# fgnt/padertorch

Measured on AMD Instinct MI355X. Metric: training frames/sec (PIT mask-est, 2-spk 8 kHz), higher is better.
Workload: dtype f32; 1 GPU; BASELINE configs[1]: PIT mask estimator (3xBLSTM-600, K=2, 23.5M params), 32 x 4 s 2-spk 8000 Hz mixtures per GPU and micro-step (8096 frames), 1 micro-step(s) per optimizer step, STFT 512/128 on device, full optimizer step (Adam, clip 1); global_batch=32, parallelism=dp1, blstm=HIP recurrence (csrc/lstm_split.hip), step_driver=one hipGraph per optimizer step (train.graphed.GraphedStep), replayed, lstm_weight_gradients=in place, side stream next to the next recurrence

## Files before the change

include/ptmi.h:

```cpp
#ifndef PTMI_H_
#define PTMI_H_

#include <stdint.h>

#ifdef __cplusplus
extern "C" {
#endif

#define PTMI_OK 0
#define PTMI_E_INVALID (-1)
#define PTMI_E_UNSUPPORTED (-2)

typedef void* ptmi_stream_t;

const char* ptmi_version(void);
const char* ptmi_error_string(int code);

typedef struct ptmi_stft_geom {
    int32_t size;
    int32_t shift;
    int32_t window_length;
    int32_t pad_left;
    int32_t pad_right;
    int32_t pad;
} ptmi_stft_geom;

int64_t ptmi_stft_num_frames(const ptmi_stft_geom* g, int64_t num_samples);
int64_t ptmi_istft_num_samples(const ptmi_stft_geom* g, int64_t num_frames);

#define PTMI_LAYOUT_INTERLEAVED 0
#define PTMI_LAYOUT_CONCAT 1

int ptmi_stft_forward(const float* x, int64_t batch, int64_t x_row_stride, int64_t num_samples,
                      const int32_t* row_samples, const float* window, const float* twiddle,
                      const ptmi_stft_geom* g, int64_t out_frames, int32_t layout, float edge_scale,
                      float* out, ptmi_stream_t stream);

int ptmi_istft_forward(const float* spec, int64_t batch, int64_t num_frames, const int32_t* row_frames,
                       const float* syn_window, const float* twiddle, const ptmi_stft_geom* g,
                       int32_t layout, float edge_scale, int64_t cut_left, int64_t out_samples,
                       int64_t out_row_stride, float* out, ptmi_stream_t stream);

int ptmi_pit_features(const float* y, const float* s, int64_t batch, int32_t K, int64_t row_stride,
                      int64_t num_samples, const int32_t* row_samples, const float* window,
                      const float* twiddle, const ptmi_stft_geom* g, int64_t out_frames, float* Y_abs,
                      float* X_abs, float* cos_pd, ptmi_stream_t stream);
int ptmi_pit_features_packed(const float* y, const float* s, int64_t batch, int32_t K, int64_t row_stride,
                             int64_t num_samples, const int32_t* row_samples, const float* window,
                             const float* twiddle, const ptmi_stft_geom* g, int64_t out_frames, float* Y_abs,
                             float* X_abs, float* cos_pd, float* log1p_packed, uint16_t* log1p_planes,
                             const int64_t* packed_offsets, ptmi_stream_t stream);


int64_t ptmi_pit_workspace_elems(int64_t batch, int64_t t_len, int32_t K, int32_t F);
int ptmi_pit_pairwise_sse(const float* est, const float* obs, const float* tgt, const float* tgt_scale,
                          int64_t batch, int64_t t_len, const int64_t* strides, int32_t K, int32_t F,
                          const int32_t* row_frames, double* workspace, double* sse,
                          ptmi_stream_t stream);

int ptmi_pit_assign(const double* sse, int64_t batch, int32_t nvar, int32_t K, int32_t F,
                    int64_t t_len, const int32_t* row_frames, float* loss, int32_t* perm,
                    float* ex_loss, ptmi_stream_t stream);

int ptmi_pit_backward(const float* est, const float* obs, const float* tgt, const float* tgt_scale,
                      const int32_t* perm, const float* gscale, int64_t batch, int64_t t_len,
                      const int64_t* strides, int32_t K, int32_t F, int32_t nvar, const int32_t* row_frames,
                      float* grad, ptmi_stream_t stream);

int64_t ptmi_dc_workspace_elems(int64_t batch, int64_t T, int32_t F);
int ptmi_dc_loss_forward(const float* x, const float* t, int64_t batch, int64_t T, const int64_t* strides,
                         int32_t E, int32_t K, int32_t F, const int32_t* row_frames, float* workspace,
                         double* gram, float* ex_loss, float* loss, ptmi_stream_t stream);
int ptmi_dc_loss_backward(const float* x, const float* t, const double* gram, const float* gscale,
                          int64_t batch, int64_t T, const int64_t* strides, int32_t E, int32_t K, int32_t F,
                          const int32_t* row_frames, float* dx, ptmi_stream_t stream);


int ptmi_lstm_forward(float* gates, float* hy, float* c, const float* c0, const float* w_hh_pad, const int32_t* batch_sizes,
                      const int64_t* offsets, int32_t T, int32_t max_batch, int32_t H, int32_t KP,
                      int32_t ndir, ptmi_stream_t stream);

int ptmi_lstm_backward(const float* gates, const float* c, const float* c0, const float* dhy, const float* w_hh_t, float* dgates,
                       float* dc_state, const int32_t* batch_sizes, const int64_t* offsets, int32_t T,
                       int32_t max_batch, int32_t H, int32_t ndir, ptmi_stream_t stream);

int64_t ptmi_lstm_flags_elems(int32_t T, int32_t ndir, int32_t max_batch);
int64_t ptmi_lstm_scratch_elems(int32_t T, int32_t ndir, int32_t max_batch, int32_t H, int32_t backward);
int ptmi_lstm_weight_prep(const float* const* w_ih, const float* const* w_hh, const float* const* b_ih,
                          const float* const* b_hh, int32_t ndir, int32_t H, int32_t I, float* w_ih_cat, int32_t Ipad,
                          float* bias, float* w_pad, int32_t KP, float* w_t, uint32_t* amax, ptmi_stream_t stream);
int ptmi_lstm_set_error_sink(uint32_t* word);
int ptmi_lstm_split_enabled(void);
int32_t ptmi_lstm_handoff_cols(int32_t H, int32_t backward);
int32_t ptmi_lstm_backward_planes_ok(int32_t T, int32_t ndir, int32_t max_batch, int64_t rows, int32_t H);
int ptmi_lstm_forward_fills(int32_t T, int32_t ndir, int32_t max_batch, int32_t H);

int ptmi_lstm_forward_persistent(float* gates, float* hy, float* c, const float* c0, const float* w_hh_pad,
                                 const uint32_t* w_hh_amax, const int32_t* batch_sizes_dev, const int64_t* offsets_dev,
                                 const uint64_t* step_masks, uint32_t* flags, int32_t T, int32_t max_batch, int64_t rows,
                                 int32_t H, int32_t KP, int32_t ndir, int32_t prefilled, uint32_t* backward_scratch,
                                 ptmi_stream_t stream);

int ptmi_lstm_backward_persistent(const float* gates, const float* c, const float* c0, const float* dhy, const float* dc_n,
                                  const float* w_hh_t, float* dgates, uint16_t* dgates_t, const int32_t* batch_sizes_dev,
                                  const int64_t* offsets_dev, const uint64_t* step_masks, uint32_t* flags, float* dc_carry,
                                  int32_t T, int32_t max_batch, int64_t rows, int32_t H, int32_t ndir, int32_t s_begin,
                                  int32_t s_end, int32_t prefilled, ptmi_stream_t stream);

int ptmi_stft_logmel(const float* x, int64_t batch, int64_t x_row_stride, int64_t num_samples,
                     const int32_t* row_samples, const float* window, const float* twiddle,
                     const ptmi_stft_geom* g, int64_t out_frames, const int32_t* mel_lo, const int32_t* mel_cnt,
                     const int32_t* mel_off, const float* mel_w, int32_t mel_M, int32_t mel_nnz, int32_t power,
                     int32_t log_, float eps, float* out, ptmi_stream_t stream);
int ptmi_mel_apply(const float* spec, int64_t N, int32_t F, const int32_t* mel_lo, const int32_t* mel_cnt,
                   const int32_t* mel_off, const float* mel_w, int32_t mel_M, int32_t mel_nnz, int32_t log_,
                   float eps, float* out, ptmi_stream_t stream);

typedef struct ptmi_norm_geom {
    int32_t rank;
    int64_t size[5];
    int64_t stat_group_stride[5];
    int64_t indep_stride[5];
    int32_t batch_dim, seq_dim;
} ptmi_norm_geom;
int64_t ptmi_norm_workspace_elems(const ptmi_norm_geom* geom, int32_t which);
int ptmi_norm_reduce(int32_t mode, const float* x, const float* gy, const int32_t* lengths, const float* mean,
                     const float* rstd, const float* gamma, const ptmi_norm_geom* geom, int32_t shift,
                     double* workspace, double* out, ptmi_stream_t stream);
int ptmi_norm_elementwise(int32_t backward, const float* x, const float* gy, const int32_t* lengths,
                          const float* mean, const float* rstd, const float* gamma, const float* beta,
                          const float* c0, const float* c1, const ptmi_norm_geom* geom, int32_t shift,
                          int32_t scale, float* out, ptmi_stream_t stream);

int ptmi_unit_norm_forward(const float* x, float* y, float* inv_norm, int64_t N, int32_t E, int32_t F, float eps,
                           ptmi_stream_t stream);
int ptmi_unit_norm_backward(const float* gy, const float* y, const float* inv_norm, float* dx, int64_t N, int32_t E,
                            int32_t F, float eps, ptmi_stream_t stream);

int64_t ptmi_td_stats_elems(int32_t K);
int64_t ptmi_td_workspace_elems(int64_t batch, int32_t K, int64_t T);
int ptmi_td_pair_stats(const float* est, const float* tgt, const int32_t* lengths, int64_t batch, int32_t K,
                       int64_t T, const int64_t* strides, double* workspace, double* stats,
                       ptmi_stream_t stream);
int ptmi_td_lincomb(const float* x, const float* y, const int32_t* lengths, const float* coef_a,
                    const float* coef_b, const float* coef_c, int64_t batch, int32_t K, int64_t T,
                    const int64_t* strides, float* out, ptmi_stream_t stream);

int ptmi_tas_analysis(const float* x, const float* weight, const float* bias, float* out, int64_t B, int64_t T, int32_t N,
                      int32_t L, int32_t stride, int64_t E, int32_t relu, ptmi_stream_t stream);
int ptmi_tas_synthesis(const float* p, const float* mask, const float* gate, const float* weight, const float* bias, float* y,
                       int32_t K, int64_t B, int32_t N, int32_t L, int32_t stride, int64_t E, int64_t T_out,
                       ptmi_stream_t stream);
int ptmi_tas_masked_decode_backward(const float* gy, const float* mask, const float* encoded, const float* weight, float* dmask,
                                    float* dencoded, int32_t K, int64_t B, int64_t T, int32_t N, int32_t L, int32_t stride,
                                    int64_t E, ptmi_stream_t stream);
int64_t ptmi_tas_wgrad_workspace_elems(int64_t B, int32_t N, int32_t L, int32_t stride, int64_t E);
int ptmi_tas_wgrad(const float* g, const float* mask, const float* gate, const float* x, int32_t K, int64_t B, int64_t T,
                   int32_t N, int32_t L, int32_t stride, int64_t E, float* workspace, float* out, ptmi_stream_t stream);

int64_t ptmi_tcn_depthwise_workspace_elems(int64_t B, int64_t T, int32_t H, int32_t K);
int ptmi_tcn_depthwise_forward(const float* u, const float* slope_in, const float* weight, const float* bias, const float* slope_out,
                               float* v, float* stats, double* workspace, int64_t B, int64_t T, int32_t H, int32_t K,
                               int32_t dilation, float eps, ptmi_stream_t stream);
int ptmi_tcn_depthwise_backward(const float* gv, const float* u, const float* slope_in, const float* weight, const float* bias,
                                const float* slope_out, float* gz, float* gu, float* dparams, double* workspace, int64_t B,
                                int64_t T, int32_t H, int32_t K, int32_t dilation, ptmi_stream_t stream);
int64_t ptmi_tcn_norm_workspace_elems(int64_t B, int64_t T, int32_t C);
int ptmi_tcn_norm_stats(const float* x, float* stats, double* workspace, int64_t B, int64_t T, int32_t C, int32_t rows, float eps,
                        ptmi_stream_t stream);
int ptmi_tcn_norm_apply(const float* x, const float* stats, const float* gamma, const float* beta, float* y, int64_t B, int64_t T,
                        int32_t C, int32_t rows, ptmi_stream_t stream);
int ptmi_tcn_norm_backward(const float* gy, const float* x, const float* stats, const float* gamma, float* dx, float* dparams,
                           float* gsum, double* workspace, int64_t B, int64_t T, int32_t C, int32_t rows, ptmi_stream_t stream);

int64_t ptmi_tasnet_entry_norm_workspace_elems(int64_t B, int32_t N, int64_t E);
int ptmi_tasnet_entry_norm_forward(const float* w, const float* gamma, const float* beta, const void* lengths, int32_t lengths_int64,
                                   float* y, float* stats, int64_t B, int32_t N, int64_t E, float eps, ptmi_stream_t stream);
int ptmi_tasnet_entry_norm_backward(const float* gy, const float* w, const float* stats, const float* gamma, const void* lengths,
                                    int32_t lengths_int64, float* dw, float* dparams, double* workspace, int64_t B, int32_t N,
                                    int64_t E, ptmi_stream_t stream);
int64_t ptmi_tasnet_prelu_workspace_elems(int64_t n);
int ptmi_tasnet_prelu_forward(const float* x, const float* slope, float* y, int64_t n, ptmi_stream_t stream);
int ptmi_tasnet_prelu_backward(const float* g, const float* x, const float* slope, float* gx, float* dslope, double* workspace,
                               int64_t n, ptmi_stream_t stream);
// ... 141 lines not shown
```

padertorch_amd/_lib.py:

```python
import ctypes
import os
import threading
from ctypes import c_char_p, c_double, c_float, c_int, c_int32, c_int64, c_void_p, POINTER
from pathlib import Path

import torch

_PKG = Path(__file__).resolve().parent
LIB_PATH = _PKG / 'libptmi.so'
if os.environ.get('PTMI_LIB'):
    LIB_PATH = Path(os.environ['PTMI_LIB'])


class StftGeom(ctypes.Structure):
    _fields_ = [('size', c_int32), ('shift', c_int32), ('window_length', c_int32),
                ('pad_left', c_int32), ('pad_right', c_int32), ('pad', c_int32)]


class NormGeom(ctypes.Structure):
    _fields_ = [('rank', c_int32), ('size', c_int64 * 5), ('stat_group_stride', c_int64 * 5),
                ('indep_stride', c_int64 * 5), ('batch_dim', c_int32), ('seq_dim', c_int32)]


_P = c_void_p
_G = POINTER(StftGeom)
_I64P = POINTER(c_int64)

SIGNATURES = {
    'ptmi_version': (c_char_p, []),
    'ptmi_error_string': (c_char_p, [c_int]),
    'ptmi_stft_num_frames': (c_int64, [_G, c_int64]),
    'ptmi_istft_num_samples': (c_int64, [_G, c_int64]),
    'ptmi_stft_forward': (c_int, [_P, c_int64, c_int64, c_int64, _P, _P, _P, _G, c_int64, c_int32,
                                  c_float, _P, _P]),
    'ptmi_istft_forward': (c_int, [_P, c_int64, c_int64, _P, _P, _P, _G, c_int32, c_float, c_int64,
                                   c_int64, c_int64, _P, _P]),
    'ptmi_pit_features': (c_int, [_P, _P, c_int64, c_int32, c_int64, c_int64, _P, _P, _P, _G, c_int64,
                                  _P, _P, _P, _P]),
    'ptmi_pit_features_packed': (c_int, [_P, _P, c_int64, c_int32, c_int64, c_int64, _P, _P, _P, _G, c_int64,
                                         _P, _P, _P, _P, _P, _P, _P]),
    'ptmi_pit_workspace_elems': (c_int64, [c_int64, c_int64, c_int32, c_int32]),
    'ptmi_pit_pairwise_sse': (c_int, [_P, _P, _P, _P, c_int64, c_int64, _I64P, c_int32, c_int32, _P,
                                      _P, _P, _P]),
    'ptmi_pit_assign': (c_int, [_P, c_int64, c_int32, c_int32, c_int32, c_int64, _P, _P, _P, _P, _P]),
    'ptmi_pit_backward': (c_int, [_P, _P, _P, _P, _P, _P, c_int64, c_int64, _I64P, c_int32, c_int32,
                                  c_int32, _P, _P, _P]),
    'ptmi_dc_workspace_elems': (c_int64, [c_int64, c_int64, c_int32]),
    'ptmi_dc_loss_forward': (c_int, [_P, _P, c_int64, c_int64, _I64P, c_int32, c_int32, c_int32, _P, _P, _P, _P, _P, _P]),
    'ptmi_dc_loss_backward': (c_int, [_P, _P, _P, _P, c_int64, c_int64, _I64P, c_int32, c_int32, c_int32, _P, _P, _P]),
    'ptmi_stft_logmel': (c_int, [_P, c_int64, c_int64, c_int64, _P, _P, _P, _G, c_int64, _P, _P, _P, _P,
                                 c_int32, c_int32, c_int32, c_int32, c_float, _P, _P]),
    'ptmi_mel_apply': (c_int, [_P, c_int64, c_int32, _P, _P, _P, _P, c_int32, c_int32, c_int32, c_float, _P, _P]),
    'ptmi_norm_workspace_elems': (c_int64, [POINTER(NormGeom), c_int32]),
    'ptmi_norm_reduce': (c_int, [c_int32, _P, _P, _P, _P, _P, _P, POINTER(NormGeom), c_int32, _P, _P, _P]),
    'ptmi_norm_elementwise': (c_int, [c_int32, _P, _P, _P, _P, _P, _P, _P, _P, _P, POINTER(NormGeom), c_int32,
                                      c_int32, _P, _P]),
    'ptmi_td_stats_elems': (c_int64, [c_int32]),
    'ptmi_td_workspace_elems': (c_int64, [c_int64, c_int32, c_int64]),
    'ptmi_td_pair_stats': (c_int, [_P, _P, _P, c_int64, c_int32, c_int64, _I64P, _P, _P, _P]),
    'ptmi_td_lincomb': (c_int, [_P, _P, _P, _P, _P, _P, c_int64, c_int32, c_int64, _I64P, _P, _P]),
    'ptmi_tas_analysis': (c_int, [_P, _P, _P, _P, c_int64, c_int64, c_int32, c_int32, c_int32, c_int64, c_int32, _P]),
    'ptmi_tas_synthesis': (c_int, [_P, _P, _P, _P, _P, _P, c_int32, c_int64, c_int32, c_int32, c_int32, c_int64, c_int64, _P]),
    'ptmi_tas_masked_decode_backward': (c_int, [_P, _P, _P, _P, _P, _P, c_int32, c_int64, c_int64, c_int32, c_int32, c_int32,
                                                c_int64, _P]),
    'ptmi_tas_wgrad_workspace_elems': (c_int64, [c_int64, c_int32, c_int32, c_int32, c_int64]),
    'ptmi_tas_wgrad': (c_int, [_P, _P, _P, _P, c_int32, c_int64, c_int64, c_int32, c_int32, c_int32, c_int64, _P, _P, _P]),
    'ptmi_tcn_depthwise_workspace_elems': (c_int64, [c_int64, c_int64, c_int32, c_int32]),
    'ptmi_tcn_depthwise_forward': (c_int, [_P, _P, _P, _P, _P, _P, _P, _P, c_int64, c_int64, c_int32, c_int32, c_int32, c_float, _P]),
    'ptmi_tcn_depthwise_backward': (c_int, [_P, _P, _P, _P, _P, _P, _P, _P, _P, _P, c_int64, c_int64, c_int32, c_int32, c_int32, _P]),
    'ptmi_tcn_norm_workspace_elems': (c_int64, [c_int64, c_int64, c_int32]),
    'ptmi_tcn_norm_stats': (c_int, [_P, _P, _P, c_int64, c_int64, c_int32, c_int32, c_float, _P]),
    'ptmi_tcn_norm_apply': (c_int, [_P, _P, _P, _P, _P, c_int64, c_int64, c_int32, c_int32, _P]),
    'ptmi_tcn_norm_backward': (c_int, [_P, _P, _P, _P, _P, _P, _P, _P, c_int64, c_int64, c_int32, c_int32, _P]),
    'ptmi_tasnet_entry_norm_workspace_elems': (c_int64, [c_int64, c_int32, c_int64]),
    'ptmi_tasnet_entry_norm_forward': (c_int, [_P, _P, _P, _P, c_int32, _P, _P, c_int64, c_int32, c_int64, c_float, _P]),
    'ptmi_tasnet_entry_norm_backward': (c_int, [_P, _P, _P, _P, _P, c_int32, _P, _P, _P, c_int64, c_int32, c_int64, _P]),
    'ptmi_tasnet_prelu_workspace_elems': (c_int64, [c_int64]),
    'ptmi_tasnet_prelu_forward': (c_int, [_P, _P, _P, c_int64, _P]),
    'ptmi_tasnet_prelu_backward': (c_int, [_P, _P, _P, _P, _P, _P, c_int64, _P]),
    'ptmi_tasnet_mask_head_forward': (c_int, [_P, _P, _P, c_int64, c_int64, c_int32, c_int32, c_int32, c_int32, _P]),
    'ptmi_tasnet_mask_head_backward': (c_int, [_P, _P, _P, _P, c_int64, c_int64, c_int32, c_int32, c_int32, c_int32, _P]),
    'ptmi_tasnet_center_workspace_elems': (c_int64, [c_int64, c_int64, c_int64, c_int64]),
    'ptmi_tasnet_center': (c_int, [_P, _P, _P, c_int64, c_int64, c_int64, c_int64, c_int32, _P]),
    'ptmi_td_rect_workspace_elems': (c_int64, [c_int64, c_int32, c_int32, c_int64]),
    'ptmi_td_rect_stats': (c_int, [_P, _P, c_int64, c_int32, c_int32, c_int64, _I64P, _P, _P, _P, _P]),
    'ptmi_orpit_select': (c_int, [_P, _P, _P, _P, _P, _P, _P, _P, c_int64, c_int32, c_int64, _P]),
    'ptmi_td_rect_lincomb': (c_int, [_P, _P, _P, _P, _P, c_int64, c_int32, c_int32, c_int64, _I64P, _P, _P]),
    'ptmi_orpit_flag_workspace_elems': (c_int64, [c_int64, c_int32, c_int64]),
    'ptmi_orpit_flag_forward': (c_int, [_P, _P, _P, _P, _P, _P, _P, _P, _P, _P, c_int64, c_int32, c_int64, c_int32, c_int32, c_int32,
                                        c_int32, _P]),
    'ptmi_orpit_flag_backward': (c_int, [_P, _P, _P, _P, _P, _P, _P, _P, _P, _P, _P, _P, _P, _P, _P, c_int64, c_int32, c_int64, c_int32,
                                         c_int32, c_int32, c_int32, _P]),
    'ptmi_mask_loss_workspace_elems': (c_int64, [c_int64, c_int32, c_int32, c_int32]),
    'ptmi_mask_loss_forward': (c_int, [_P, _P, _P, c_int32, _P, _I64P, c_int64, c_int32, c_int32, c_int32, c_int32, _P, _P, _P, _P, _P,
                                       _P]),
    'ptmi_mask_loss_backward': (c_int, [_P, _P, _P, c_int32, _P, _I64P, _P, _P, _P, _P, c_int64, c_int32, c_int32, c_int32, c_int32, _P,
                                        _P]),
    'ptmi_gl_partials_elems': (c_int64, []),
    'ptmi_gl_project': (c_int, [_P, _P, c_int64, _P, _P]),
    'ptmi_gl_project_backward': (c_int, [_P, _P, c_int64, _P, _P]),
    'ptmi_gl_update': (c_int, [_P, _P, _P, c_int64, c_float, _P, _P, _P, _P]),
    'ptmi_gl_stft_update': (c_int, [_P, c_int64, c_int64, c_int64, _P, _P, _G, c_int64, c_float, _P, _P, _P, _P, _P, _P]),
    'ptmi_gl_finish': (c_int, [_P, c_int64, c_double, c_int32, _P, _P, _P]),
    'ptmi_bf_psd_workspace_elems': (c_int64, [c_int64, c_int32, c_int64, c_int64, c_int32]),
    'ptmi_bf_psd': (c_int, [_P, _P, _P, _P, c_int64, c_int32, c_int64, c_int64, c_int32, c_int32, c_int32, _P, _P, _P]),
    'ptmi_bf_souden': (c_int, [_P, _P, c_int64, c_int64, c_int32, c_int32, _P, _P, _P, _P, _P]),
    'ptmi_bf_apply': (c_int, [_P, _P, _P, c_int64, c_int32, c_int64, c_int64, _P, _P]),
    'ptmi_bf_eig': (c_int, [_P, _P, c_int64, c_int64, c_int32, c_int32, c_int32, _P, _P, _P, _P]),
    'ptmi_bf_ban': (c_int, [_P, _P, c_int64, c_int64, c_int32, _P, _P]),
    'ptmi_bf_phase': (c_int, [_P, c_int64, c_int64, c_int32, _P, _P]),
    'ptmi_dprnn_num_chunks': (c_int64, [c_int64, c_int32, c_int32]),
    'ptmi_dprnn_tables': (c_int, [_P, c_int32, c_int32, c_int32, c_int32, c_int32, _P, _P, _P, _P]),
    'ptmi_chunk_lstm_max_hidden': (c_int32, []),
    'ptmi_chunk_lstm_max_resident_hidden': (c_int32, []),
    'ptmi_chunk_lstm_tile': (c_int32, []),
    'ptmi_chunk_lstm_forward': (c_int, [_P, _P, _P, _P, _P, _P, _P, _P, c_int32, c_int32, c_int32, c_int32, _P]),
    'ptmi_chunk_lstm_backward': (c_int, [_P, _P, _P, _P, _P, _P, _P, _P, c_int32, c_int32, c_int32, c_int32, _P]),
    'ptmi_dprnn_colsum_workspace_elems': (c_int64, [c_int64, c_int32]),
    'ptmi_dprnn_colsum': (c_int, [_P, c_int64, _P, _P, _P, c_int64, c_int32, _P]),
    'ptmi_dprnn_norm_residual_forward': (c_int, [_P, _P, _P, _P, _P, _P, _P, c_int64, c_int32, c_int32, c_int32, c_float, _P]),
    'ptmi_dprnn_norm_residual_backward': (c_int, [_P, _P, _P, _P, _P, _P, _P, _P, _P, c_int64, c_int32, c_int32, c_int32, _P]),
    'ptmi_dprnn_segment': (c_int, [_P, _I64P, _P, c_int64, c_int64, c_int32, c_int32, c_int32, c_int32, _P]),
    'ptmi_dprnn_overlap_add': (c_int, [_P, _I64P, _P, c_int64, c_int64, c_int32, c_int32, c_int32, c_int32, c_int32, _P]),
    'ptmi_lstm_forward': (c_int, [_P, _P, _P, _P, _P, _P, _P, c_int32, c_int32, c_int32, c_int32, c_int32, _P]),
    'ptmi_lstm_backward': (c_int, [_P, _P, _P, _P, _P, _P, _P, _P, _P, c_int32, c_int32, c_int32, c_int32, _P]),
    'ptmi_unit_norm_forward': (c_int, [_P, _P, _P, c_int64, c_int32, c_int32, c_float, c_void_p]),
    'ptmi_unit_norm_backward': (c_int, [_P, _P, _P, _P, c_int64, c_int32, c_int32, c_float, c_void_p]),
    'ptmi_lstm_flags_elems': (c_int64, [c_int32, c_int32, c_int32]),
    'ptmi_lstm_scratch_elems': (c_int64, [c_int32, c_int32, c_int32, c_int32, c_int32]),
    'ptmi_lstm_weight_prep': (c_int, [_P, _P, _P, _P, c_int32, c_int32, c_int32, _P, c_int32, _P, _P, c_int32, _P, _P, _P]),
    'ptmi_lstm_set_error_sink': (c_int, [_P]),
    'ptmi_lstm_split_enabled': (c_int, []),
    'ptmi_lstm_handoff_cols': (c_int32, [c_int32, c_int32]),
    'ptmi_lstm_forward_persistent': (c_int, [_P, _P, _P, _P, _P, _P, _P, _P, _P, _P, c_int32, c_int32, c_int64, c_int32, c_int32,
                                             c_int32, c_int32, _P, _P]),
    'ptmi_lstm_forward_fills': (c_int, [c_int32, c_int32, c_int32, c_int32]),
    'ptmi_lstm_backward_planes_ok': (c_int32, [c_int32, c_int32, c_int32, c_int64, c_int32]),
    'ptmi_lstm_backward_persistent': (c_int, [_P, _P, _P, _P, _P, _P, _P, _P, _P, _P, _P, _P, _P, c_int32, c_int32, c_int64, c_int32,
                                              c_int32, c_int32, c_int32, c_int32, _P]),
    'ptmi_absmax': (c_int, [_P, c_int64, c_int64, c_int64, _P, _P]),
    'ptmi_absmax_accumulate': (c_int, [_P, c_int64, c_int64, c_int64, _P, _P]),
    'ptmi_planes_elems': (c_int64, [c_int64, c_int64]),
    'ptmi_pack_planes_t': (c_int, [_P, c_int64, c_int64, c_int64, _P, _P, _P]),
    'ptmi_gemm_planes_workspace_elems': (c_int64, [c_int32, c_int32, c_int32, c_int32]),
    'ptmi_pack_planes_n': (c_int, [_P, c_int64, c_int64, c_int64, _P, _P, _P]),
    'ptmi_gemm_planes': (c_int, [_P, _P, _P, _P, _P, _P, c_int64, c_int32, c_int32, c_int32, c_int32, c_int32, c_int32, _P, _P]),
    'ptmi_gemm_planes_relu': (c_int, [_P, _P, _P, _P, _P, _P, c_int64, c_int32, c_int32, c_int32, c_int32, c_int32, _P, _P, c_int32, _P]),
    'ptmi_relu_backward_absmax': (c_int, [_P, _P, _P, c_int64, c_int64, c_int64, c_int64, c_int64, _P, c_int32, _P]),
    'ptmi_pack_planes_t_bf16': (c_int, [_P, c_int64, c_int64, c_int64, _P, _P]),
    'ptmi_pack_planes_n_bf16': (c_int, [_P, c_int64, c_int64, c_int64, _P, _P]),
    'ptmi_pack_planes_into': (c_int, [_P, c_int64, c_int64, c_int64, c_int32, c_int32, _P, _P, c_int64, c_int64, c_int64, _P]),
    'ptmi_gemm_planes_bf16': (c_int, [_P, _P, _P, _P, c_int64, c_int32, c_int32, c_int32, c_int32, c_int32, c_int32, _P, _P]),
    'ptmi_gemm_planes_bf16_two': (c_int, [_P, _P, _P, _P, c_int32, c_int64, c_int32, c_int32, c_int32, c_int32, c_int32, c_int32, _P, _P]),
    'ptmi_gemm_planes_plan': (c_int32, [c_int32, c_int32, c_int32, c_int32]),
    'ptmi_gemm_planes_bf16_group': (c_int, [_P, c_int32, c_int32, _P, _P, c_int32, _P, _P, c_int32, c_int32, c_int32, c_int32, _P, _P]),
    'ptmi_gemm_planes_group_workspace_elems': (c_int64, [c_int32, c_int32, _P, c_int32, _P, c_int32, c_int32]),
    'ptmi_gemm_planes_group_plan': (c_int32, [c_int32, c_int32, _P, c_int32, _P, c_int32, c_int32]),
    'ptmi_pack_planes_t_bf16_list': (c_int, [_P, _P, _P, _P, c_int32, c_int64, _P]),
    'ptmi_comm_rccl_version': (c_int32, []),
    'ptmi_comm_unique_id': (c_int, [_P]),
    'ptmi_comm_create': (c_int, [_P, c_int32, c_int32, _P]),
    'ptmi_allreduce_sum': (c_int, [_P, _P, c_int64, _P]),
    'ptmi_comm_destroy': (c_int, [_P]),
    'ptmi_lstm_bias_grad_add': (c_int, [_P, c_int32, c_int32, _P, _P, _P]),
    'ptmi_grad_norm_workspace_elems': (c_int64, []),
    'ptmi_grad_norm': (c_int32, [_P, c_int64, _P, _P, _P]),
    'ptmi_adam_flat': (c_int32, [_P, _P, _P, _P, c_int32, c_int64, _P, c_float, _P, _P, _P, _P, c_double, c_double, c_double,
                                 c_double, c_double, _P, c_int32, _P]),
}

_lib = None


def load():
    global _lib
    if _lib is None:
        if not LIB_PATH.exists():
            raise ImportError(
                f'{LIB_PATH} is missing: build the HIP kernels first '
                f'(python -m padertorch_amd.build, or __graft_entry__.build()). '
                f'padertorch_amd has no CPU fallback.')
        lib = ctypes.CDLL(str(LIB_PATH))
        for name, (res, args) in SIGNATURES.items():
            fn = getattr(lib, name)
            fn.restype = res
            fn.argtypes = args
        _lib = lib
    return _lib


_hooks = None


def test_hooks():
    global _hooks
    if _hooks is None:
        path = _PKG / 'libptmi_testhooks.so'
        if not path.exists():
            raise ImportError(f'{path} is missing: python -m padertorch_amd.build')
        lib = ctypes.CDLL(str(path))
        lib.ptmi_test_occupy.restype = c_int
        lib.ptmi_test_occupy.argtypes = [c_int32, c_int32, c_int32, c_int64, _P]
        _hooks = lib
    return _hooks


def select_gemm_tile(tile):
    if tile is None or tile < 0:
        os.environ.pop('PTMI_GEMM_TILE', None)
    else:
        assert 0 <= tile <= 5, tile
        os.environ['PTMI_GEMM_TILE'] = str(int(tile))
    return 0


def check(rc, what=''):
    if rc != 0:
        msg = load().ptmi_error_string(int(rc)).decode()
        raise RuntimeError(f'{what}: {msg} (code {rc})')


def ptr(t):
    return None if t is None else t.data_ptr()


def require_gpu(*tensors):
    for t in tensors:
        if t is not None and not t.is_cuda:
            raise RuntimeError(
                'padertorch_amd ops run on an MI355X (HIP) device only and have no CPU fallback; '
                f'got a tensor on {t.device}. Move the example to the GPU first.')


def stream(device):
    return torch.cuda.current_stream(device).cuda_stream


def device_key(device):
    device = torch.device(device)
    return device.type, device.index if device.index is not None else torch.cuda.current_device()


KERNEL_TIMERS = None


def timed(name, fn, *args):
    if KERNEL_TIMERS is None:
        return fn(*args)
    e0 = torch.cuda.Event(enable_timing=True)
    e1 = torch.cuda.Event(enable_timing=True)
    e0.record()
    rc = fn(*args)
    e1.record()
    KERNEL_TIMERS.append((name, e0, e1))
    return rc


class _Staging:

    def __init__(self, half_bytes=1 << 24):
        self.half = half_bytes
        self.buf = torch.empty(2 * half_bytes, dtype=torch.uint8, pin_memory=True)
        self.np = self.buf.numpy()
        self.which, self.off = 0, 0
        self.events = [[], []]
        self.streams = [{}, {}]
        self.lock = threading.Lock()

    def put(self, t, device):
        n = t.numel() * t.element_size()
        if n > self.half // 4:
            return t.pin_memory().to(device, non_blocking=True)
        with self.lock:
            if self.off + n > self.half:
                for stream in self.streams[self.which].values():
                    ev = torch.cuda.Event()
                    ev.record(stream)
                    self.events[self.which].append(ev)
                self.streams[self.which] = {}
                self.which, self.off = self.which ^ 1, 0
                for ev in self.events[self.which]:
                    ev.synchronize()
                self.events[self.which] = []
            start = self.which * self.half + self.off
            self.off += (n + 63) // 64 * 64
            stage = self.buf[start:start + n].view(t.dtype).view(t.shape)
            self.np[start:start + n] = t.numpy().reshape(-1).view('uint8')
            cur = torch.cuda.current_stream(device)
            self.streams[self.which][cur.cuda_stream] = cur
            return stage.to(device, non_blocking=True)


_STAGING = {}


def host_to_device(values, dtype, device):
    t = torch.as_tensor(values, dtype=dtype)
    device = torch.device(device)
# ... 34 lines not shown
```

padertorch_amd/csrc/gemm_planes.hip:

```cpp
#include <algorithm>

#include "common.h"

namespace ptmi {

typedef _Float16 h8 __attribute__((ext_vector_type(8)));
typedef __bf16 b8 __attribute__((ext_vector_type(8)));
typedef float f4 __attribute__((ext_vector_type(4)));

constexpr int PBM = 128, PBN = 128;
constexpr int FR = 64;

__device__ __forceinline__ float plane_scale(const unsigned* amax_bits) {
    if (!amax_bits) return 1.f;
    const unsigned e = (*amax_bits >> 23) & 0xffu;
    if (e == 0u || e == 0xffu) return 1.f;
    return __uint_as_float((unsigned)(127 + 13 + 127 - (int)e) << 23);
}

struct PlanesArgs {
    const uint4* A;
    const uint4* B;
    float* C;
    float* workspace;
    const unsigned* amax_a;
    const unsigned* amax_b;
    const float* bias;
    int M, N, KB;
    long long ldc;
    int accumulate;
    int kb_per_split;
    int tiles_m, tiles_n;
    float* C2 = nullptr;
    int m_split = 0;
    int relu = 0;
    unsigned* amax_out = nullptr;
};

__device__ __forceinline__ void block_amax(unsigned* out, unsigned m, unsigned* red) {
#pragma unroll
    for (int o = 32; o > 0; o >>= 1) m = max(m, (unsigned)__shfl_xor((int)m, o));
    if ((threadIdx.x & 63) == 0) red[threadIdx.x >> 6] = m;
    __syncthreads();
    if (threadIdx.x == 0) {
        for (unsigned w = 1; w < (blockDim.x >> 6); ++w) m = max(m, red[w]);
        if (m != 0u) atomicMax(out, m >= 0x7f800000u ? 0x7f7fffffu : m);
    }
}

template <bool BF16, bool ONE, bool RELU = false>
__global__ __launch_bounds__(256, 2) void gemm_planes_kernel(const PlanesArgs G) {
#if __HIP_DEVICE_COMPILE__
    constexpr int PIECES = 32;
    __shared__ uint4 lds[2 * PIECES * FR];
    const int tid = threadIdx.x, lane = tid & 63, wave = tid >> 6;
    const int T = G.tiles_m * G.tiles_n;
    const int q = T / 8, r8 = T % 8, xcd = blockIdx.x & 7, idx = blockIdx.x >> 3;
    if (idx >= (xcd < r8 ? q + 1 : q)) return;
    const int tile = (xcd < r8 ? xcd * (q + 1) : r8 * (q + 1) + (xcd - r8) * q) + idx;
    const int tm = tile / G.tiles_n, tn = tile - tm * G.tiles_n;
    const int kb0 = blockIdx.z * G.kb_per_split, kb1 = min(G.KB, kb0 + G.kb_per_split);
    const int wm = wave >> 1, wn = wave & 1;
    const float inv = 1.f / (plane_scale(G.amax_a) * plane_scale(G.amax_b));
    const int rta = (G.M + 15) / 16, rtb = (G.N + 15) / 16;
    const uint4* gsrc[8];
#pragma unroll
    for (int i = 0; i < 8; ++i) {
        const int f = wave * 8 + i;
        const bool isa = f < 16;
        const int rt = (f & 15) >> 1, p = f & 1;
        const long long row_tile = min((long long)(isa ? tm : tn) * 8 + rt, (long long)(isa ? rta : rtb) - 1);
        gsrc[i] = (isa ? G.A : G.B) + ((row_tile * G.KB + kb0) * 2 + p) * FR + lane;
    }
    f4 acc[4][4];
#pragma unroll
    for (int i = 0; i < 4; ++i)
#pragma unroll
        for (int j = 0; j < 4; ++j) acc[i][j] = f4{0.f, 0.f, 0.f, 0.f};
    if (kb0 < kb1) {
#pragma unroll
        for (int i = 0; i < 8; ++i)
            if (!ONE || !(i & 1)) __builtin_amdgcn_global_load_lds(gsrc[i], &lds[(wave * 8 + i) * FR], 16, 0, 0);
    }
    for (int kb = kb0; kb < kb1; ++kb) {
        const int st = (kb - kb0) & 1;
        asm volatile("s_waitcnt vmcnt(0)" ::: "memory");
        __builtin_amdgcn_s_barrier();
        const uint4* sa = &lds[(st * PIECES + wm * 8) * FR + lane];
        const uint4* sb = &lds[(st * PIECES + 16 + wn * 8) * FR + lane];
        const bool more = kb + 1 < kb1;
        h8 bh[4], bl[4];
#pragma unroll
        for (int j = 0; j < 4; ++j) {
            bh[j] = __builtin_bit_cast(h8, sb[(j * 2 + 0) * FR]);
            bl[j] = ONE ? bh[j] : __builtin_bit_cast(h8, sb[(j * 2 + 1) * FR]);
        }
        h8 ah = __builtin_bit_cast(h8, sa[0]), al = ONE ? ah : __builtin_bit_cast(h8, sa[FR]);
#pragma unroll
        for (int i = 0; i < 4; ++i) {
            h8 nh = ah, nl = al;
            if (i + 1 < 4) {
                nh = __builtin_bit_cast(h8, sa[((i + 1) * 2 + 0) * FR]);
                nl = ONE ? nh : __builtin_bit_cast(h8, sa[((i + 1) * 2 + 1) * FR]);
            }
            if (more) {
#pragma unroll
                for (int pc = 2 * i; pc < 2 * i + 2; ++pc)
                    if (!ONE || !(pc & 1))
                        __builtin_amdgcn_global_load_lds(gsrc[pc] + (long long)(kb + 1 - kb0) * 2 * FR,
                                                         &lds[((st ^ 1) * PIECES + wave * 8 + pc) * FR], 16, 0, 0);
            }
#pragma unroll
            for (int p = ONE ? 2 : 0; p < 3; ++p)
#pragma unroll
                for (int j = 0; j < 4; ++j)
                    acc[i][j] = BF16 ? __builtin_amdgcn_mfma_f32_16x16x32_bf16(__builtin_bit_cast(b8, p == 0 ? bl[j] : bh[j]),
                                                                               __builtin_bit_cast(b8, p == 1 ? al : ah), acc[i][j], 0, 0, 0)
                                     : __builtin_amdgcn_mfma_f32_16x16x32_f16(p == 0 ? bl[j] : bh[j], p == 1 ? al : ah, acc[i][j], 0, 0, 0);
            ah = nh;
            al = nl;
        }
    }
    const bool slab = gridDim.z > 1;
    float* const Cz = slab ? G.workspace + (long long)blockIdx.z * G.M * G.N : G.C;
    const long long ldc = slab ? G.N : G.ldc;
    const bool vec = (ldc & 3) == 0 && ((reinterpret_cast<unsigned long long>(Cz) | reinterpret_cast<unsigned long long>(G.C2)) & 15) == 0;
    const bool add = G.accumulate && !slab;
    const int r = lane & 15, g = lane >> 4;
    f4 bv[4];
    {
        const bool bias_on = G.bias != nullptr && !slab;
        const bool bvec = (reinterpret_cast<unsigned long long>(G.bias) & 15) == 0;
#pragma unroll
        for (int j = 0; j < 4; ++j) {
            const int n = tn * PBN + wn * 64 + j * 16 + g * 4;
            bv[j] = f4{0.f, 0.f, 0.f, 0.f};
            if (bias_on && bvec && n + 3 < G.N) {
                bv[j] = *reinterpret_cast<const f4*>(G.bias + n);
            } else if (bias_on) {
#pragma unroll
                for (int e = 0; e < 4; ++e) bv[j][e] = G.bias[min(n + e, G.N - 1)];
            }
        }
    }
    const bool fuse = RELU && !slab;
    unsigned mx = 0u;
#pragma unroll
    for (int i = 0; i < 4; ++i) {
        const int m = tm * PBM + wm * 64 + i * 16 + r;
        if (m >= G.M) continue;
        const bool second = !slab && G.C2 != nullptr && m >= G.m_split;
        float* const rowp = second ? G.C2 + (long long)(m - G.m_split) * ldc : Cz + (long long)m * ldc;
#pragma unroll
        for (int j = 0; j < 4; ++j) {
            const int n = tn * PBN + wn * 64 + j * 16 + g * 4;
            float* o = rowp + n;
            f4 v = acc[i][j] * inv + bv[j];
            if (RELU && fuse) {
#pragma unroll
                for (int e = 0; e < 4; ++e) {
                    v[e] = v[e] < 0.f ? 0.f : v[e];
                    if (n + e < G.N) mx = max(mx, __float_as_uint(v[e]));
                }
            }
            if (vec && n + 3 < G.N) {
                f4* o4 = reinterpret_cast<f4*>(o);
                *o4 = add ? *o4 + v : v;
            } else {
#pragma unroll
                for (int e = 0; e < 4; ++e)
                    if (n + e < G.N) o[e] = add ? o[e] + v[e] : v[e];
            }
        }
    }
    if constexpr (RELU) {
        if (!slab && G.amax_out) {
            __shared__ unsigned red[4];
            block_amax(G.amax_out, mx, red);
        }
    }
#endif
}

struct BigArgs {
    const uint4* A;
    const uint4* B;
    float* C;
    const unsigned* amax_a;
    const unsigned* amax_b;
    const float* bias;
    int M, N, KB;
    long long ldc;
    int accumulate;
    int tiles_m, tiles_n, band;
    unsigned a_bytes, b_bytes;
    int splits = 1, kb_per_split = 0;
    float* slabs = nullptr;
    float* C2 = nullptr;
    int m_split = 0;
    int relu = 0;
    unsigned* amax_out = nullptr;
};

constexpr int GROUP_SEGS = 3, GROUP_BLOCKS = 6;
struct GroupTable {
    const uint4* B[GROUP_SEGS];
    unsigned b_bytes[GROUP_SEGS];
    int rtb[GROUP_SEGS];
    int part_rt0[2], part_rts[2];
    int tile_start[GROUP_BLOCKS + 1];
    int total_tiles;
    int tiles_m[GROUP_BLOCKS], tiles_n[GROUP_BLOCKS], part[GROUP_BLOCKS], seg[GROUP_BLOCKS], rows[GROUP_BLOCKS], cols[GROUP_BLOCKS];
    long long slab_off[GROUP_BLOCKS], slab_stride[GROUP_BLOCKS];
};
struct GroupBigArgs : BigArgs {
    GroupTable T;
};

template <bool BF16, int MT, int NT, bool ONE, bool RELU = false, class ARGS = BigArgs>
__global__ __launch_bounds__(512, 2) void gemm_planes_big_kernel(const ARGS G) {
#if __HIP_DEVICE_COMPILE__
    constexpr bool GROUP = __is_same(ARGS, GroupBigArgs);
    constexpr int WM = 2, WN = 4, RA = WM * MT, RB = WN * NT, PIECES = 2 * (RA + RB);
    constexpr int PA = 2 * RA / 8, PB = 2 * RB / 8, PW = PA + PB;
    static_assert((2 * RA) % 8 == 0 && (2 * RB) % 8 == 0, "pieces per wave");
    __shared__ uint4 lds[2 * PIECES * FR];
    const int lane = threadIdx.x & 63;
    const int wave = __builtin_amdgcn_readfirstlane(threadIdx.x >> 6);
    const int wm = wave / WN, wn = wave % WN;
    const __amdgpu_buffer_rsrc_t ra = __builtin_amdgcn_make_buffer_rsrc(const_cast<uint4*>(G.A), 0, G.a_bytes, 0x00020000);
    const __amdgpu_buffer_rsrc_t rb = __builtin_amdgcn_make_buffer_rsrc(const_cast<uint4*>(G.B), 0, G.b_bytes, 0x00020000);
    const int voff = lane * 16;
    const int KB = G.KB;
    const int rta = (G.M + 15) / 16, rtb = (G.N + 15) / 16;
    const float inv = GROUP ? 1.f : 1.f / (plane_scale(G.amax_a) * plane_scale(G.amax_b));

    int TT = G.tiles_m * G.tiles_n;
    if constexpr (GROUP) TT = G.T.total_tiles;
    const int T = TT * G.splits;
    const int xcd = blockIdx.x & 7, j0 = blockIdx.x >> 3, per = gridDim.x >> 3;
    const int q = T / 8, r8 = T % 8;
    const int cnt = xcd < r8 ? q + 1 : q;
    const int first = xcd < r8 ? xcd * (q + 1) : r8 * (q + 1) + (xcd - r8) * q;
    if (j0 >= cnt) return;
    const int band_tiles = G.band * G.tiles_n;
    auto tile_rc = [&](int item, int& tm, int& tn, int& z) {
        z = item / TT;
        const int idx = item - z * TT;
        const int b = idx / band_tiles, rem = idx - b * band_tiles;
        const int h = min(G.band, G.tiles_m - b * G.band);
        tn = rem / h;
        tm = b * G.band + (rem - tn * h);
    };
    struct Blk {
        int a_rt0, a_rts, b_rts;
        __amdgpu_buffer_rsrc_t rb;
        int rows, cols;
        long long slab;
        long long slab_stride;
    };
    auto tile_rc_group = [&](int item, int& tm, int& tn, int& z, Blk& k) {
        if constexpr (GROUP) {
            z = item / TT;
            int idx = item - z * TT, blk = 0;
#pragma unroll
            for (int b = 1; b < GROUP_BLOCKS; ++b) blk += idx >= G.T.tile_start[b] ? 1 : 0;
            idx -= G.T.tile_start[blk];
            const int tiles_m = G.T.tiles_m[blk], tiles_n = G.T.tiles_n[blk];
            const int bt = G.band * tiles_n;
            const int b = idx / bt, rem = idx - b * bt;
            const int h = min(G.band, tiles_m - b * G.band);
            tn = rem / h;
            tm = b * G.band + (rem - tn * h);
            const int p = G.T.part[blk], s = G.T.seg[blk];
            k.a_rt0 = G.T.part_rt0[p];
            k.a_rts = G.T.part_rts[p];
            k.b_rts = G.T.rtb[s];
            k.rb = __builtin_amdgcn_make_buffer_rsrc(const_cast<uint4*>(G.T.B[s]), 0, G.T.b_bytes[s], 0x00020000);
            k.rows = G.T.rows[blk];
            k.cols = G.T.cols[blk];
            k.slab = G.T.slab_off[blk];
            k.slab_stride = G.T.slab_stride[blk];
        }
    };
// ... 24 lines not shown
                __builtin_amdgcn_raw_ptr_buffer_load_lds(rbk, &lds[(st * PIECES + 2 * RA + f) * FR], 16, voff, ((rt * KB + kb) * 2 + (f & 1)) * 1024, 0, 0);
        }
    };

    f4 acc[MT][NT];
#pragma unroll
    for (int i = 0; i < MT; ++i)
#pragma unroll
        for (int j = 0; j < NT; ++j) acc[i][j] = f4{0.f, 0.f, 0.f, 0.f};

    int idx = j0, tm, tn, tz;
    Blk bk{}, nbk{};
    if constexpr (GROUP) {
        tile_rc_group(first + idx, tm, tn, tz, bk);
#pragma unroll
        for (int i = 0; i < PW; ++i) issue_group(i, tm, tn, tz * KBS, 0, bk.a_rt0, bk.a_rts, bk.b_rts, bk.rb);
    } else {
        tile_rc(first + idx, tm, tn, tz);
#pragma unroll
        for (int i = 0; i < PW; ++i) issue(i, tm, tn, tz * KBS, 0);
    }
    int st = 0;
    constexpr int PPI = (PW + MT - 1) / MT;
    unsigned relu_max = 0u;
    while (true) {
        const int nidx = idx + per;
        const bool has_next_tile = nidx < cnt;
        int ntm = tm, ntn = tn, ntz = tz;
        if constexpr (GROUP) {
            nbk = bk;
            if (has_next_tile) tile_rc_group(first + nidx, ntm, ntn, ntz, nbk);
        } else {
            if (has_next_tile) tile_rc(first + nidx, ntm, ntn, ntz);
        }
        const int kb_lo = tz * KBS, kb_hi = min(KB, kb_lo + KBS);
        for (int kb = kb_lo; kb < kb_hi; ++kb) {
            asm volatile("s_waitcnt vmcnt(0)" ::: "memory");
            __builtin_amdgcn_s_barrier();
            const bool last = kb + 1 == kb_hi;
            const int ptm = last ? ntm : tm, ptn = last ? ntn : tn, pkb = last ? ntz * KBS : kb + 1;
            const int pa0 = last ? nbk.a_rt0 : bk.a_rt0, pas = last ? nbk.a_rts : bk.a_rts, pbs = last ? nbk.b_rts : bk.b_rts;
            const __amdgpu_buffer_rsrc_t prb = last ? nbk.rb : bk.rb;
            const uint4* sa = &lds[(st * PIECES + wm * MT * 2) * FR + lane];
            const uint4* sb = &lds[(st * PIECES + 2 * RA + wn * NT * 2) * FR + lane];
            h8 bh[NT], bl[NT];
#pragma unroll
            for (int j = 0; j < NT; ++j) {
                bh[j] = __builtin_bit_cast(h8, sb[(j * 2 + 0) * FR]);
                bl[j] = ONE ? bh[j] : __builtin_bit_cast(h8, sb[(j * 2 + 1) * FR]);
            }
            h8 ah = __builtin_bit_cast(h8, sa[0]), al = ONE ? ah : __builtin_bit_cast(h8, sa[FR]);
#pragma unroll
            for (int i = 0; i < MT; ++i) {
                h8 nh = ah, nl = al;
                if (i + 1 < MT) {
                    nh = __builtin_bit_cast(h8, sa[((i + 1) * 2 + 0) * FR]);
                    nl = ONE ? nh : __builtin_bit_cast(h8, sa[((i + 1) * 2 + 1) * FR]);
                }
#pragma unroll
                for (int pc = i * PPI; pc < (i + 1) * PPI; ++pc) {
                    if constexpr (GROUP) {
                        if (pc < PW) issue_group(pc, ptm, ptn, pkb, st ^ 1, pa0, pas, pbs, prb);
                    } else {
                        if (pc < PW) issue(pc, ptm, ptn, pkb, st ^ 1);
                    }
                }
#pragma unroll
                for (int p = ONE ? 2 : 0; p < 3; ++p)
#pragma unroll
                    for (int j = 0; j < NT; ++j)
                        acc[i][j] = BF16 ? __builtin_amdgcn_mfma_f32_16x16x32_bf16(__builtin_bit_cast(b8, p == 0 ? bl[j] : bh[j]),
                                                                                   __builtin_bit_cast(b8, p == 1 ? al : ah), acc[i][j], 0, 0, 0)
                                         : __builtin_amdgcn_mfma_f32_16x16x32_f16(p == 0 ? bl[j] : bh[j], p == 1 ? al : ah, acc[i][j], 0, 0, 0);
                ah = nh;
                al = nl;
            }
            st ^= 1;
        }
        {
            const int r = lane & 15, g = lane >> 4;
            const int n0 = (tn * WN + wn) * NT * 16 + g * 4;
            const bool vec = (G.ldc & 3) == 0 && ((reinterpret_cast<unsigned long long>(G.C) | reinterpret_cast<unsigned long long>(G.C2)) & 15) == 0;
            const bool full = vec && (tn * WN + wn + 1) * NT * 16 <= G.N;
            f4 bv[NT];
#pragma unroll
            for (int j = 0; j < NT; ++j) {
                bv[j] = f4{0.f, 0.f, 0.f, 0.f};
                if (G.bias) {
#pragma unroll
                    for (int e = 0; e < 4; ++e) bv[j][e] = G.bias[min(n0 + j * 16 + e, G.N - 1)];
                }
            }
            const int mrow = (tm * WM + wm) * MT * 16 + r;
            if (GROUP || G.splits > 1) {
                const int sM = GROUP ? bk.rows : G.M, sN = GROUP ? bk.cols : G.N;
                float* const srow = GROUP ? G.slabs + bk.slab + tz * bk.slab_stride + (long long)mrow * sN + n0
                                          : G.slabs + ((long long)tz * G.M + mrow) * G.N + n0;
                const bool svec = (sN & 3) == 0 && (reinterpret_cast<unsigned long long>(G.slabs) & 15) == 0;
                const bool sfull = svec && (tn * WN + wn + 1) * NT * 16 <= sN;
#pragma unroll
                for (int i = 0; i < MT; ++i) {
                    const bool ok = mrow + i * 16 < sM;
#pragma unroll
                    for (int j = 0; j < NT; ++j) {
                        const f4 v = acc[i][j] * inv;
                        acc[i][j] = f4{0.f, 0.f, 0.f, 0.f};
                        float* o = srow + (long long)i * 16 * sN + j * 16;
                        if (sfull) {
                            if (ok) *reinterpret_cast<f4*>(o) = v;
                        } else {
#pragma unroll
                            for (int e = 0; e < 4; ++e)
                                if (ok && n0 + j * 16 + e < sN) o[e] = v[e];
                        }
                    }
                }
                if (!has_next_tile) break;
                idx = nidx;
                tm = ntm;
                tn = ntn;
                tz = ntz;
                if constexpr (GROUP) bk = nbk;
                continue;
            }
            auto rowp = [&](int i) {
                const int m = mrow + i * 16;
                return (G.C2 != nullptr && m >= G.m_split ? G.C2 + (long long)(m - G.m_split) * G.ldc : G.C + (long long)m * G.ldc) + n0;
            };
            if (RELU) {
#pragma unroll
                for (int i = 0; i < MT; ++i) {
                    const bool ok = mrow + i * 16 < G.M;
#pragma unroll
                    for (int j = 0; j < NT; ++j) {
                        f4 v = acc[i][j] * inv + bv[j];
                        acc[i][j] = f4{0.f, 0.f, 0.f, 0.f};
#pragma unroll
                        for (int e = 0; e < 4; ++e) {
                            v[e] = v[e] < 0.f ? 0.f : v[e];
                            if (ok && n0 + j * 16 + e < G.N) relu_max = max(relu_max, __float_as_uint(v[e]));
                        }
                        float* o = rowp(i) + j * 16;
                        if (full) {
                            if (ok) *reinterpret_cast<f4*>(o) = v;
                        } else {
#pragma unroll
                            for (int e = 0; e < 4; ++e)
                                if (ok && n0 + j * 16 + e < G.N) o[e] = v[e];
                        }
                    }
                }
            } else if (full && !G.accumulate) {
#pragma unroll
                for (int i = 0; i < MT; ++i) {
#pragma unroll
                    for (int j = 0; j < NT; ++j) {
                        const f4 v = acc[i][j] * inv + bv[j];
                        acc[i][j] = f4{0.f, 0.f, 0.f, 0.f};
                        if (mrow + i * 16 < G.M) *reinterpret_cast<f4*>(rowp(i) + j * 16) = v;
                    }
                }
            } else if (full) {
#pragma unroll
                for (int i = 0; i < MT; ++i) {
                    const bool ok = mrow + i * 16 < G.M;
                    f4 old[NT];
#pragma unroll
                    for (int j = 0; j < NT; ++j)
                        old[j] = ok ? *reinterpret_cast<const f4*>(rowp(i) + j * 16) : f4{0.f, 0.f, 0.f, 0.f};
#pragma unroll
                    for (int j = 0; j < NT; ++j) {
                        const f4 v = acc[i][j] * inv + bv[j] + old[j];
                        acc[i][j] = f4{0.f, 0.f, 0.f, 0.f};
                        if (ok) *reinterpret_cast<f4*>(rowp(i) + j * 16) = v;
                    }
                }
            } else {
#pragma unroll
                for (int i = 0; i < MT; ++i) {
                    const bool ok = mrow + i * 16 < G.M;
#pragma unroll
                    for (int j = 0; j < NT; ++j) {
                        const f4 v = acc[i][j] * inv + bv[j];
                        acc[i][j] = f4{0.f, 0.f, 0.f, 0.f};
                        float* o = rowp(i) + j * 16;
#pragma unroll
                        for (int e = 0; e < 4; ++e)
                            if (ok && n0 + j * 16 + e < G.N) o[e] = G.accumulate ? o[e] + v[e] : v[e];
                    }
                }
            }
        }
        if (!has_next_tile) break;
        idx = nidx;
        tm = ntm;
        tn = ntn;
        tz = ntz;
    }
    asm volatile("s_waitcnt vmcnt(0)" ::: "memory");
    if constexpr (RELU) {
        if (G.amax_out && G.splits == 1) {
            __shared__ unsigned red[8];
            block_amax(G.amax_out, relu_max, red);
        }
    }
#endif
}

__global__ __launch_bounds__(256) void absmax_kernel(const float* __restrict__ x, long long rows, long long cols, long long ld,
                                                     unsigned* __restrict__ out) {
    __shared__ unsigned red[4];
    const long long n = rows * cols;
    unsigned m = 0u;
    if (ld == cols && (cols & 3) == 0 && (reinterpret_cast<uintptr_t>(x) & 15) == 0) {
        const long long n4 = n >> 2, stride = (long long)gridDim.x * 256;
        const f4* x4 = reinterpret_cast<const f4*>(x);
        long long i = blockIdx.x * 256ll + threadIdx.x;
        for (; i + 3 * stride < n4; i += 4 * stride) {
            const f4 v0 = x4[i], v1 = x4[i + stride], v2 = x4[i + 2 * stride], v3 = x4[i + 3 * stride];
#pragma unroll
            for (int q = 0; q < 4; ++q)
                m = max(max(m, __float_as_uint(v0[q]) & 0x7fffffffu),
                        max(max(__float_as_uint(v1[q]) & 0x7fffffffu, __float_as_uint(v2[q]) & 0x7fffffffu), __float_as_uint(v3[q]) & 0x7fffffffu));
        }
        for (; i < n4; i += stride) {
            const f4 v = x4[i];
#pragma unroll
            for (int q = 0; q < 4; ++q) m = max(m, __float_as_uint(v[q]) & 0x7fffffffu);
        }
    } else {
        for (long long i = blockIdx.x * 256ll + threadIdx.x; i < n; i += (long long)gridDim.x * 256) {
            const long long r = i / cols, c = i - r * cols;
            m = max(m, __float_as_uint(x[r * ld + c]) & 0x7fffffffu);
        }
    }
#pragma unroll
    for (int o = 32; o > 0; o >>= 1) m = max(m, (unsigned)__shfl_xor((int)m, o));
    if ((threadIdx.x & 63) == 0) red[threadIdx.x >> 6] = m;
    __syncthreads();
    if (threadIdx.x == 0) {
        m = max(max(red[0], red[1]), max(red[2], red[3]));
        if (m >= 0x7f800000u) m = 0x7f7fffffu;
        atomicMax(out, m);
    }
}

template <bool BF16>
__device__ __forceinline__ void split_chunk(const float (&v)[8], uint4* hi_out, uint4* lo_out) {
    if (BF16) {
        b8 hi, lo;
#pragma unroll
        for (int e = 0; e < 8; ++e) {
            hi[e] = (__bf16)v[e];
            lo[e] = (__bf16)(v[e] - (float)hi[e]);
        }
        *hi_out = __builtin_bit_cast(uint4, hi);
        *lo_out = __builtin_bit_cast(uint4, lo);
    } else {
        h8 hi, lo;
#pragma unroll
        for (int e = 0; e < 8; ++e) {
            hi[e] = (_Float16)v[e];
            lo[e] = (_Float16)(v[e] - (float)hi[e]);
        }
        *hi_out = __builtin_bit_cast(uint4, hi);
        *lo_out = __builtin_bit_cast(uint4, lo);
    }
}

__global__ __launch_bounds__(256) void planes_reduce_kernel(const float* __restrict__ ws, int splits, float* __restrict__ C, long long ldc,
                                                            const float* __restrict__ bias, int M, int N, int accumulate,
                                                            float* __restrict__ C2 = nullptr, int m_split = 0, int relu = 0,
                                                            unsigned* __restrict__ amax_out = nullptr) {
    const long long total = (long long)M * N;
    unsigned mx = 0u;
    for (long long i = blockIdx.x * 256ll + threadIdx.x; i < total; i += (long long)gridDim.x * 256) {
        const int r = (int)(i / N), c = (int)(i - (long long)r * N);
        float sum = 0.f;
        for (int z = 0; z < splits; ++z) sum += ws[(long long)z * total + i];
        if (bias) sum += bias[c];
        if (relu) {
            sum = sum < 0.f ? 0.f : sum;
            mx = max(mx, __float_as_uint(sum));
        }
        float* o = (C2 != nullptr && r >= m_split) ? C2 + (long long)(r - m_split) * ldc + c : C + (long long)r * ldc + c;
        *o = accumulate ? *o + sum : sum;
    }
    if (relu && amax_out) {
        __shared__ unsigned red[4];
        block_amax(amax_out, mx, red);
    }
}

struct ReduceGroupArgs {
    const float* ws;
    int splits, nblocks, accumulate;
    long long start[GROUP_BLOCKS + 1];
    long long slab_off[GROUP_BLOCKS], slab_stride[GROUP_BLOCKS];
    float* C[GROUP_BLOCKS];
    long long ldc[GROUP_BLOCKS];
    int cols[GROUP_BLOCKS];
    int vec[GROUP_BLOCKS];
};

__global__ __launch_bounds__(256) void planes_reduce_kernel(const ReduceGroupArgs R) {
    const long long total = R.start[R.nblocks];
    for (long long i = blockIdx.x * 256ll + threadIdx.x; i < total; i += (long long)gridDim.x * 256) {
        int b = 0;
#pragma unroll
        for (int q = 1; q < GROUP_BLOCKS; ++q) b += (q < R.nblocks && i >= R.start[q]) ? 1 : 0;
        const int N = R.cols[b];
        const long long stride = R.slab_stride[b];
        if (R.vec[b]) {
            const long long j = (i - R.start[b]) * 4;
            const int r = (int)(j / N), c = (int)(j - (long long)r * N);
            const float* w = R.ws + R.slab_off[b] + j;
            f4 sum = {0.f, 0.f, 0.f, 0.f};
            for (int z = 0; z < R.splits; ++z) sum += *reinterpret_cast<const f4*>(w + (long long)z * stride);
            f4* o = reinterpret_cast<f4*>(R.C[b] + (long long)r * R.ldc[b] + c);
            *o = R.accumulate ? *o + sum : sum;
        } else {
            const long long j = i - R.start[b];
            const int r = (int)(j / N), c = (int)(j - (long long)r * N);
            const float* w = R.ws + R.slab_off[b] + j;
            float sum = 0.f;
            for (int z = 0; z < R.splits; ++z) sum += w[(long long)z * stride];
            float* o = R.C[b] + (long long)r * R.ldc[b] + c;
            *o = R.accumulate ? *o + sum : sum;
        }
    }
}

__global__ __launch_bounds__(256) void relu_backward_absmax_kernel(const float* __restrict__ g, const float* __restrict__ y, float* __restrict__ out,
                                                                   long long rows, long long cols, long long ld_g, long long ld_y, long long ld_o,
                                                                   unsigned* __restrict__ amax_out) {
    unsigned mx = 0u;
    const long long n = rows * cols;
    if (ld_g == cols && ld_y == cols && ld_o == cols && (cols & 3) == 0 &&
        ((reinterpret_cast<uintptr_t>(g) | reinterpret_cast<uintptr_t>(y) | reinterpret_cast<uintptr_t>(out)) & 15) == 0) {
        const long long n4 = n >> 2, stride = (long long)gridDim.x * 256;
        const f4* g4 = reinterpret_cast<const f4*>(g);
        const f4* y4 = reinterpret_cast<const f4*>(y);
        f4* o4 = reinterpret_cast<f4*>(out);
        long long i = blockIdx.x * 256ll + threadIdx.x;
        for (; i + stride < n4; i += 2 * stride) {
            const f4 ga = g4[i], ya = y4[i], gb = g4[i + stride], yb = y4[i + stride];
            f4 va, vb;
#pragma unroll
            for (int q = 0; q < 4; ++q) {
                va[q] = ya[q] <= 0.f ? 0.f : ga[q];
                vb[q] = yb[q] <= 0.f ? 0.f : gb[q];
                mx = max(mx, max(__float_as_uint(va[q]) & 0x7fffffffu, __float_as_uint(vb[q]) & 0x7fffffffu));
            }
            o4[i] = va;
            o4[i + stride] = vb;
        }
        for (; i < n4; i += stride) {
            const f4 ga = g4[i], ya = y4[i];
            f4 va;
// ... 170 lines not shown
    PTMI_RETURN_IF((reinterpret_cast<uintptr_t>(out) & 15) != 0, PTMI_E_INVALID);
    const long long own = (k_rows + 31) / 32, KB = kbn ? kbn : own, KBS = kbs ? kbs : KB, cb = (cols + 63) / 64;
    PTMI_RETURN_IF(KB < own || kbo < 0 || kbo + KB > KBS, PTMI_E_INVALID);
    hipStream_t st = static_cast<hipStream_t>(stream);
    if (ld % 4 == 0 && (reinterpret_cast<uintptr_t>(x) & 15) == 0 && KB <= 65535) {
        const dim3 grid4((unsigned)cb, (unsigned)KB);
        if (bf16)
            hipLaunchKernelGGL(pack_planes_t4_kernel<true>, grid4, dim3(256), 0, st, x, (long long)k_rows, (long long)cols, (long long)ld, amax,
                               reinterpret_cast<uint4*>(out), KBS, (long long)kbo);
        else
            hipLaunchKernelGGL(pack_planes_t4_kernel<false>, grid4, dim3(256), 0, st, x, (long long)k_rows, (long long)cols, (long long)ld, amax,
                               reinterpret_cast<uint4*>(out), KBS, (long long)kbo);
        return launch_status();
    }
    PTMI_RETURN_IF(cb > 65535, PTMI_E_UNSUPPORTED);
    const dim3 grid((unsigned)KB, (unsigned)cb);
    if (bf16)
        hipLaunchKernelGGL(pack_planes_t_kernel<true>, grid, dim3(256), 0, st, x, (long long)k_rows, (long long)cols, (long long)ld, amax,
                           reinterpret_cast<uint4*>(out), KBS, (long long)kbo);
    else
        hipLaunchKernelGGL(pack_planes_t_kernel<false>, grid, dim3(256), 0, st, x, (long long)k_rows, (long long)cols, (long long)ld, amax,
                           reinterpret_cast<uint4*>(out), KBS, (long long)kbo);
    return launch_status();
}

static int pack_n_impl(bool bf16, const float* x, int64_t rows, int64_t k, int64_t ld, const uint32_t* amax, uint16_t* out,
                       ptmi_stream_t stream, int64_t kbs = 0, int64_t kbo = 0, int64_t kbn = 0) {
    PTMI_RETURN_IF(!x || !out || rows < 1 || k < 1 || ld < k, PTMI_E_INVALID);
    PTMI_RETURN_IF((reinterpret_cast<uintptr_t>(out) & 15) != 0, PTMI_E_INVALID);
    const long long own = (k + 31) / 32, KB = kbn ? kbn : own, KBS = kbs ? kbs : KB, rt = (rows + 15) / 16;
    PTMI_RETURN_IF(KB < own || kbo < 0 || kbo + KB > KBS, PTMI_E_INVALID);
    PTMI_RETURN_IF(rt > 65535, PTMI_E_UNSUPPORTED);
    const dim3 grid((unsigned)((KB + 3) / 4), (unsigned)rt);
    hipStream_t st = static_cast<hipStream_t>(stream);
    if (bf16)
        hipLaunchKernelGGL(pack_planes_n_kernel<true>, grid, dim3(256), 0, st, x, (long long)rows, (long long)k, (long long)ld, amax,
                           reinterpret_cast<uint4*>(out), KB, KBS, (long long)kbo);
    else
        hipLaunchKernelGGL(pack_planes_n_kernel<false>, grid, dim3(256), 0, st, x, (long long)rows, (long long)k, (long long)ld, amax,
                           reinterpret_cast<uint4*>(out), KB, KBS, (long long)kbo);
    return launch_status();
}

int ptmi_pack_planes_t(const float* x, int64_t k_rows, int64_t cols, int64_t ld, const uint32_t* amax, uint16_t* out,
                       ptmi_stream_t stream) {
    return pack_t_impl(false, x, k_rows, cols, ld, amax, out, stream);
}

int ptmi_pack_planes_n(const float* x, int64_t rows, int64_t k, int64_t ld, const uint32_t* amax, uint16_t* out,
                       ptmi_stream_t stream) {
    return pack_n_impl(false, x, rows, k, ld, amax, out, stream);
}

int ptmi_pack_planes_t_bf16(const float* x, int64_t k_rows, int64_t cols, int64_t ld, uint16_t* out, ptmi_stream_t stream) {
    return pack_t_impl(true, x, k_rows, cols, ld, nullptr, out, stream);
}

int ptmi_pack_planes_n_bf16(const float* x, int64_t rows, int64_t k, int64_t ld, uint16_t* out, ptmi_stream_t stream) {
    return pack_n_impl(true, x, rows, k, ld, nullptr, out, stream);
}

int ptmi_pack_planes_into(const float* x, int64_t rows_or_k, int64_t cols, int64_t ld, int32_t transposed, int32_t bf16, const uint32_t* amax,
                          uint16_t* out, int64_t kb_total, int64_t kb_offset, int64_t kb_count, ptmi_stream_t stream) {
    PTMI_RETURN_IF(kb_total < 1 || kb_count < 1, PTMI_E_INVALID);
    return transposed ? pack_t_impl(bf16 != 0, x, rows_or_k, cols, ld, amax, out, stream, kb_total, kb_offset, kb_count)
                      : pack_n_impl(bf16 != 0, x, rows_or_k, cols, ld, amax, out, stream, kb_total, kb_offset, kb_count);
}

int64_t ptmi_gemm_planes_workspace_elems(int32_t m, int32_t n, int32_t k, int32_t split_k) {
    const int KB = (k + 31) / 32;
    if (split_k < 0) split_k = -split_k;
    const int splits = std::max(1, std::min<int>(split_k, KB));
    return splits > 1 ? (int64_t)splits * m * n : 0;
}

}

#include <type_traits>
static int tile_override() {
    const char* v = getenv("PTMI_GEMM_TILE");
    if (!v || !*v) return -1;
    const int t = atoi(v);
    return (t >= 0 && t <= 5) ? t : -1;
}

static int cu_count() {
    static int cus = 0;
    if (!cus) {
        int dev = 0, v = 0;
        if (hipGetDevice(&dev) == hipSuccess && hipDeviceGetAttribute(&v, hipDeviceAttributeMultiprocessorCount, dev) == hipSuccess && v > 0)
            cus = v;
        else
            cus = 256;
    }
    return cus;
}

struct Tile { int mt, nt; double eff; };
constexpr Tile TILES[] = {{8, 5, 1.0}, {8, 4, 1.0}, {8, 3, 0.92}, {4, 5, 0.86}, {4, 4, 0.85}};
constexpr int NTILES = 5;

template <int I = NTILES - 1, class F>
static void with_tile(int tile, F&& f) {
    if constexpr (I > 0)
        if (tile != I) return with_tile<I - 1>(tile, f);
    f(std::integral_constant<int, I>{});
}

template <class F>
static void with_variant(bool bf16, bool one, bool relu, F&& f) {
    constexpr std::true_type yes{};
    constexpr std::false_type no{};
    if (relu) return f(no, no, yes);
    if (bf16) return one ? f(yes, yes, no) : f(yes, no, no);
    return one ? f(no, yes, no) : f(no, no, no);
}

constexpr long long PLANES_LIMIT = 1ll << 31;
static long long planes_bytes(int rows, int KB) { return (long long)((rows + 15) / 16) * KB * 2048; }

static int whole_ranges(int split_k, int KB) {
    const int splits = std::max(1, std::min(split_k, KB));
    const int per = (KB + splits - 1) / splits;
    return (KB + per - 1) / per;
}

struct BigPick { int tile; int splits; };

static BigPick pick_big(const int* rows, const int* cols, int nblocks, int KB, int max_splits, bool always_slabs, int pinned) {
    const int cus = cu_count();
    const double unit = 3.1e-5;
    BigPick best{-1, 1};
    double best_cost = 1e300;
    const int smax = std::max(1, std::min(max_splits, KB / 4));
    double elems = 0.0;
    for (int b = 0; b < nblocks; ++b) elems += (double)rows[b] * cols[b];
    for (int i = -1; i < NTILES; ++i) {
        if (pinned >= 0 && pinned != (i < 0 ? 5 : i)) continue;
        const int tr = i < 0 ? 128 : 32 * TILES[i].mt, tc = i < 0 ? 128 : 64 * TILES[i].nt;
        const double area = (double)tr * tc;
        const double eff = i < 0 ? 0.79 : TILES[i].eff;
        long long tiles = 0;
        for (int b = 0; b < nblocks; ++b) tiles += (long long)((rows[b] + tr - 1) / tr) * ((cols[b] + tc - 1) / tc);
        const int slots = i < 0 ? 2 * cus : cus;
        const double rate = i < 0 ? 2.0 : 1.0;
        for (int S = 1; S <= smax; ++S) {
            const int per = (KB + S - 1) / S;
            if ((KB + per - 1) / per != S) continue;
            const long long rounds = (tiles * S + slots - 1) / slots;
            double cost = (max_splits <= 1 && !always_slabs) ? (double)rounds * rate * area / eff * KB * unit
                                                             : (double)rounds * rate * (per * area * unit / eff + 10.0 * area * unit);
            if (S > 1 || always_slabs) cost += (double)(S + 2) * elems * 4.0 / 4.0e6 + 8.0;
            if (cost < best_cost) {
                best_cost = cost;
                best = BigPick{i, S};
            }
        }
    }
    return best;
}

struct Plan { int tile, splits, kb_per_split, KB; };

static Plan plan_call(int m, int n, int k, int split_k) {
    const int KB = (k + 31) / 32;
    const bool co_resident = split_k < 0;
    const int splits = whole_ranges(co_resident ? -split_k : split_k, KB), pinned = tile_override();
    BigPick pk = pick_big(&m, &n, 1, KB, (co_resident && pinned < 0) ? 1 : splits, false, pinned);
    if (pinned >= 0) pk.splits = splits;
    else if (co_resident) pk = BigPick{-1, splits};
    if (planes_bytes(m, KB) >= PLANES_LIMIT || planes_bytes(n, KB) >= PLANES_LIMIT) pk.tile = -1;
    return Plan{pk.tile, pk.splits, (KB + pk.splits - 1) / pk.splits, KB};
}

static int32_t plan_code(int tile, int splits) { return (tile < 0 ? 5 : tile) * 100 + splits; }

struct PlanesCall {
    const uint16_t *a = nullptr, *b = nullptr;
    const uint32_t *amax_a = nullptr, *amax_b = nullptr;
    const float* bias = nullptr;
    float *c = nullptr, *c2 = nullptr;
    int32_t m_split = 0;
    int64_t ldc = 0;
    int32_t m = 0, n = 0, k = 0, accumulate = 0, split_k = 1;
    int relu = 0;
    uint32_t* amax_out = nullptr;
    float* workspace = nullptr;
    bool bf16 = false, one = false;
    ptmi_stream_t stream = nullptr;
};

static BigArgs big_args(const PlanesCall& q, const Plan& p) {
    const bool slabs = p.splits > 1;
    return {.A = reinterpret_cast<const uint4*>(q.a), .B = reinterpret_cast<const uint4*>(q.b), .C = q.c, .amax_a = q.amax_a, .amax_b = q.amax_b,
            .bias = slabs ? nullptr : q.bias, .M = q.m, .N = q.n, .KB = p.KB, .ldc = q.ldc, .accumulate = (q.accumulate && !slabs) ? 1 : 0,
            .band = 4, .a_bytes = (unsigned)planes_bytes(q.m, p.KB), .b_bytes = (unsigned)planes_bytes(q.n, p.KB), .splits = p.splits,
            .kb_per_split = p.kb_per_split, .slabs = q.workspace, .C2 = q.c2, .m_split = q.m_split, .relu = slabs ? 0 : q.relu,
            .amax_out = q.amax_out};
}

static PlanesArgs planes_args(const PlanesCall& q, const Plan& p) {
    return {.A = reinterpret_cast<const uint4*>(q.a), .B = reinterpret_cast<const uint4*>(q.b), .C = q.c, .workspace = q.workspace,
            .amax_a = q.amax_a, .amax_b = q.amax_b, .bias = q.bias, .M = q.m, .N = q.n, .KB = p.KB, .ldc = q.ldc,
            .accumulate = q.accumulate ? 1 : 0, .kb_per_split = p.kb_per_split, .tiles_m = (q.m + PBM - 1) / PBM, .tiles_n = (q.n + PBN - 1) / PBN,
            .C2 = q.c2, .m_split = q.m_split, .relu = p.splits > 1 ? 0 : q.relu, .amax_out = q.amax_out};
}

static int reduce_slabs(const PlanesCall& q, int splits, hipStream_t st) {
    const long long total = (long long)q.m * q.n;
    const unsigned rgrid = (unsigned)std::min<long long>((total + 255) / 256, q.relu ? 1024 : 4096);
    hipLaunchKernelGGL(planes_reduce_kernel, dim3(rgrid), dim3(256), 0, st, q.workspace, splits, q.c, (long long)q.ldc, q.bias, q.m, q.n,
                       q.accumulate ? 1 : 0, q.c2, q.m_split, q.relu, q.amax_out);
    return launch_status();
}

static int gemm_planes_impl(const PlanesCall& q) {
    PTMI_RETURN_IF(!q.a || !q.b || !q.c || q.m < 1 || q.n < 1 || q.k < 1 || q.ldc < q.n, PTMI_E_INVALID);
    PTMI_RETURN_IF(q.relu && (q.accumulate || q.c2 || q.bf16 || q.one), PTMI_E_INVALID);
    PTMI_RETURN_IF(q.c2 && (q.m_split < 16 || q.m_split >= q.m || q.m_split % 16 != 0), PTMI_E_INVALID);
    PTMI_RETURN_IF(((reinterpret_cast<uintptr_t>(q.a) | reinterpret_cast<uintptr_t>(q.b)) & 15) != 0, PTMI_E_INVALID);
    PTMI_RETURN_IF(!q.workspace && ptmi_gemm_planes_workspace_elems(q.m, q.n, q.k, q.split_k) > 0, PTMI_E_INVALID);
    const Plan p = plan_call(q.m, q.n, q.k, q.split_k);
    const bool relu = q.relu && p.splits == 1;
    hipStream_t st = static_cast<hipStream_t>(q.stream);
    if (p.tile >= 0) {
        BigArgs G = big_args(q, p);
        with_tile(p.tile, [&](auto t) {
            constexpr int MT = TILES[decltype(t)::value].mt, NT = TILES[decltype(t)::value].nt;
            G.tiles_m = (q.m + 32 * MT - 1) / (32 * MT);
            G.tiles_n = (q.n + 64 * NT - 1) / (64 * NT);
            const dim3 grid((unsigned)std::min((G.tiles_m * G.tiles_n * p.splits + 7) / 8 * 8, cu_count() / 8 * 8));
            with_variant(q.bf16, q.one, relu, [&](auto bf16, auto one, auto rl) {
                hipLaunchKernelGGL((gemm_planes_big_kernel<decltype(bf16)::value, MT, NT, decltype(one)::value, decltype(rl)::value>), grid,
                                   dim3(512), 0, st, G);
            });
        });
    } else {
        const PlanesArgs G = planes_args(q, p);
        const dim3 grid((unsigned)((G.tiles_m * G.tiles_n + 7) / 8 * 8), 1u, (unsigned)p.splits);
        with_variant(q.bf16, q.one, relu, [&](auto bf16, auto one, auto rl) {
            hipLaunchKernelGGL((gemm_planes_kernel<decltype(bf16)::value, decltype(one)::value, decltype(rl)::value>), grid, dim3(256), 0, st, G);
        });
    }
    const int rc = launch_status();
    return (rc != PTMI_OK || p.splits == 1) ? rc : reduce_slabs(q, p.splits, st);
}

extern "C" {

int ptmi_gemm_planes_relu(const uint16_t* a, const uint32_t* amax_a, const uint16_t* b, const uint32_t* amax_b, const float* bias, float* c,
                          int64_t ldc, int32_t m, int32_t n, int32_t k, int32_t split_k, int32_t products, float* workspace,
                          uint32_t* amax_out, int32_t amax_zeroed, ptmi_stream_t stream) {
    PTMI_RETURN_IF(products != 3 && products != 1, PTMI_E_INVALID);
    if (amax_out && !amax_zeroed) {
        hipError_t e = zero_words_async(amax_out, 1, static_cast<hipStream_t>(stream));
        if (e != hipSuccess) return (int)e;
    }
    return gemm_planes_impl({.a = a, .b = b, .amax_a = amax_a, .amax_b = amax_b, .bias = bias, .c = c, .ldc = ldc, .m = m, .n = n, .k = k,
                             .split_k = split_k, .relu = 1, .amax_out = amax_out, .workspace = workspace, .one = products == 1, .stream = stream});
}

int ptmi_relu_backward_absmax(const float* g, const float* y, float* out, int64_t rows, int64_t cols, int64_t ld_g, int64_t ld_y,
                              int64_t ld_out, uint32_t* amax_out, int32_t amax_zeroed, ptmi_stream_t stream) {
    PTMI_RETURN_IF(!g || !y || !out || !amax_out || rows < 0 || cols < 0 || ld_g < cols || ld_y < cols || ld_out < cols, PTMI_E_INVALID);
    hipStream_t st = static_cast<hipStream_t>(stream);
    if (!amax_zeroed) {
        hipError_t e = zero_words_async(amax_out, 1, st);
        if (e != hipSuccess) return (int)e;
    }
    if (rows * cols == 0) return PTMI_OK;
    const long long work = (rows * cols + 4095) / 4096;
    const unsigned grid = (unsigned)std::min<long long>(std::max<long long>(work, 1), 1024);
    hipLaunchKernelGGL(relu_backward_absmax_kernel, dim3(grid), dim3(256), 0, st, g, y, out, (long long)rows, (long long)cols, (long long)ld_g,
                       (long long)ld_y, (long long)ld_out, amax_out);
    return launch_status();
}

int ptmi_gemm_planes(const uint16_t* a, const uint32_t* amax_a, const uint16_t* b, const uint32_t* amax_b, const float* bias, float* c,
                     int64_t ldc, int32_t m, int32_t n, int32_t k, int32_t accumulate, int32_t split_k, int32_t products,
                     float* workspace, ptmi_stream_t stream) {
    PTMI_RETURN_IF(products != 3 && products != 1, PTMI_E_INVALID);
    return gemm_planes_impl({.a = a, .b = b, .amax_a = amax_a, .amax_b = amax_b, .bias = bias, .c = c, .ldc = ldc, .m = m, .n = n, .k = k,
                             .accumulate = accumulate, .split_k = split_k, .workspace = workspace, .one = products == 1, .stream = stream});
}

int32_t ptmi_gemm_planes_plan(int32_t m, int32_t n, int32_t k, int32_t split_k) {
    if (m < 1 || n < 1 || k < 1) return -1;
    const Plan p = plan_call(m, n, k, split_k);
    return plan_code(p.tile, p.splits);
}

int ptmi_gemm_planes_bf16(const uint16_t* a, const uint16_t* b, const float* bias, float* c, int64_t ldc, int32_t m, int32_t n,
                          int32_t k, int32_t accumulate, int32_t split_k, int32_t products, float* workspace, ptmi_stream_t stream) {
    PTMI_RETURN_IF(products != 3 && products != 1, PTMI_E_INVALID);
    return gemm_planes_impl({.a = a, .b = b, .bias = bias, .c = c, .ldc = ldc, .m = m, .n = n, .k = k, .accumulate = accumulate,
// ... 181 lines not shown
```

padertorch_amd/csrc/lstm.hip:

```cpp
#include <stdio.h>
#include <stdlib.h>

#include "common.h"
#include "lstm_common.h"

namespace ptmi {

struct StepMeta {
    long long row0[2];
    long long prow0[2];
    long long qrow0[2];
    int nb[2];
    int nprev[2];
    int npv[2];
};

struct LstmArgs {
    float* gx;
    float* hy;
    float* c;
    const float* w;
    int H, KP, ndir, dbg;
    StepMeta m;
    const float* c0;
// ... 361 lines not shown
    return T >= 1 && max_batch >= 1 && rows >= 1 && H >= 1 && H % 4 == 0 && (ndir == 1 || ndir == 2) && ptmi_lstm_split_enabled();
}

struct BwdPlan {
    bool ok;
    int G32;
    int mtl;
    int ntiles;
    int nx;
    int per_launch;
    bool planes;
};

static BwdPlan bwd_plan(int T, int ndir, int max_batch, int64_t rows, int H) {
    BwdPlan p{};
    if (!plannable(T, ndir, max_batch, rows, H)) return p;
    constexpr int NW = 8, CB = 10;
    const int G32 = round32(4 * H);
    if ((G32 / 32 + NW - 1) / NW > CB) return p;
    p.G32 = G32;
    const int resident = cu_count() - 16;
    p.nx = (H + 15) / 16;
    if ((long long)p.nx * ndir > resident || p.nx > kSlots) return p;
    const int nt16 = (max_batch + 15) / 16, fit = resident / (p.nx * ndir);
    p.mtl = nt16 > fit ? 2 : 1;
    p.ntiles = (nt16 + p.mtl - 1) / p.mtl;
    p.per_launch = std::min(p.ntiles, fit);
    p.planes = rows == (int64_t)T * max_batch && max_batch % 16 == 0;
    p.ok = true;
    return p;
}

struct FwdPlan {
    bool ok;
    int KP32;
    int jt, mtl;
    int ntiles;
    int jx;
    int per_launch;
    int fills;
};

static FwdPlan fwd_plan(int T, int ndir, int max_batch, int64_t rows, int H) {
    FwdPlan p{};
    if (!plannable(T, ndir, max_batch, rows, H)) return p;
    constexpr int NW = 8, CB = 3;
    const int KP32 = round32(H);
    if ((KP32 / 32 + NW - 1) / NW > CB) return p;
    p.KP32 = KP32;
    const int cus = cu_count();
    p.jt = max_batch <= 16 ? 8 : 12;
    p.mtl = max_batch <= 32 ? 1 : 2;
    if (p.jt == 12 && (long long)((H + 11) / 12) * ndir > cus) p.jt = 16;
    if (p.jt == 16 && (long long)((H + 15) / 16) * ndir > cus) p.jt = 8;
    p.ntiles = (max_batch + 16 * p.mtl - 1) / (16 * p.mtl);
    p.jx = (H + p.jt - 1) / p.jt;
    const int cap = p.jt >= 12 ? cus : cus * 7 / 4;
    if ((long long)p.jx * ndir > cap || p.jx > kSlots) return p;
    p.per_launch = std::min(p.ntiles, cap / (p.jx * ndir));
    if (!fwd_split_instantiated(p.jt, p.mtl) || (long long)p.jx * ndir * p.per_launch > cus) return p;
    p.ok = true;
    if ((long long)p.jx * ndir * p.ntiles <= cus && 16 * p.mtl * p.jt <= 7 * 64 && bwd_plan(T, ndir, max_batch, rows, H).G32) p.fills = 2;
    return p;
}

int32_t ptmi_lstm_handoff_cols(int32_t H, int32_t backward) {
    return backward ? bwd_plan(1, 1, 1, 1, H).G32 : fwd_plan(1, 1, 1, 1, H).KP32;
}

int ptmi_lstm_forward_fills(int32_t T, int32_t ndir, int32_t max_batch, int32_t H) {
    return fwd_plan(T, ndir, max_batch, (int64_t)T * max_batch, H).fills;
}

int32_t ptmi_lstm_backward_planes_ok(int32_t T, int32_t ndir, int32_t max_batch, int64_t rows, int32_t H) {
    const BwdPlan p = bwd_plan(T, ndir, max_batch, rows, H);
    return p.ok && p.planes ? 1 : 0;
}

static int env_int(const char* name, int fallback) {
    const char* v = getenv(name);
    return v ? atoi(v) : fallback;
}

int ptmi_lstm_forward_persistent(float* gates, float* hy, float* c, const float* c0, const float* w_hh_pad,
                                 const uint32_t* w_hh_amax, const int32_t* batch_sizes_dev, const int64_t* offsets_dev,
                                 const uint64_t* step_masks, uint32_t* flags, int32_t T, int32_t max_batch, int64_t rows,
                                 int32_t H, int32_t KP, int32_t ndir, int32_t prefilled, uint32_t* backward_scratch,
                                 ptmi_stream_t stream) {
    PTMI_RETURN_IF(!gates || !hy || !c || !w_hh_pad || !batch_sizes_dev || !offsets_dev || !flags, PTMI_E_INVALID);
    PTMI_RETURN_IF(T < 1 || max_batch < 1 || H < 1 || (ndir != 1 && ndir != 2) || rows < 1, PTMI_E_INVALID);
    const bool uniform = rows == (int64_t)T * max_batch;
    PTMI_RETURN_IF(step_masks && (c0 || !uniform || max_batch > 64), PTMI_E_UNSUPPORTED);
    PTMI_RETURN_IF(H % 4 != 0 || KP != (H + 15) / 16 * 16, PTMI_E_UNSUPPORTED);
    const FwdPlan P = fwd_plan(T, ndir, max_batch, rows, H);
    PTMI_RETURN_IF(!P.ok, PTMI_E_UNSUPPORTED);
    const long long hy_bytes = rows * ndir * H * 4;
    PTMI_RETURN_IF(hy_bytes > 0x7fffffffLL, PTMI_E_UNSUPPORTED);

    hipStream_t st = static_cast<hipStream_t>(stream);
    const int64_t plane_elems = lstm_tile_elems(T, ndir, max_batch, P.KP32), flag_elems = ptmi_lstm_flags_elems(T, ndir, max_batch);
    float* const hyt = reinterpret_cast<float*>(flags);
    flags += plane_elems;
    if (!prefilled) {
        int fe = daf_fill_and_zero(hyt, (size_t)plane_elems, flags, (size_t)flag_elems, st);
        if (fe) return fe;
    } else {
        hipError_t e = zero_words_async(flags, (size_t)flag_elems, st);
        if (e != hipSuccess) return (int)e;
    }
    LstmPersistArgs A{gates, hy, c, w_hh_pad, batch_sizes_dev, offsets_dev, flags, T, H, KP, ndir,
                      (unsigned)P.jx, (unsigned)env_int("PTMI_LSTM_MAX_POLLS", 1 << 22), (int)hy_bytes, (unsigned)(flag_elems - 8),
                      env_int("PTMI_LSTM_DBG", 0), 0, P.ntiles, c0, max_batch, hyt, (max_batch + 15) / 16, w_hh_amax, P.KP32};
    A.err_sink = error_sink();
    A.uniform = uniform ? 1 : 0;
    A.masks = reinterpret_cast<const unsigned long long*>(step_masks);
    if (backward_scratch && P.fills) {
        A.fill_ptr = reinterpret_cast<uint4*>(backward_scratch);
        A.fill_n16 = (unsigned long long)lstm_tile_elems(T, ndir, max_batch, bwd_plan(T, ndir, max_batch, rows, H).G32) / 4;
        A.zero_n16 = (unsigned long long)bwd_tail_elems(T, ndir, max_batch, H) / 4;
    }
    const int cus = cu_count();
    for (int t0 = 0; t0 < P.ntiles; t0 += P.per_launch) {
        A.tile0 = t0;
        A.nx = P.jx;
        A.nt = std::min(P.per_launch, P.ntiles - t0);
        const int chains = ndir * A.nt;
        A.span = (chains <= 8 && 8 % chains == 0 && (P.jx + 8 / chains - 1) / (8 / chains) * 8 <= cus) ? 8 / chains : 0;
        const dim3 grid = A.span ? dim3((unsigned)((P.jx + A.span - 1) / A.span * 8))
                                 : dim3((unsigned)P.jx, (unsigned)ndir, (unsigned)A.nt);
        int rc = launch_fwd_split(A, P.jt, P.mtl, grid, st);
        if (rc) return rc;
    }
    return PTMI_OK;
}

__global__ void zero_tp_tail_kernel(uint4* planes, long long tiles, int kb_total) {
    const long long i = (long long)blockIdx.x * blockDim.x + threadIdx.x;
    if (i >= tiles * 64) return;
    const long long tile = i >> 6;
    const int plane = (int)(i >> 5) & 1, ch = 32 + (int)(i & 31);
    planes[((tile * kb_total + kb_total - 1) * 2 + plane) * 64 + ch] = make_uint4(0u, 0u, 0u, 0u);
}

int ptmi_lstm_backward_persistent(const float* gates, const float* c, const float* c0, const float* dhy, const float* dc_n,
                                  const float* w_hh_t, float* dgates, uint16_t* dgates_t, const int32_t* batch_sizes_dev,
                                  const int64_t* offsets_dev, const uint64_t* step_masks, uint32_t* flags, float* dc_carry,
                                  int32_t T, int32_t max_batch, int64_t rows, int32_t H, int32_t ndir, int32_t s_begin,
                                  int32_t s_end, int32_t prefilled, ptmi_stream_t stream) {
    PTMI_RETURN_IF(!gates || !c || !dhy || !w_hh_t || !batch_sizes_dev || !offsets_dev || !flags, PTMI_E_INVALID);
    PTMI_RETURN_IF(T < 1 || max_batch < 1 || H < 1 || (ndir != 1 && ndir != 2) || rows < 1, PTMI_E_INVALID);
    PTMI_RETURN_IF(!dgates && !dgates_t, PTMI_E_INVALID);
    PTMI_RETURN_IF(dgates_t && (reinterpret_cast<uintptr_t>(dgates_t) & 15) != 0, PTMI_E_INVALID);
    PTMI_RETURN_IF(s_begin < 0 || s_end > T || s_begin >= s_end, PTMI_E_INVALID);
    const bool whole = s_begin == 0 && s_end == T;
    PTMI_RETURN_IF(!whole && (!dc_carry || dc_n), PTMI_E_INVALID);
    const bool uniform = rows == (int64_t)T * max_batch;
    PTMI_RETURN_IF(dc_n && step_masks, PTMI_E_UNSUPPORTED);
    PTMI_RETURN_IF(step_masks && (c0 || !uniform || max_batch > 64 || !whole), PTMI_E_UNSUPPORTED);
    PTMI_RETURN_IF(H % 4 != 0, PTMI_E_UNSUPPORTED);
    const BwdPlan P = bwd_plan(T, ndir, max_batch, rows, H);
    PTMI_RETURN_IF(!P.ok, PTMI_E_UNSUPPORTED);
    PTMI_RETURN_IF(dgates_t && !P.planes, PTMI_E_UNSUPPORTED);
    const long long dg_bytes = rows * ndir * 4 * H * 4;
    PTMI_RETURN_IF(dg_bytes > 0x7fffffffLL, PTMI_E_UNSUPPORTED);

    hipStream_t st = static_cast<hipStream_t>(stream);
    const int64_t plane_elems = lstm_tile_elems(T, ndir, max_batch, P.G32), tail_elems = bwd_tail_elems(T, ndir, max_batch, H);
    float* const dgt = reinterpret_cast<float*>(flags);
    flags += plane_elems;
    float* const dbias = reinterpret_cast<float*>(flags);
    if (s_begin == 0 && !prefilled) {
        int fe = daf_fill_and_zero(dgt, (size_t)plane_elems, flags, (size_t)tail_elems, st);
        if (fe) return fe;
    } else if (s_begin == 0 && prefilled != 2) {
        hipError_t e = zero_words_async(flags, (size_t)tail_elems, st);
        if (e != hipSuccess) return (int)e;
    }
    flags += ndir * 4 * H;
    uint32_t* const dg_amax = flags;
    flags += 8;
    const int nt16 = (max_batch + 15) / 16;
    LstmPersistBwdArgs A{gates, c, dhy, w_hh_t, dgates, batch_sizes_dev, offsets_dev, flags, T, H, ndir,
                         (unsigned)P.nx, (unsigned)env_int("PTMI_LSTM_MAX_POLLS", 1 << 22), (int)dg_bytes,
                         (unsigned)(ptmi_lstm_flags_elems(T, ndir, max_batch) - 8), 0, P.ntiles, env_int("PTMI_LSTM_DBG", 0), c0, max_batch,
                         0, 0, 0, dgt, nt16, dbias, dg_amax, P.G32};
    A.err_sink = error_sink();
    A.uniform = uniform ? 1 : 0;
    A.masks = reinterpret_cast<const unsigned long long*>(step_masks);
    A.dcn = dc_n;
    A.s_begin = s_begin;
    A.s_end = s_end;
    A.dc_carry = dc_carry;
    if (dgates_t) {
        const int64_t range_rows = (int64_t)(s_end - s_begin) * max_batch;
        A.dgtp = reinterpret_cast<uint4*>(dgates_t);
        A.tp_kb = (int)((range_rows + 31) / 32);
        A.tp_dir_stride = (long long)(4 * H / 16) * A.tp_kb * 2 * 64;
        A.tp_row0[0] = (long long)(T - s_end) * max_batch;
        A.tp_row0[1] = (long long)s_begin * max_batch;
        if (range_rows % 32 != 0) {
            const long long tiles = (long long)ndir * (4 * H / 16);
            hipLaunchKernelGGL(zero_tp_tail_kernel, dim3((unsigned)((tiles * 64 + 255) / 256)), dim3(256), 0, st, A.dgtp, tiles, A.tp_kb);
            int rc = launch_status();
            if (rc) return rc;
        }
    }
    for (int t0 = 0; t0 < P.ntiles; t0 += P.per_launch) {
        A.tile0 = t0;
        A.nx = P.nx;
        A.nt = std::min(P.per_launch, P.ntiles - t0);
        const int chains = A.nt * ndir;
        A.span = (chains <= 8 && 8 % chains == 0) ? 8 / chains : 0;
        const unsigned nwg = A.span ? (unsigned)((P.nx + A.span - 1) / A.span * 8) : (unsigned)(P.nx * chains);
        int rc = launch_bwd_split(A, P.mtl, nwg, st);
        if (rc) return rc;
    }
// ... 5 lines not shown
```

padertorch_amd/csrc/lstm_common.h:

```cpp
#pragma once
#include "common.h"

namespace ptmi {

typedef float f32x4 __attribute__((ext_vector_type(4)));

__device__ __forceinline__ float sigmoidf_(float x) {
    return __builtin_amdgcn_rcpf(1.f + __builtin_amdgcn_exp2f(-1.4426950408889634f * x));
}
__device__ __forceinline__ float tanhf_(float x) {
    const float t = __builtin_amdgcn_exp2f(-2.8853900817779268f * fabsf(x));
    return copysignf((1.f - t) * __builtin_amdgcn_rcpf(1.f + t), x);
}

struct LstmPersistArgs {
    float* gx;
    float* hy;
    float* c;
    const float* w;
    const int32_t* bs;
    const int64_t* offs;
    unsigned* flags;
    int T, H, KP, ndir;
    unsigned expected;
    unsigned max_polls;
    int hy_bytes;
    unsigned err_off;
    int dbg;
    int tile0, ntiles;
    const float* c0;
    int max_batch;
    float* hyt;
    int nt16;
    const unsigned* w_amax;
    int KP32;
    unsigned* err_sink = nullptr;
    int nx = 0, nt = 0, span = 0;
    int uniform = 0;
    uint4* fill_ptr = nullptr;
    unsigned long long fill_n16 = 0;
    unsigned long long zero_n16 = 0;
    const unsigned long long* masks = nullptr;
};

constexpr int kSlots = 128;

struct LstmPersistBwdArgs {
    const float* gates;
    const float* c;
    const float* dhy;
    const float* wt;
    float* dg;
    const int32_t* bs;
    const int64_t* offs;
    unsigned* flags;
    int T, H, ndir;
    unsigned expected;
    unsigned max_polls;
    int dg_bytes;
    unsigned err_off;
    int tile0, ntiles;
    int dbg;
    const float* c0;
    int max_batch;
    int nx, nt, span;
    float* dgt;
    int nt16;
    float* dbias;
    unsigned* dg_amax;
    int G32;
    unsigned* err_sink = nullptr;
    int s_begin = 0, s_end = -1;
    float* dc_carry = nullptr;
    int uniform = 0;
    uint4* dgtp = nullptr;
    long long tp_dir_stride = 0;
    int tp_kb = 0;
    long long tp_row0[2] = {0, 0};
    const unsigned long long* masks = nullptr;
    const float* dcn = nullptr;
};

__device__ __forceinline__ bool chain_tile(int nx, int nt, int span, int* x, int* y, int* dir, int nchains = 1 << 30) {
    const int L = blockIdx.x;
    int chain;
    if (span > 0) {
        const int xcd = L & 7;
        chain = xcd / span;
        *x = (L >> 3) * span + (xcd - chain * span);
        if (*x >= nx || chain >= nchains) return false;
    } else {
        *x = L % nx;
        chain = L / nx;
    }
    *y = chain % nt;
    *dir = chain / nt;
    return true;
}


bool fwd_split_instantiated(int jt, int mtl);
int daf_fill_and_zero(void* p, size_t words, void* z, size_t zero_words, hipStream_t st);
int launch_fwd_split(const LstmPersistArgs& A, int jt, int mtl, dim3 grid, hipStream_t st);
int launch_bwd_split(const LstmPersistBwdArgs& A, int mtl, unsigned nwg, hipStream_t st);

}
```

padertorch_amd/csrc/lstm_split.hip:

```cpp
#include <stdlib.h>

#include <algorithm>

#include "lstm_common.h"

namespace ptmi {

typedef _Float16 h16x8 __attribute__((ext_vector_type(8)));
typedef __bf16 b16x8 __attribute__((ext_vector_type(8)));
typedef _Float16 h16x2 __attribute__((ext_vector_type(2)));
typedef __bf16 b16x2 __attribute__((ext_vector_type(2)));

__device__ __forceinline__ int handoff_index(int col, int plane, int row) {
    return (((col >> 5) * 2 + plane) * 64 + ((col & 31) >> 3) * 16 + row) * 8 + (col & 7);
}

constexpr unsigned kFill = 0xffffffffu;
typedef unsigned short us2 __attribute__((ext_vector_type(2)));
__device__ __forceinline__ unsigned fold_max16(const uint4 v, unsigned m) {
    us2 x = __builtin_elementwise_max(__builtin_bit_cast(us2, v.x), __builtin_bit_cast(us2, v.y));
    x = __builtin_elementwise_max(x, __builtin_bit_cast(us2, v.z));
    x = __builtin_elementwise_max(x, __builtin_bit_cast(us2, v.w));
    return __builtin_bit_cast(unsigned, __builtin_elementwise_max(x, __builtin_bit_cast(us2, m)));
}
__device__ __forceinline__ bool has_fill(unsigned m) { return (m & 0xffffu) == 0xffffu || (m >> 16) == 0xffffu; }

template <class T>
__device__ __forceinline__ T ld_const(const T* p, int idx) {
    typedef const __attribute__((address_space(4))) T* cptr;
    return reinterpret_cast<cptr>(reinterpret_cast<unsigned long long>(p))[idx];
}
__device__ __forceinline__ unsigned long long ld_const64(const unsigned long long* p, int idx) { return ld_const(p, idx); }

struct DafHold {
    unsigned hold, failed;
    unsigned long long ref;
    __device__ __forceinline__ void mark() { ref = __builtin_amdgcn_s_memrealtime(); }
    __device__ __forceinline__ void wait() const {
        while ((unsigned)(__builtin_amdgcn_s_memrealtime() - ref) < hold) __builtin_amdgcn_s_sleep(1);
    }
    __device__ __forceinline__ void update(bool first_clean, int step, bool adapt) {
        if (!adapt) return;
        if (!first_clean) {
            hold = min(hold + 3u, 1000u);
            failed = 1u;
        }
        if ((step & 63) == 63) {
            if (!failed && hold > 0u) --hold;
            failed = 0u;
        }
    }
};

__global__ void fill_and_zero_kernel(uint4* p, size_t n16, unsigned word, unsigned* z, size_t nz) {
    const uint4 v = make_uint4(word, word, word, word);
    const size_t i0 = (size_t)blockIdx.x * blockDim.x + threadIdx.x, step = (size_t)gridDim.x * blockDim.x;
    for (size_t i = i0; i < n16; i += step) p[i] = v;
    for (size_t i = i0; i < nz; i += step) z[i] = 0u;
}

int daf_fill_and_zero(void* p, size_t words, void* z, size_t zero_words, hipStream_t st) {
    const size_t n16 = words / 4;
    const unsigned grid = (unsigned)std::min<size_t>((std::max(n16, zero_words) + 255) / 256, 8192);
    hipLaunchKernelGGL(fill_and_zero_kernel, dim3(grid), dim3(256), 0, st, static_cast<uint4*>(p), n16, kFill, static_cast<unsigned*>(z), zero_words);
    return launch_status();
}

constexpr float kHScale = 1024.f;

__device__ __forceinline__ float pow2_scale(const unsigned* amax_bits) {
    if (!amax_bits) return 1.f;
    const unsigned e = (*amax_bits >> 23) & 0xffu;
    if (e == 0u || e == 0xffu) return 1.f;
    return __uint_as_float((unsigned)(127 + 13 + 127 - (int)e) << 23);
}

template <bool BF16>
__device__ __forceinline__ void split1(float v, unsigned* hi, unsigned* lo) {
    if (BF16) {
        const __bf16 h = (__bf16)v;
        const __bf16 l = (__bf16)(v - (float)h);
        *hi = __builtin_bit_cast(unsigned short, h);
        *lo = __builtin_bit_cast(unsigned short, l);
    } else {
        const _Float16 h = (_Float16)v;
        const _Float16 l = (_Float16)(v - (float)h);
        *hi = __builtin_bit_cast(unsigned short, h);
        *lo = __builtin_bit_cast(unsigned short, l);
    }
}

template <bool BF16>
__device__ __forceinline__ void split8(const float (&v)[8], uint4* hi, uint4* lo) {
    unsigned h[8], l[8];
#pragma unroll
    for (int e = 0; e < 8; ++e) split1<BF16>(v[e], &h[e], &l[e]);
    *hi = make_uint4(h[0] | (h[1] << 16), h[2] | (h[3] << 16), h[4] | (h[5] << 16), h[6] | (h[7] << 16));
    *lo = make_uint4(l[0] | (l[1] << 16), l[2] | (l[3] << 16), l[4] | (l[5] << 16), l[6] | (l[7] << 16));
}

template <bool BF16>
__device__ __forceinline__ f32x4 mma16(const uint4 a, const uint4 b, const f32x4 c) {
    if (BF16) return __builtin_amdgcn_mfma_f32_16x16x32_bf16(__builtin_bit_cast(b16x8, a), __builtin_bit_cast(b16x8, b), c, 0, 0, 0);
    return __builtin_amdgcn_mfma_f32_16x16x32_f16(__builtin_bit_cast(h16x8, a), __builtin_bit_cast(h16x8, b), c, 0, 0, 0);
}

template <bool BF16>
__device__ __forceinline__ unsigned pair_word(float v, int lane, int* plane) {
    unsigned hi, lo;
    split1<BF16>(v, &hi, &lo);
    const bool odd = lane & 1;
    const unsigned send = odd ? hi : lo;
    const unsigned recv = (unsigned)__builtin_amdgcn_mov_dpp((int)send, 0xB1, 0xF, 0xF, true);
    *plane = odd ? 1 : 0;
    return odd ? (recv | (lo << 16)) : (hi | (recv << 16));
}

#ifdef PTMI_LSTM_ABLATE
constexpr bool ABL = true;
#else
constexpr bool ABL = false;
#endif

template <int JT, int NW, int CB, int MTL, int RED_PAD = 4>
__global__ __launch_bounds__(NW * 64, 2) void lstm_fwd_daf_kernel(const LstmPersistArgs A) {
    constexpr int NC = 4 * JT;
    constexpr int NT = NC / 16;
    constexpr int MR = 16 * MTL;
    constexpr int ACTW = (MR * JT + 63) / 64;
    int bx = blockIdx.x, bz = blockIdx.z, dir = blockIdx.y;
    if (A.span > 0 && !chain_tile(A.nx, A.nt, A.span, &bx, &bz, &dir, A.ndir * A.nt)) return;
    const unsigned wg_lin = A.span > 0 ? (unsigned)((dir * A.nt + bz) * A.nx + bx)
                                       : (blockIdx.z * gridDim.y + blockIdx.y) * gridDim.x + blockIdx.x;
    const unsigned wg_cnt = A.span > 0 ? (unsigned)(A.ndir * A.nt * A.nx) : gridDim.x * gridDim.y * gridDim.z;
    const int j0 = bx * JT;
    const int m0 = (A.tile0 + bz) * MR;
    const int H = A.H, G = 4 * H;
    const long long ld_g = (long long)A.ndir * G, ld_h = (long long)A.ndir * H;
    const int tid = threadIdx.x, lane = tid & 63, wave = tid >> 6;
    const int g4 = lane >> 4, r = lane & 15;
    __shared__ float red[2][NW][MR][NC + RED_PAD];
    const bool uniform = A.uniform != 0;
    auto bs_at = [&](int t) { return uniform ? A.max_batch : ld_const(A.bs, t); };
    auto offs_at = [&](int t) { return uniform ? (long long)t * A.max_batch : (long long)ld_const(A.offs, t); };
    const bool masked = A.masks != nullptr;
    typedef unsigned long long u64;
    auto alive_at = [&](int t) -> u64 { return masked ? ld_const64(A.masks, 3 * t) : ~0ull; };
// ... 607 lines not shown
```

padertorch_amd/csrc/pit_loss.hip:

```cpp
#include "reduce.h"

namespace ptmi {

constexpr int kTChunk = 8;
constexpr int kMaxK = 8;

struct PitArgs {
    const float* est;
    const float* obs;
    const float* tgt;
    const float* scl;
    const int32_t* row_frames;
    long long t_len;
    long long est_bs, est_ts, obs_bs, obs_ts, tgt_bs, tgt_ts;
    int K, F, nvar, nchunks;
};

template <int K>
__global__ __launch_bounds__(256) void pit_pairwise_kernel(const PitArgs A, double* __restrict__ partial) {
    const int b = blockIdx.x / A.nchunks;
    const int c = blockIdx.x - b * A.nchunks;
    const long long T_b = A.row_frames ? (long long)A.row_frames[b] : A.t_len;
    const long long t0 = (long long)c * kTChunk;
    long long t1 = t0 + kTChunk;
// ... 25 lines not shown
            h[i] = A.scl ? g[i] * A.scl[toff + i * F] : 0.f;
        }
#pragma unroll
        for (int i = 0; i < K; ++i)
#pragma unroll
            for (int j = 0; j < K; ++j) {
                const float d0 = e[i] - g[j];
                acc[0][i][j] += d0 * d0;
                const float d1 = e[i] - h[j];
                acc[1][i][j] += d1 * d1;
            }
    }

    __shared__ float red[4][2 * K * K];
    const int lane = threadIdx.x & 63, wave = threadIdx.x >> 6;
#pragma unroll
    for (int v = 0; v < 2; ++v)
#pragma unroll
        for (int i = 0; i < K; ++i)
#pragma unroll
            for (int j = 0; j < K; ++j) {
                const float s = wave_sum(acc[v][i][j]);
                if (lane == 0) red[wave][(v * K + i) * K + j] = s;
            }
    __syncthreads();
    if (threadIdx.x < nvar * K * K) {
        const double s = (double)red[0][threadIdx.x] + (double)red[1][threadIdx.x] +
                         (double)red[2][threadIdx.x] + (double)red[3][threadIdx.x];
        partial[((long long)b * A.nchunks + c) * (nvar * K * K) + threadIdx.x] = s;
    }
}

__global__ __launch_bounds__(256) void pit_pairwise_generic_kernel(const PitArgs A, double* __restrict__ partial) {
    const int K = A.K, F = A.F;
    const int b = blockIdx.x / A.nchunks;
    const int c = blockIdx.x - b * A.nchunks;
    const int i = blockIdx.y / K, j = blockIdx.y - i * K;
    const long long T_b = A.row_frames ? (long long)A.row_frames[b] : A.t_len;
    const long long t0 = (long long)c * kTChunk;
    long long t1 = t0 + kTChunk;
    if (t1 > T_b) t1 = T_b;
    float a0 = 0.f, a1 = 0.f;
    const long long n = (t1 > t0) ? (t1 - t0) * F : 0;
    for (long long idx = threadIdx.x; idx < n; idx += 256) {
        const long long tt = idx / F;
        const int f = (int)(idx - tt * F);
        const long long t = t0 + tt;
        const float o = A.obs ? A.obs[b * A.obs_bs + t * A.obs_ts + f] : 1.f;
        const float e = A.est[b * A.est_bs + t * A.est_ts + (long long)i * F + f] * o;
        const long long off = b * A.tgt_bs + t * A.tgt_ts + (long long)j * F + f;
        const float g = A.tgt[off];
        const float h = A.scl ? g * A.scl[off] : 0.f;
        a0 += (e - g) * (e - g);
        a1 += (e - h) * (e - h);
    }
    __shared__ float red[4][2];
    const int lane = threadIdx.x & 63, wave = threadIdx.x >> 6;
    a0 = wave_sum(a0);
    a1 = wave_sum(a1);
    if (lane == 0) {
        red[wave][0] = a0;
        red[wave][1] = a1;
    }
    __syncthreads();
    if (threadIdx.x < A.nvar) {
        const int v = threadIdx.x;
        const double s = (double)red[0][v] + (double)red[1][v] + (double)red[2][v] + (double)red[3][v];
        partial[((long long)b * A.nchunks + c) * (A.nvar * K * K) + (v * K + i) * K + j] = s;
    }
}

__global__ void pit_reduce_kernel(const double* __restrict__ partial, double* __restrict__ sse, int nchunks,
                                  int per, const int32_t* row_frames, long long t_len) {
    const int b = blockIdx.x;
    const long long T_b = row_frames ? (long long)row_frames[b] : t_len;
    const int used = (int)((T_b + kTChunk - 1) / kTChunk);
    for (int e = threadIdx.x; e < per; e += blockDim.x) {
        double s = 0.0;
        for (int c = 0; c < used && c < nchunks; ++c) s += partial[((long long)b * nchunks + c) * per + e];
        sse[(long long)b * per + e] = s;
    }
}

__global__ void pit_assign_kernel(const double* __restrict__ sse, int batch, int nvar, int K, int F,
                                  long long t_len, const int32_t* row_frames, float* __restrict__ loss,
                                  int32_t* __restrict__ perm_out, float* ex_loss, float* scratch) {
    const int total = batch * nvar;
    for (int id = threadIdx.x; id < total; id += blockDim.x) {
        const int b = id / nvar;
        const double* m = sse + (long long)id * K * K;
        const long long T_b = row_frames ? (long long)row_frames[b] : t_len;
        const double denom = (double)T_b * K * F;
        int p[kMaxK], best[kMaxK];
        for (int j = 0; j < K; ++j) p[j] = best[j] = j;
        float best_loss = 0.f;
        bool first = true;
        while (true) {
            double s = 0.0;
            for (int j = 0; j < K; ++j) s += m[p[j] * K + j];
            const float cand = (float)(s / denom);
            if (first || cand < best_loss) {
                best_loss = cand;
                for (int j = 0; j < K; ++j) best[j] = p[j];
                first = false;
            }
            int i = K - 2;
            while (i >= 0 && p[i] > p[i + 1]) --i;
            if (i < 0) break;
            int j = K - 1;
            while (p[j] < p[i]) --j;
            int tmp = p[i]; p[i] = p[j]; p[j] = tmp;
            for (int lo = i + 1, hi = K - 1; lo < hi; ++lo, --hi) { tmp = p[lo]; p[lo] = p[hi]; p[hi] = tmp; }
        }
        for (int j = 0; j < K; ++j) perm_out[(long long)id * K + j] = best[j];
        scratch[id] = best_loss;
        if (ex_loss) ex_loss[id] = best_loss;
    }
    __syncthreads();
    if ((int)threadIdx.x < nvar) {
        double s = 0.0;
        for (int b = 0; b < batch; ++b) s += (double)scratch[b * nvar + threadIdx.x];
        loss[threadIdx.x] = (float)(s / batch);
    }
}

struct PitBwdArgs {
    const float* est;
    const float* obs;
    const float* tgt;
    const float* scl;
    const int32_t* perm;
    const float* gscale;
    const int32_t* row_frames;
    float* grad;
    long long batch, t_len;
    long long est_bs, est_ts, obs_bs, obs_ts, tgt_bs, tgt_ts;
    int K, F, nvar, nchunks;
};

__global__ __launch_bounds__(256) void pit_backward_kernel(const PitBwdArgs A) {
    const int b = blockIdx.x / A.nchunks;
    const int c = blockIdx.x - b * A.nchunks;
    const int K = A.K, F = A.F;
    const long long T_b = A.row_frames ? (long long)A.row_frames[b] : A.t_len;
    const long long t0 = (long long)c * kTChunk;
    long long t1 = t0 + kTChunk;
    if (t1 > A.t_len) t1 = A.t_len;
    __shared__ int inv[2][32];
    __shared__ float coef[2];
    if (threadIdx.x < A.nvar * K) {
        const int v = threadIdx.x / K, j = threadIdx.x - v * K;
        inv[v][A.perm[((long long)b * A.nvar + v) * K + j]] = j;
    }
    if (threadIdx.x < A.nvar)
        coef[threadIdx.x] = T_b > 0 ? A.gscale[threadIdx.x] * (float)(2.0 / ((double)A.batch * T_b * K * F)) : 0.f;
    __syncthreads();
    const long long n = (t1 > t0) ? (t1 - t0) * K * F : 0;
    for (long long idx = threadIdx.x; idx < n; idx += 256) {
        const long long tk = idx / F;
        const int f = (int)(idx - tk * F);
        const long long tt = tk / K;
        const int i = (int)(tk - tt * K);
        const long long t = t0 + tt;
        const long long eoff = b * A.est_bs + t * A.est_ts + (long long)i * F + f;
        float gval = 0.f;
        if (t < T_b) {
            const float o = A.obs ? A.obs[b * A.obs_bs + t * A.obs_ts + f] : 1.f;
            const float e = A.est[eoff] * o;
            for (int v = 0; v < A.nvar; ++v) {
                const long long off = b * A.tgt_bs + t * A.tgt_ts + (long long)inv[v][i] * F + f;
                float g = A.tgt[off];
                if (v == 1) g *= A.scl[off];
                gval += coef[v] * (e - g);
            }
            gval *= o;
        }
        A.grad[eoff] = gval;
    }
}

}

using namespace ptmi;

extern "C" {

int64_t ptmi_pit_workspace_elems(int64_t batch, int64_t t_len, int32_t K, int32_t F) {
    (void)F;
    const int64_t nchunks = (t_len + kTChunk - 1) / kTChunk;
    return batch * nchunks * 2 * K * K + batch * 2;
}

int ptmi_pit_pairwise_sse(const float* est, const float* obs, const float* tgt, const float* tgt_scale,
                          int64_t batch, int64_t t_len, const int64_t* strides, int32_t K, int32_t F,
                          const int32_t* row_frames, double* workspace, double* sse,
                          ptmi_stream_t stream) {
    PTMI_RETURN_IF(!est || !tgt || !workspace || !sse || !strides, PTMI_E_INVALID);
    PTMI_RETURN_IF(batch < 0 || t_len < 0 || K < 1 || F < 1, PTMI_E_INVALID);
    if (batch == 0) return PTMI_OK;
    hipStream_t st = static_cast<hipStream_t>(stream);
    PitArgs A{};
    A.est = est;
    A.obs = obs;
    A.tgt = tgt;
    A.scl = tgt_scale;
    A.row_frames = row_frames;
    A.t_len = t_len;
    A.est_bs = strides[0]; A.est_ts = strides[1];
    A.obs_bs = strides[2]; A.obs_ts = strides[3];
    A.tgt_bs = strides[4]; A.tgt_ts = strides[5];
    A.K = K;
    A.F = F;
    A.nvar = tgt_scale ? 2 : 1;
    A.nchunks = (int)((t_len + kTChunk - 1) / kTChunk);
    const int per = A.nvar * K * K;
    if (A.nchunks > 0) {
        const long long blocks = (long long)batch * A.nchunks;
        PTMI_RETURN_IF(blocks > 0x7fffffffLL, PTMI_E_UNSUPPORTED);
        switch (K) {
            case 1: hipLaunchKernelGGL(pit_pairwise_kernel<1>, dim3((unsigned)blocks), dim3(256), 0, st, A, workspace); break;
            case 2: hipLaunchKernelGGL(pit_pairwise_kernel<2>, dim3((unsigned)blocks), dim3(256), 0, st, A, workspace); break;
            case 3: hipLaunchKernelGGL(pit_pairwise_kernel<3>, dim3((unsigned)blocks), dim3(256), 0, st, A, workspace); break;
            case 4: hipLaunchKernelGGL(pit_pairwise_kernel<4>, dim3((unsigned)blocks), dim3(256), 0, st, A, workspace); break;
            default:
                PTMI_RETURN_IF(K * K > 65535, PTMI_E_UNSUPPORTED);
                hipLaunchKernelGGL(pit_pairwise_generic_kernel, dim3((unsigned)blocks, (unsigned)(K * K)), dim3(256), 0, st, A, workspace);
        }
        int rc = launch_status();
        if (rc) return rc;
    }
    hipLaunchKernelGGL(pit_reduce_kernel, dim3((unsigned)batch), dim3(64), 0, st, workspace, sse, A.nchunks, per,
                       row_frames, (long long)t_len);
    return launch_status();
}

int ptmi_pit_assign(const double* sse, int64_t batch, int32_t nvar, int32_t K, int32_t F, int64_t t_len,
                    const int32_t* row_frames, float* loss, int32_t* perm, float* ex_loss,
                    ptmi_stream_t stream) {
    PTMI_RETURN_IF(!sse || !loss || !perm, PTMI_E_INVALID);
    PTMI_RETURN_IF(batch < 1 || nvar < 1 || nvar > 2 || K < 1, PTMI_E_INVALID);
    PTMI_RETURN_IF(K > kMaxK, PTMI_E_UNSUPPORTED);
    hipStream_t st = static_cast<hipStream_t>(stream);
    float* scratch = ex_loss;
    if (!scratch) {
        hipError_t e = hipMallocAsync(reinterpret_cast<void**>(&scratch), sizeof(float) * batch * nvar, st);
        if (e != hipSuccess) return (int)e;
    }
    hipLaunchKernelGGL(pit_assign_kernel, dim3(1), dim3(256), 0, st, sse, (int)batch, (int)nvar, (int)K, (int)F,
                       (long long)t_len, row_frames, loss, perm, ex_loss, scratch);
    int rc = launch_status();
    if (!ex_loss) (void)hipFreeAsync(scratch, st);
    return rc;
}

int ptmi_pit_backward(const float* est, const float* obs, const float* tgt, const float* tgt_scale,
                      const int32_t* perm, const float* gscale, int64_t batch, int64_t t_len,
                      const int64_t* strides, int32_t K, int32_t F, int32_t nvar, const int32_t* row_frames,
                      float* grad, ptmi_stream_t stream) {
    PTMI_RETURN_IF(!est || !tgt || !perm || !gscale || !grad || !strides, PTMI_E_INVALID);
    PTMI_RETURN_IF(nvar < 1 || nvar > 2 || (nvar == 2 && !tgt_scale) || K < 1 || K > 32, PTMI_E_INVALID);
    if (batch == 0 || t_len == 0) return PTMI_OK;
    PitBwdArgs A{};
    A.est = est;
    A.obs = obs;
    A.tgt = tgt;
    A.scl = tgt_scale;
    A.perm = perm;
    A.gscale = gscale;
    A.row_frames = row_frames;
    A.grad = grad;
    A.batch = batch;
    A.t_len = t_len;
    A.est_bs = strides[0]; A.est_ts = strides[1];
    A.obs_bs = strides[2]; A.obs_ts = strides[3];
    A.tgt_bs = strides[4]; A.tgt_ts = strides[5];
    A.K = K;
    A.F = F;
    A.nvar = nvar;
    A.nchunks = (int)((t_len + kTChunk - 1) / kTChunk);
    const long long blocks = (long long)batch * A.nchunks;
    PTMI_RETURN_IF(blocks > 0x7fffffffLL, PTMI_E_UNSUPPORTED);
    hipLaunchKernelGGL(pit_backward_kernel, dim3((unsigned)blocks), dim3(256), 0, static_cast<hipStream_t>(stream), A);
    return launch_status();
}

}
```

padertorch_amd/ops/library.py:

```python
import ctypes
from typing import List, Optional, Tuple

import torch
from torch import Tensor

from .. import _lib

_LIBRARY = torch.library.Library('ptmi', 'DEF')


def _register(schema):
    name = schema.split('(', 1)[0].strip()

    def deco(fn):
        _LIBRARY.define(schema)
        _LIBRARY.impl(name, fn, 'CUDA')
        return getattr(torch.ops.ptmi, name)
    return deco


def _geom(g: List[int]):
    return _lib.StftGeom(*[int(v) for v in g])


@_register('stft_forward(Tensor x, Tensor? row_samples, Tensor window, Tensor twiddle, int[] geom, int frames, int layout, '
           'float edge_scale, str timer) -> Tensor')
def stft_forward(x, row_samples, window, twiddle, geom, frames, layout, edge_scale, timer):
    lib = _lib.load()
    rows, T = x.shape
    F = geom[0] // 2 + 1
    shape = (rows, frames, F, 2) if layout == 0 else (rows, frames, 2 * F)
    out = torch.empty(shape, dtype=torch.float32, device=x.device)
    g = _geom(geom)
    args = (x.data_ptr(), rows, x.stride(0), T, _lib.ptr(row_samples), window.data_ptr(), twiddle.data_ptr(), g, frames,
            layout, edge_scale, out.data_ptr(), _lib.stream(x.device))
    rc = _lib.timed(timer, lib.ptmi_stft_forward, *args) if timer else lib.ptmi_stft_forward(*args)
    _lib.check(rc, 'ptmi_stft_forward')
    return out


@_register('istft_forward(Tensor spec, Tensor window, Tensor twiddle, int[] geom, int layout, float edge_scale, int cut_left, '
           'int out_samples, str timer) -> Tensor')
def istft_forward(spec, window, twiddle, geom, layout, edge_scale, cut_left, out_samples, timer):
    lib = _lib.load()
    rows, frames = spec.shape[0], spec.shape[1]
    out = torch.empty((rows, max(out_samples, 0)), dtype=torch.float32, device=spec.device)
    if out_samples > 0:
        args = (spec.data_ptr(), rows, frames, None, window.data_ptr(), twiddle.data_ptr(), _geom(geom), layout, edge_scale,
                cut_left, out_samples, out_samples, out.data_ptr(), _lib.stream(spec.device))
        rc = _lib.timed(timer, lib.ptmi_istft_forward, *args) if timer else lib.ptmi_istft_forward(*args)
        _lib.check(rc, 'ptmi_istft_forward')
    return out


@_register('pit_features(Tensor y, Tensor? s, Tensor? num_samples, Tensor window, Tensor twiddle, int[] geom, int frames) '
           '-> (Tensor, Tensor?, Tensor?)')
def pit_features(y, s, num_samples, window, twiddle, geom, frames):
    return _pit_features(y, s, num_samples, window, twiddle, geom, frames, None, None, None)


@_register('pit_features_packed(Tensor y, Tensor? s, Tensor? num_samples, Tensor window, Tensor twiddle, int[] geom, int frames, '
           'Tensor(a!) log1p_packed, Tensor(b!)? log1p_planes, Tensor? packed_offsets) -> (Tensor, Tensor?, Tensor?)')
def pit_features_packed(y, s, num_samples, window, twiddle, geom, frames, log1p_packed, log1p_planes, packed_offsets):
    return _pit_features(y, s, num_samples, window, twiddle, geom, frames, log1p_packed, log1p_planes, packed_offsets)


def _pit_features(y, s, num_samples, window, twiddle, geom, frames, log1p_packed, log1p_planes, packed_offsets):
    lib = _lib.load()
    B, N = y.shape
    K = s.shape[1] if s is not None else 0
    F = geom[0] // 2 + 1
    dev = y.device
    Y_abs = torch.empty((B, frames, F), dtype=torch.float32, device=dev)
    X_abs = cos_pd = None
    if K:
        X_abs = torch.empty((B, frames, K, F), dtype=torch.float32, device=dev)
        cos_pd = torch.empty((B, frames, K, F), dtype=torch.float32, device=dev)
    rc = _lib.timed('pit_features', lib.ptmi_pit_features_packed, y.data_ptr(), _lib.ptr(s), B, K, N, N, _lib.ptr(num_samples),
                    window.data_ptr(), twiddle.data_ptr(), _geom(geom), frames, Y_abs.data_ptr(), _lib.ptr(X_abs),
                    _lib.ptr(cos_pd), _lib.ptr(log1p_packed), _lib.ptr(log1p_planes), _lib.ptr(packed_offsets), _lib.stream(dev))
    if rc == -2:
        raise NotImplementedError(f'pit_features: STFT size {geom[0]} / window {geom[2]} beyond what the direct-DFT kernel stages in LDS')
    _lib.check(rc, 'ptmi_pit_features')
    return Y_abs, X_abs, cos_pd


@_register('pit_loss_forward(Tensor est, Tensor? obs, Tensor tgt, Tensor? scale, Tensor? row_frames, int B, int T, int K, int F, '
           'int[] strides) -> (Tensor, Tensor, Tensor, Tensor)')
def pit_loss_forward(est, obs, tgt, scale, row_frames, B, T, K, F, strides):
    lib = _lib.load()
    dev = est.device
    nvar = 2 if scale is not None else 1
    ws = torch.empty(int(lib.ptmi_pit_workspace_elems(B, T, K, F)), dtype=torch.float64, device=dev)
    sse = torch.empty((B, nvar, K, K), dtype=torch.float64, device=dev)
    st = _lib.stream(dev)
    _lib.check(_lib.timed('pit_pairwise_sse', lib.ptmi_pit_pairwise_sse, est.data_ptr(), _lib.ptr(obs), tgt.data_ptr(),
                          _lib.ptr(scale), B, T, _lib.strides6(*strides), K, F, _lib.ptr(row_frames), ws.data_ptr(),
                          sse.data_ptr(), st), 'ptmi_pit_pairwise_sse')
    loss = torch.empty(nvar, dtype=torch.float32, device=dev)
    perm = torch.empty((B, nvar, K), dtype=torch.int32, device=dev)
    ex_loss = torch.empty((B, nvar), dtype=torch.float32, device=dev)
    _lib.check(lib.ptmi_pit_assign(sse.data_ptr(), B, nvar, K, F, T, _lib.ptr(row_frames), loss.data_ptr(), perm.data_ptr(),
                                   ex_loss.data_ptr(), st), 'ptmi_pit_assign')
    return loss, perm, ex_loss, sse


@_register('pit_loss_backward(Tensor est, Tensor? obs, Tensor tgt, Tensor? scale, Tensor perm, Tensor g_loss, Tensor? row_frames, '
           'int B, int T, int K, int F, int[] strides) -> Tensor')
def pit_loss_backward(est, obs, tgt, scale, perm, g_loss, row_frames, B, T, K, F, strides):
    lib = _lib.load()
    nvar = 2 if scale is not None else 1
    grad = torch.empty_strided(est.shape, est.stride(), dtype=est.dtype, device=est.device)
    _lib.check(_lib.timed('pit_backward', lib.ptmi_pit_backward, est.data_ptr(), _lib.ptr(obs), tgt.data_ptr(), _lib.ptr(scale),
                          perm.data_ptr(), g_loss.data_ptr(), B, T, _lib.strides6(*strides), K, F, nvar, _lib.ptr(row_frames),
                          grad.data_ptr(), _lib.stream(est.device)), 'ptmi_pit_backward')
    return grad


@_register('dc_loss_forward(Tensor x, Tensor t, Tensor? row_frames, int B, int T, int E, int K, int F, int[] strides) '
           '-> (Tensor, Tensor, Tensor)')
def dc_loss_forward(x, t, row_frames, B, T, E, K, F, strides):
    lib = _lib.load()
    dev = x.device
    ws = torch.empty(int(lib.ptmi_dc_workspace_elems(B, T, F)), dtype=torch.float32, device=dev)
    gram = torch.empty((B, 32, 32), dtype=torch.float64, device=dev)
    ex_loss = torch.empty(B, dtype=torch.float32, device=dev)
    loss = torch.empty(1, dtype=torch.float32, device=dev)
    _lib.check(_lib.timed('dc_loss_forward', lib.ptmi_dc_loss_forward, x.data_ptr(), t.data_ptr(), B, T, _lib.strides8(*strides),
                          E, K, F, _lib.ptr(row_frames), ws.data_ptr(), gram.data_ptr(), ex_loss.data_ptr(), loss.data_ptr(),
                          _lib.stream(dev)), 'ptmi_dc_loss_forward')
    return loss, ex_loss, gram


@_register('dc_loss_backward(Tensor x, Tensor t, Tensor gram, Tensor g_loss, Tensor? row_frames, int B, int T, int E, int K, int F, '
           'int[] strides, bool zero_fill) -> Tensor')
def dc_loss_backward(x, t, gram, g_loss, row_frames, B, T, E, K, F, strides, zero_fill):
    lib = _lib.load()
    dx = torch.zeros_like(x, memory_format=torch.preserve_format) if zero_fill \
        else torch.empty_strided(x.shape, x.stride(), dtype=x.dtype, device=x.device)
    _lib.check(_lib.timed('dc_loss_backward', lib.ptmi_dc_loss_backward, x.data_ptr(), t.data_ptr(), gram.data_ptr(),
                          g_loss.data_ptr(), B, T, _lib.strides8(*strides), E, K, F, _lib.ptr(row_frames), dx.data_ptr(),
                          _lib.stream(x.device)), 'ptmi_dc_loss_backward')
    return dx


def _tas_dims(feat, weight):
    B, N, E = feat.shape
    assert weight.shape[0] == N and weight.is_contiguous() and feat.is_contiguous(), (feat.shape, weight.shape)
    return B, N, E, weight.numel() // N


@_register('tas_analysis(Tensor x, Tensor weight, Tensor? bias, int stride, int frames, bool relu) -> Tensor')
def tas_analysis(x, weight, bias, stride, frames, relu):
    B, T = x.shape
    N = weight.shape[0]
    L = weight.numel() // N
    assert x.is_contiguous() and weight.is_contiguous()
    out = torch.empty((B, N, frames), dtype=torch.float32, device=x.device)
    _lib.check(_lib.timed('tas_analysis', _lib.load().ptmi_tas_analysis, x.data_ptr(), weight.data_ptr(), _lib.ptr(bias), out.data_ptr(),
                          B, T, N, L, stride, frames, int(relu), _lib.stream(x.device)), 'ptmi_tas_analysis')
    return out


@_register('tas_synthesis(Tensor p, Tensor? mask, Tensor? gate, Tensor weight, Tensor? bias, int stride, int samples) -> Tensor')
def tas_synthesis(p, mask, gate, weight, bias, stride, samples):
    B, N, E, L = _tas_dims(p, weight)
    K = 1
    if mask is not None:
        K = mask.shape[0]
        assert mask.shape == (K, B, N, E) and mask.is_contiguous(), mask.shape
    assert gate is None or (gate.shape == p.shape and gate.is_contiguous())
    y = torch.empty((B, samples) if mask is None else (K, B, samples), dtype=torch.float32, device=p.device)
    _lib.check(_lib.timed('tas_synthesis', _lib.load().ptmi_tas_synthesis, p.data_ptr(), _lib.ptr(mask), _lib.ptr(gate), weight.data_ptr(),
                          _lib.ptr(bias), y.data_ptr(), K, B, N, L, stride, E, samples, _lib.stream(p.device)), 'ptmi_tas_synthesis')
    return y


@_register('tas_masked_decode_backward(Tensor gy, Tensor mask, Tensor encoded, Tensor weight, int stride) -> (Tensor, Tensor)')
def tas_masked_decode_backward(gy, mask, encoded, weight, stride):
    B, N, E, L = _tas_dims(encoded, weight)
    K, _, T = gy.shape
    assert mask.shape == (K, B, N, E) and gy.shape[1] == B and mask.is_contiguous() and gy.is_contiguous(), (mask.shape, gy.shape)
    dmask, denc = torch.empty_like(mask), torch.empty_like(encoded)
    _lib.check(_lib.timed('tas_masked_decode_backward', _lib.load().ptmi_tas_masked_decode_backward, gy.data_ptr(), mask.data_ptr(),
# ... 653 lines not shown


@_register('gemm_planes_bf16_(Tensor(a!) out, Tensor a, int a_offset, Tensor b, Tensor? bias, int M, int N, int K, bool accumulate, '
           'int split_k) -> ()')
def gemm_planes_bf16_(out, a, a_offset, b, bias, M, N, K, accumulate, split_k):
    _gemm_planes_call('ptmi_gemm_planes_bf16', 'gemm_planes_bf16', out, M, N, K, split_k,
                      (a.data_ptr() + a_offset, b.data_ptr(), _lib.ptr(bias), out.data_ptr(), max(out.stride(0), N), M, N, K, int(accumulate)))


@_register('gemm_planes_bf16_two_(Tensor(a!) out, Tensor(b!) out2, Tensor a, int a_offset, Tensor b, int M, int N, int K, bool accumulate, '
           'int split_k) -> ()')
def gemm_planes_bf16_two_(out, out2, a, a_offset, b, M, N, K, accumulate, split_k):
    assert out.shape[0] + out2.shape[0] == M and out.shape[1] == out2.shape[1] == N and out.stride(0) == out2.stride(0), (out.shape, out2.shape)
    _gemm_planes_call('ptmi_gemm_planes_bf16_two', 'gemm_planes_bf16', out, M, N, K, split_k,
                      (a.data_ptr() + a_offset, b.data_ptr(), out.data_ptr(), out2.data_ptr(), out.shape[0], max(out.stride(0), N), M, N, K,
                       int(accumulate)))


@_register('pack_planes_bf16_list(Tensor[] xs) -> Tensor[]')
def pack_planes_bf16_list(xs):
    lib = _lib.load()
    n, k = len(xs), xs[0].shape[0]
    assert 1 <= n <= 3 and all(x.dim() == 2 and x.shape[0] == k and x.dtype == torch.float32 and (x.stride(1) == 1 or x.shape[1] == 1)
                               for x in xs), [tuple(x.shape) for x in xs]
    outs = [torch.empty(int(lib.ptmi_planes_elems(x.shape[1], k)), dtype=torch.bfloat16, device=x.device) for x in xs]
    src = (ctypes.c_void_p * n)(*[x.data_ptr() for x in xs])
    dst = (ctypes.c_void_p * n)(*[o.data_ptr() for o in outs])
    cols = (ctypes.c_int64 * n)(*[x.shape[1] for x in xs])
    ld = (ctypes.c_int64 * n)(*[_ld(x) for x in xs])
    _lib.check(_lib.timed(f'pack_planes_bf16_list:{k}x{sum(x.shape[1] for x in xs)}', lib.ptmi_pack_planes_t_bf16_list, src, cols, ld, dst, n,
                          k, _lib.stream(xs[0].device)), 'ptmi_pack_planes_t_bf16_list')
    return outs


@_register('gemm_planes_bf16_group_(Tensor(a!)[] outs, int[] blocks, Tensor a, int a_offset, int M, int m_split, Tensor[] bs, int[] ns, '
           'int K, bool accumulate, int split_k) -> bool')
def gemm_planes_bf16_group_(outs, blocks, a, a_offset, M, m_split, bs, ns, K, accumulate, split_k):
    lib = _lib.load()
    S = len(bs)
    assert len(outs) == len(blocks) and len(ns) == S and len(set(blocks)) == len(blocks), (len(outs), blocks, ns)
    c = (ctypes.c_void_p * (2 * S))()
    ldc = (ctypes.c_int64 * (2 * S))()
    for o, blk in zip(outs, blocks):
        p, s = divmod(int(blk), S)
        assert p in (0, 1) and o.dtype == torch.float32 and o.shape == ((M - m_split) if p else m_split, ns[s]) and o.stride(1) == 1, \
            (blk, o.shape, o.stride())
        c[blk] = o.data_ptr()
        ldc[blk] = max(o.stride(0), ns[s])
    n = (ctypes.c_int32 * S)(*[int(v) for v in ns])
    b = (ctypes.c_void_p * S)(*[t.data_ptr() for t in bs])
    if int(lib.ptmi_gemm_planes_group_plan(M, m_split, n, S, c, K, split_k)) // 100 == 5:
        return False
    ws = torch.empty(int(lib.ptmi_gemm_planes_group_workspace_elems(M, m_split, n, S, c, K, split_k)), dtype=torch.float32, device=a.device)
    shape = f'{M}/{m_split}x{"+".join(str(int(v)) for v in ns)}x{K}'
    rc = _lib.timed(f'gemm_group_bf16:{shape}:{split_k}', lib.ptmi_gemm_planes_bf16_group, a.data_ptr() + a_offset, M, m_split, b, n, S, c,
                    ldc, K, int(accumulate), split_k, _products(), ws.data_ptr(), _lib.stream(a.device))
    if rc == -2:
        return False
    _lib.check(rc, 'ptmi_gemm_planes_bf16_group')
    return True


@_register('unit_norm_forward(Tensor x, float eps) -> (Tensor, Tensor)')
def unit_norm_forward(x, eps):
    N, E, F = x.shape
    y = torch.empty_like(x)
    inv = torch.empty((N, F), dtype=torch.float32, device=x.device)
    _lib.check(_lib.timed('unit_norm_forward', _lib.load().ptmi_unit_norm_forward, _lib.ptr(x), _lib.ptr(y), _lib.ptr(inv),
                          N, E, F, eps, _lib.stream(x.device)), 'ptmi_unit_norm_forward')
    return y, inv


@_register('unit_norm_backward(Tensor gy, Tensor y, Tensor inv, float eps) -> Tensor')
def unit_norm_backward(gy, y, inv, eps):
    N, E, F = y.shape
    dx = torch.empty_like(y)
    _lib.check(_lib.timed('unit_norm_backward', _lib.load().ptmi_unit_norm_backward, _lib.ptr(gy), _lib.ptr(y), _lib.ptr(inv),
                          _lib.ptr(dx), N, E, F, eps, _lib.stream(y.device)), 'ptmi_unit_norm_backward')
    return dx


@_register('lstm_recurrence_forward(Tensor(a!) gates, Tensor(b!) hy, Tensor? c0, Tensor w_hh_pad, Tensor? w_amax, Tensor bs_dev, '
           'Tensor offs_dev, int bs_host, int offs_host, int T, int max_batch, int rows, int H, int KP, int ndir, bool persistent, '
           'Tensor(c!)? scratch=None, bool prefilled=False, Tensor(d!)? backward_scratch=None, Tensor? step_masks=None) -> (Tensor, Tensor?)')
def lstm_recurrence_forward(gates, hy, c0, w_hh_pad, w_amax, bs_dev, offs_dev, bs_host, offs_host, T, max_batch, rows, H, KP, ndir,
                            persistent, scratch=None, prefilled=False, backward_scratch=None, step_masks=None):
    lib = _lib.load()
    dev = gates.device
    st = _lib.stream(dev)
    c = (torch.zeros if step_masks is not None else torch.empty)((rows, ndir * H), dtype=torch.float32, device=dev)
    rc = -2
    flags = None
    if persistent:
        n = int(lib.ptmi_lstm_scratch_elems(T, ndir, max_batch, H, 0))
        flags = scratch if scratch is not None else torch.empty(n, dtype=torch.int32, device=dev)
        assert flags.numel() >= n and flags.dtype == torch.int32
        assert step_masks is None or (step_masks.dtype == torch.int64 and step_masks.numel() == 3 * T)
        rc = _lib.timed('lstm_forward', lib.ptmi_lstm_forward_persistent, gates.data_ptr(), hy.data_ptr(), c.data_ptr(),
                        _lib.ptr(c0), w_hh_pad.data_ptr(), _lib.ptr(w_amax), bs_dev.data_ptr(), offs_dev.data_ptr(),
                        _lib.ptr(step_masks), flags.data_ptr(), T, max_batch, rows, H, KP, ndir,
                        int(bool(prefilled and scratch is not None)), _lib.ptr(backward_scratch), st)
        if rc != -2 or step_masks is not None:
            _lib.check(rc, 'ptmi_lstm_forward_persistent')
    if rc == -2:
        flags = None
        _lib.check(_lib.timed('lstm_forward', lib.ptmi_lstm_forward, gates.data_ptr(), hy.data_ptr(), c.data_ptr(), _lib.ptr(c0),
                              w_hh_pad.data_ptr(), ctypes.c_void_p(bs_host), ctypes.c_void_p(offs_host), T, max_batch, H, KP, ndir,
                              st), 'ptmi_lstm_forward')
    return c, flags


@_register('lstm_recurrence_backward(Tensor gates, Tensor c, Tensor? c0, Tensor dhy, Tensor w_hh_t, Tensor bs_dev, Tensor offs_dev, '
           'int bs_host, int offs_host, int T, int max_batch, int rows, int H, int ndir, bool persistent, Tensor(a!)? scratch=None, '
           'int prefilled=0, Tensor? step_masks=None) -> (Tensor, Tensor?)')
def lstm_recurrence_backward(gates, c, c0, dhy, w_hh_t, bs_dev, offs_dev, bs_host, offs_host, T, max_batch, rows, H, ndir, persistent,
                             scratch=None, prefilled=0, step_masks=None):
    lib = _lib.load()
    dev = gates.device
    dg = torch.empty_like(gates)
    flags = None
    if persistent:
        n = int(lib.ptmi_lstm_scratch_elems(T, ndir, max_batch, H, 1))
        flags = scratch if scratch is not None else torch.empty(n, dtype=torch.int32, device=dev)
        assert flags.numel() >= n and flags.dtype == torch.int32
        persistent = _lstm_backward_persistent(gates, c, c0, dhy, w_hh_t, dg, None, flags, None, bs_dev, offs_dev, T, max_batch, rows, H,
                                               ndir, 0, T, int(prefilled) if scratch is not None else 0, step_masks=step_masks)
        if not persistent and step_masks is not None:
            _lib.check(-2, 'ptmi_lstm_backward_persistent')
    if not persistent:
        flags = None
        dcs = torch.empty((max_batch, ndir, H), dtype=torch.float32, device=dev)
        _lib.check(_lib.timed('lstm_backward', lib.ptmi_lstm_backward, gates.data_ptr(), c.data_ptr(), _lib.ptr(c0), dhy.data_ptr(),
                              w_hh_t.data_ptr(), dg.data_ptr(), dcs.data_ptr(), ctypes.c_void_p(bs_host), ctypes.c_void_p(offs_host),
                              T, max_batch, H, ndir, _lib.stream(dev)), 'ptmi_lstm_backward')
    return dg, flags


def _i32c(*tensors):
    for t in tensors:
        assert t is None or (t.is_contiguous() and t.dtype == torch.int32 and t.is_cuda), (t.shape, t.stride(), t.dtype, t.device)


@_register('dprnn_tables(Tensor like, Tensor? lengths, int B, int S, int K, int P) -> (Tensor, Tensor, Tensor)')
def dprnn_tables(like, lengths, B, S, K, P):
    lengths, is64 = _lengths(lengths, B)
    dev = like.device
    chunks = torch.empty(B, dtype=torch.int32, device=dev)
    intra = torch.empty((B * S, 3), dtype=torch.int32, device=dev)
    inter = torch.empty((B * K, 3), dtype=torch.int32, device=dev)
    _lib.check(_lib.timed('dprnn_tables', _lib.load().ptmi_dprnn_tables, _lib.ptr(lengths), is64, B, S, K, P, chunks.data_ptr(),
                          intra.data_ptr(), inter.data_ptr(), _lib.stream(dev)), 'ptmi_dprnn_tables')
    return chunks, intra, inter


def _chunk_lstm_dims(gates, table, H):
    _f32c(gates)
    _i32c(table)
    assert gates.dim() == 2 and table.dim() == 2 and table.shape[1] == 3 and gates.shape[1] % (4 * H) == 0, (gates.shape, table.shape, H)
    ndir = gates.shape[1] // (4 * H)
    assert ndir in (1, 2), gates.shape
    return gates.shape[0], ndir


@_register('chunk_lstm_forward(Tensor(a!) gates, Tensor w_hh, Tensor? w_hh_reverse, Tensor b_hh, Tensor? b_hh_reverse, Tensor table, '
           'int cap, int H) -> (Tensor, Tensor)')
def chunk_lstm_forward(gates, w_hh, w_hh_reverse, b_hh, b_hh_reverse, table, cap, H):
    rows, ndir = _chunk_lstm_dims(gates, table, H)
    _f32c(w_hh, w_hh_reverse, b_hh, b_hh_reverse)
    assert w_hh.shape == (4 * H, H) and b_hh.shape == (4 * H,) and (ndir == 1 or (w_hh_reverse.shape == (4 * H, H)
                                                                                  and b_hh_reverse.shape == (4 * H,)))
    h = torch.empty((rows, ndir * H), dtype=torch.float32, device=gates.device)
    c = torch.empty((rows, ndir * H), dtype=torch.float32, device=gates.device)
    _lib.check(_lib.timed(f'chunk_lstm_forward:{table.shape[0]}x{cap}x{H}', _lib.load().ptmi_chunk_lstm_forward, gates.data_ptr(),
                          w_hh.data_ptr(), _lib.ptr(w_hh_reverse), b_hh.data_ptr(), _lib.ptr(b_hh_reverse), h.data_ptr(), c.data_ptr(),
                          table.data_ptr(), table.shape[0], cap, H, ndir, _lib.stream(gates.device)), 'ptmi_chunk_lstm_forward')
    return h, c


@_register('chunk_lstm_backward(Tensor(a!) gates, Tensor dh, Tensor w_hh, Tensor? w_hh_reverse, Tensor h, Tensor c, Tensor table, '
           'int cap, int H) -> Tensor')
def chunk_lstm_backward(gates, dh, w_hh, w_hh_reverse, h, c, table, cap, H):
    rows, ndir = _chunk_lstm_dims(gates, table, H)
    _f32c(dh, w_hh, w_hh_reverse, h, c)
    assert dh.shape == h.shape == c.shape == (rows, ndir * H), (dh.shape, h.shape, c.shape)
    hprev = torch.empty_like(h)
    _lib.check(_lib.timed(f'chunk_lstm_backward:{table.shape[0]}x{cap}x{H}', _lib.load().ptmi_chunk_lstm_backward, gates.data_ptr(),
                          dh.data_ptr(), w_hh.data_ptr(), _lib.ptr(w_hh_reverse), h.data_ptr(), c.data_ptr(), hprev.data_ptr(),
                          table.data_ptr(), table.shape[0], cap, H, ndir, _lib.stream(gates.device)), 'ptmi_chunk_lstm_backward')
# ... 157 lines not shown
```

padertorch_amd/ops/lstm.py:

```python
import types

import torch
from torch.nn.utils.rnn import PackedSequence

from .. import _lib
from . import capture as _capture
from . import context as _context
from . import gemm as _gemm
from . import library
from . import lstm_forms as _forms
from . import watchdog as _watchdog
from . import wgrad as _wgrad
from .lstm_forms import begin_captured_step, end_captured_step
from .pack_meta import _PackMeta, _meta, pack_meta
from .watchdog import check_errors, error_count, error_word, errors_since_last_report, raise_timeout
from .wgrad import flush_pending as flush_pending_wgrad, gemm_keys_safe, sync_deferred, warm_side_stream, wgrad_key

__all__ = ['packed_lstm']


PERSISTENT = True
CHECK_PERSISTENT_ERRORS = False
DEFER_WGRAD = False
GRAD_READY_HOOK = None
# ... 101 lines not shown
def _backward_planes(lib, meta, plan, job, saved, scratch_b, pre_b, ndir, G, H):
    device, chunks, T = saved[3].device, plan.chunks, meta.T
    flags, pre = _backward_scratch(lib, meta, scratch_b, pre_b, ndir, H, device)
    cuts = [T * i // chunks for i in range(chunks + 1)]
    carry = torch.empty((ndir, meta.max_batch, H), dtype=torch.float32, device=device) if chunks > 1 else None
    ok, dg_t, part_t = _launch_planes_range(lib, meta, saved, flags, carry, pre, plan.masks, ndir, G, H, cuts[0], cuts[1])
    if not ok:
        return None
    for i in range(1, chunks):
        done = torch.cuda.Event()
        done.record(plan.main)
        finished, finished_part = dg_t, part_t
        ok, dg_t, part_t = _launch_planes_range(lib, meta, saved, flags, carry, pre, plan.masks, ndir, G, H, cuts[i], cuts[i + 1])
        if not ok:
            raise RuntimeError('ptmi_lstm_backward_persistent: a later range was refused')
        plan.side.wait_event(done)
        job.rows(None, finished_part, None, dg_t=finished)
        finished.record_stream(plan.side)
    return None, dg_t, flags, carry, part_t


def _backward_ranges(lib, meta, plan, job, saved, scratch_b, pre_b, ndir, G, H, dcn):
    gates, c, c0, dhy, w_t = saved
    chunks, T = plan.chunks, meta.T
    dg = torch.empty_like(gates)
    flags, pre = _backward_scratch(lib, meta, scratch_b, pre_b, ndir, H, dhy.device)
    carry = torch.empty((ndir, meta.max_batch, H), dtype=torch.float32, device=dhy.device)
    cuts = [T * i // chunks for i in range(chunks + 1)]
    amax_word = _scratch_tail(lib, flags, meta, ndir, G)[1]
    offs = [int(v) for v in meta.offs_host[:T]] + [meta.rows]
    todo = [(0, meta.rows)] * ndir
    for i in range(chunks):
        if i:
            snap = amax_word.clone()
            done = torch.cuda.Event()
            done.record(plan.main)
            plan.side.wait_event(done)
            s0, s1 = cuts[i - 1], cuts[i]
            job.rows(dg, [(offs[T - s1], offs[T - s0]), (offs[s0], offs[s1])][:ndir], snap)
            snap.record_stream(plan.side)
        ok = torch.ops.ptmi.lstm_recurrence_backward_range(
            gates, c, c0, dhy, w_t, dg, flags, carry, meta.bs_dev, meta.offs_dev, T, meta.max_batch, meta.rows, H,
            ndir, cuts[i], cuts[i + 1], pre, dcn)
        if not ok:
            if i:
                raise RuntimeError('ptmi_lstm_backward_persistent: a later range was refused')
            if plan.state_grad:
                raise NotImplementedError('gradients w.r.t. the initial LSTM state: this configuration cannot run on the '
                                          'persistent kernels')
            return None
    if chunks > 1:
        s0 = cuts[chunks - 1]
        todo = [(offs[0], offs[T - s0]), (offs[s0], offs[T])][:ndir]
    return dg, None, flags, carry, todo


def _backward_one_call(meta, plan, saved, scratch_b, pre_b, ndir, H):
    gates, c, c0, dhy, w_t = saved
    dg, flags = torch.ops.ptmi.lstm_recurrence_backward(
        gates, c, c0, dhy, w_t, meta.bs_dev, meta.offs_dev, meta.bs_host.ctypes.data, meta.offs_host.ctypes.data,
        meta.T, meta.max_batch, meta.rows, H, ndir, PERSISTENT, scratch_b, int(pre_b), plan.masks)
    return dg, None, flags, None, [(0, meta.rows)] * ndir


def _input_grad(ctx, lib, plan, dg, flags, amax_dg, amax_kernel, w_ih, ndir, H):
    meta, gm, params = ctx.meta, ctx.gemm, ctx.params
    if not ctx.needs_input_grad[0]:
        return None
    if gm is None:
        return dg @ w_ih
    cols = plan.cols_dx if (flags is not None and amax_kernel is not None) else 0
    if cols and _gemm.planes_enabled() and plan.uniform_rows:
        pdx = ctx.forms.w_ih_planes_dx if ctx.forms is not None else None
        wplanes = pdx[0] if (pdx is not None and pdx[1] == cols) else _gemm.stacked_planes_t_bf16(
            w_ih, ndir, cols, None if params is None else [ps[0] for ps in params])
        dx = torch.empty((meta.rows, w_ih.shape[1]), dtype=torch.float32, device=flags.device)
        torch.ops.ptmi.gemm_planes_bf16_(dx, flags, 0, wplanes, None, meta.rows, w_ih.shape[1], ndir * cols, False,
                                         _gemm.auto_split_k(meta.rows, w_ih.shape[1], ndir * cols))
        return dx
    return _gemm.mm(dg, w_ih, amax_x=amax_dg, amax_y=gm[1])


GROUP_WGRAD = True


class _WgradJob:

    def __init__(self, ctx, lib, plan, x, hy, h0, ndir, H):
        self.lib, self.plan, self.meta, self.gm, self.params, self.oc = lib, plan, ctx.meta, ctx.gemm, ctx.params, ctx.oc
        self.x, self.hy, self.h0, self.ext, self.ndir, self.H, self.G = x, hy, h0, ctx.ext, ndir, H, 4 * H
        self.first_layer = not ctx.needs_input_grad[0]
        self.operands, self.xplanes, self.dgplanes, self.group = None, {}, {}, {}

    def rows(self, dg, ranges, amax_dg, both_queues=False, dg_t=None):
        lib, gm, params, x, h0, ndir, H, G = self.lib, self.gm, self.params, self.x, self.h0, self.ndir, self.H, self.G
        main, side, xplanes = self.plan.main, self.plan.side, self.xplanes
        if self._grouped(dg_t, ranges):
            r0, r1 = ranges[0]
            with torch.cuda.stream(main if both_queues else side):
                if self.operands is None:
                    self.operands = _recurrent_operands(self.meta, dg, self.hy, self.ext, h0, ndir, H)
                px, pf, pb = torch.ops.ptmi.pack_planes_bf16_list([x[r0:r1], self.operands[0][1][r0:r1], self.operands[1][1][r0:r1]])
                ok = torch.ops.ptmi.gemm_planes_bf16_group_(
                    [params[0][0].grad, params[0][1].grad, params[1][0].grad, params[1][1].grad], self.GROUP_BLOCKS, dg_t, 0, 2 * G, G,
                    [px, pf, pb], [x.shape[1], H, H], r1 - r0, True, _gemm.auto_split_k(G, H, r1 - r0))
                assert ok, 'ptmi_gemm_planes_bf16_group refused a call its plan had accepted'
            return
        fused_ih = False
        if (dg_t is not None and ndir == 2 and ranges[0] == ranges[1] and ranges[0][1] > ranges[0][0]):
            ga, gb = params[0][0].grad, params[1][0].grad
            if ga.stride() == gb.stride() and (ga.data_ptr() ^ gb.data_ptr()) & 15 == 0 and ga.is_contiguous():
                r0, r1 = ranges[0]
                with torch.cuda.stream(main if both_queues else side):
                    key = (r0, r1)
                    if key not in xplanes:
                        xplanes[key] = torch.ops.ptmi.pack_planes_bf16(x[r0:r1], True)
                    torch.ops.ptmi.gemm_planes_bf16_two_(ga, gb, dg_t, 0, xplanes[key], 2 * G, x.shape[1], r1 - r0, True,
                                                         _gemm.auto_split_k(2 * G, x.shape[1], r1 - r0))
                fused_ih = True
        for d, ((p_wih, p_whh, _, _), (r0, r1)) in enumerate(zip(params, ranges)):
            q_ih = main if both_queues else side
            q_hh = main if both_queues and d == 1 else side
            with torch.cuda.stream(q_ih):
                if self.operands is None:
                    self.operands = _recurrent_operands(self.meta, dg, self.hy, self.ext, h0, ndir, H)
                dgd, h_prev = self.operands[d]
                if r1 <= r0:
                    continue
                if dg_t is not None:
                    k = r1 - r0
                    key = (r0, r1)
                    a_off = d * int(lib.ptmi_planes_elems(G, k)) * 2
                    if key not in xplanes and not fused_ih:
                        xplanes[key] = torch.ops.ptmi.pack_planes_bf16(x[r0:r1], True)
                    if not fused_ih:
                        torch.ops.ptmi.gemm_planes_bf16_(p_wih.grad, dg_t, a_off, xplanes[key], None, G, x.shape[1], k, True,
                                                         _gemm.auto_split_k(G, x.shape[1], k))
                    with torch.cuda.stream(q_hh):
                        hpl = torch.ops.ptmi.pack_planes_bf16(h_prev[r0:r1], True)
                        torch.ops.ptmi.gemm_planes_bf16_(p_whh.grad, dg_t, a_off, hpl, None, G, H, k, True, _gemm.auto_split_k(G, H, k))
                    continue
                dgt = dgd[r0:r1].t()
                if gm is not None and _gemm.planes_enabled():
                    k = r1 - r0
                    key = (r0, r1)
                    dgp = self.dgplanes.get((d, key))
                    if dgp is None:
                        dgp = _gemm.pack_t(dgd[r0:r1], amax_dg)
                    if key not in xplanes:
                        xplanes[key] = _gemm.pack_t(x[r0:r1], gm[0])
                    _gemm.mm_planes_(p_wih.grad, dgp, xplanes[key], G, x.shape[1], k, accumulate=True, split_k=_gemm.auto_split_k(G, x.shape[1], k))
                    with torch.cuda.stream(q_hh):
                        hpl = _gemm.pack_t(h_prev[r0:r1], _gemm.UNIT_RANGE if h0 is None else None)
                        _gemm.mm_planes_(p_whh.grad, dgp, hpl, G, H, k, accumulate=True, split_k=_gemm.auto_split_k(G, H, k))
                elif gm is not None:
                    _gemm.mm(dgt, x[r0:r1], out=p_wih.grad, accumulate=True, amax_x=amax_dg, amax_y=gm[0])
                    _gemm.mm(dgt, h_prev[r0:r1], out=p_whh.grad, accumulate=True, amax_x=amax_dg,
                             amax_y=_gemm.UNIT_RANGE if h0 is None else None)
                else:
                    p_wih.grad.addmm_(dgt, x[r0:r1])
                    p_whh.grad.addmm_(dgt, h_prev[r0:r1])

    GROUP_BLOCKS = [0, 1, 3, 5]

    def _grouped(self, dg_t, ranges):
        if not (GROUP_WGRAD and dg_t is not None and self.ndir == 2 and ranges[0] == ranges[1] and ranges[0][1] > ranges[0][0]):
# ... 25 lines not shown
        if _capture.ACTIVE and plan.use_side and not both and not self.first_layer:
            self.here = torch.cuda.Event()
            self.here.record(plan.main)
            _wgrad.defer(self.accumulate)
        else:
            self.accumulate()

    def accumulate(self, _start=None):
        plan, params, x, oc = self.plan, self.params, self.x, self.oc
        main, side, use_side, both = plan.main, plan.side, plan.use_side, self.both
        dg, dg_t, todo, amax_dg, db_kernel = self.dg, self.dg_t, self.todo, self.amax_dg, self.db_kernel
        if use_side:
            if self.here is not None:
                side.wait_event(self.here)
            else:
                side.wait_stream(main)
        else:
            main.wait_stream(_wgrad.stream(x.device))
        self.rows(dg, todo, amax_dg, both_queues=both, dg_t=dg_t)
        with torch.cuda.stream(side):
            if db_kernel is not None and all(ps[2].grad.is_contiguous() and ps[3].grad.is_contiguous() for ps in params):
                torch.ops.ptmi.lstm_bias_grad_add_(db_kernel, [ps[2].grad for ps in params], [ps[3].grad for ps in params])
            else:
                for d, (_, _, p_bih, p_bhh) in enumerate(params):
                    db_d = self.operands[d][0].sum(0) if db_kernel is None else db_kernel[d * self.G:(d + 1) * self.G]
                    p_bih.grad.add_(db_d)
                    p_bhh.grad.add_(db_d)
        done = None
        if use_side:
            done = torch.cuda.Event()
            done.record(side)
            _wgrad.mark_done([p for ps in params for p in ps[:2]], done)
        if both:
            main.wait_event(done)
            shared = self.dgplanes[(0, todo[0])][0] if dg_t is None else self.xplanes.get(todo[0])
            if shared is not None:
                shared.record_stream(side)
            if oc.grad_ready_hook is not None:
                side.wait_stream(main)
        if use_side:
            for t in (x, self.hy) + tuple(v for v in (dg, dg_t, self.h0, self.ext, db_kernel, amax_dg) if v is not None and torch.is_tensor(v)) \
                    + tuple(h_prev for _, h_prev in self.operands):
                t.record_stream(side)
        if oc.grad_ready_hook is not None:
            oc.grad_ready_hook([p for ps in params for p in ps])


class _LstmLayerFn(torch.autograd.Function):

    @staticmethod
    def forward(ctx, x, w_ih, bias, w_hh, meta, h0=None, c0=None, params=None, x_unit=False, anchor=None, forms=None, prev=None,
                handoff=None, top=False, oc=None):
        lib = _lib.load()
        ndir, G, H = w_hh.shape
        assert G == 4 * H
        KP = _forms.kpad_of(H)
        ctx.set_materialize_grads(False)
        stateful = h0 is not None or c0 is not None
        if stateful:
            h0 = torch.zeros_like(c0) if h0 is None else h0.detach().to(torch.float32).contiguous()
            c0 = torch.zeros_like(h0) if c0 is None else c0.detach().to(torch.float32).contiguous()
            assert h0.shape == c0.shape == (ndir, meta.max_batch, H), (h0.shape, c0.shape, meta.max_batch)
        scratch_b, pre_b = None, 0
        fills = int(lib.ptmi_lstm_forward_fills(meta.T, ndir, meta.max_batch, H)) if (
            PERSISTENT and x.is_cuda and any(ctx.needs_input_grad)) else 0
        if fills:
            scratch_b = torch.empty(int(lib.ptmi_lstm_scratch_elems(meta.T, ndir, meta.max_batch, H, 1)), dtype=torch.int32,
                                    device=x.device)
            pre_b = fills
        gates, x, ctx.gemm = _input_projection(x, w_ih, bias, meta, ndir, G, H, forms, prev, params, x_unit)
        if stateful:
            gv = gates.view(meta.rows, ndir, G)
            for d in range(ndir):
                gv[:, d].index_add_(0, meta.first_rows[d], h0[d] @ w_hh[d].t())
        if forms is not None:
            w_pad = forms.w_pad
        else:
            w_pad = torch.nn.functional.pad(w_hh, (0, KP - H)).contiguous() if KP != H else w_hh.contiguous()
        pad = meta.bs0 if meta.equal_lengths else 0
        masks = meta.masks_dev
        assert masks is None or not stateful, 'row-slot batches take no initial states'
        ext = (torch.zeros if masks is not None else torch.empty)((meta.rows + 2 * pad, ndir * H), dtype=torch.float32, device=x.device)
        hy = ext[pad:pad + meta.rows]
        if pad:
            C_ = ndir * H
            torch.as_strided(ext, (2, pad, C_), ((pad + meta.rows) * C_, C_, 1)).zero_()
            if stateful:
                ext[:pad].view(pad, ndir, H)[:, 0] = h0[0]
                if ndir > 1:
                    ext[pad + meta.rows:].view(pad, ndir, H)[:, 1] = h0[1]
        ctx.ext = ext if pad else None
        amax_whh = None
        if PERSISTENT and lib.ptmi_lstm_split_enabled():
            amax_whh = (_gemm.weights_absmax([ps[1] for ps in params]) if params is not None
                        else _gemm.absmax(w_pad.view(-1, KP)))
        if PERSISTENT:
            _watchdog.arm(x.device)
        c, flags = torch.ops.ptmi.lstm_recurrence_forward(
            gates, hy, c0, w_pad, amax_whh, meta.bs_dev, meta.offs_dev, meta.bs_host.ctypes.data, meta.offs_host.ctypes.data,
            meta.T, meta.max_batch, meta.rows, H, KP, ndir, PERSISTENT, None, False, scratch_b, masks)
        if flags is None:
            pre_b = 0
        if handoff is not None and flags is not None and not stateful and meta.uniform_rows:
            cols_out = int(lib.ptmi_lstm_handoff_cols(H, 0))
            if cols_out:
                handoff['planes'] = (flags, cols_out)
        ctx.scratch_b = (scratch_b, pre_b)
        if flags is not None and CHECK_PERSISTENT_ERRORS:
            check_errors()
        ctx.save_for_backward(x, w_ih, w_hh, gates, c, hy, h0, c0)
        ctx.meta = meta
        ctx.params = params
        ctx.forms = forms
        ctx.top = bool(top)
        ctx.oc = oc if oc is not None else _context.effective(None)
        if stateful:
            return hy, c
        return hy

    @staticmethod
    def backward(ctx, dhy, _dc=None):
        meta = ctx.meta
        if dhy is None:
            dhy = torch.zeros((meta.rows, ctx.saved_tensors[2].shape[0] * ctx.saved_tensors[2].shape[2]), dtype=torch.float32,
                              device=ctx.saved_tensors[0].device)
        lib = _lib.load()
        x, w_ih, w_hh, gates, c, hy, h0, c0 = ctx.saved_tensors
        scratch_b, pre_b = ctx.scratch_b
        ctx.scratch_b = (None, 0)
        ndir, G, H = w_hh.shape
        gm, params = ctx.gemm, ctx.params
        has_grads = params is not None and all(p.is_leaf and p.grad is not None for ps in params for p in ps)
        if ctx.forms is not None and not has_grads:
            raise RuntimeError('packed_lstm: the forward pass ran on the cached stacked weights (in-place weight gradients), '
                               'but a parameter of the layer has no .grad buffer any more')
        plan = _backward_plan(ctx, lib, x, h0, ndir, H, has_grads, _dc is not None)
        before_recurrence = None
        if _wgrad.pending() and dhy.is_cuda:
            before_recurrence = torch.cuda.Event()
            before_recurrence.record(torch.cuda.current_stream(dhy.device))
        job = _WgradJob(ctx, lib, plan, x, hy, h0, ndir, H)
        dhy = dhy.contiguous()
        w_t = ctx.forms.w_t if ctx.forms is not None else w_hh.transpose(1, 2).contiguous()
        if PERSISTENT:
            _watchdog.arm(dhy.device)
        dcn = None
        if _dc is not None and h0 is not None:
            dcv = _dc.reshape(meta.rows, ndir, H)
            dcn = torch.stack([dcv[meta.last_rows[d], d] for d in range(ndir)]).contiguous()
        if plan.state_grad and not (PERSISTENT and lib.ptmi_lstm_split_enabled()):
            raise NotImplementedError('gradients w.r.t. the LSTM states need the persistent split kernels')
        saved = (gates, c, c0, dhy, w_t)
        done = _backward_planes(lib, meta, plan, job, saved, scratch_b, pre_b, ndir, G, H) if plan.use_tp else None
        if done is None and (plan.chunks > 1 or plan.state_grad):
            done = _backward_ranges(lib, meta, plan, job, saved, scratch_b, pre_b, ndir, G, H, dcn)
        if done is None:
            done = _backward_one_call(meta, plan, saved, scratch_b, pre_b, ndir, H)
        dg, dg_t, flags, carry, todo = done
        db_kernel = amax_kernel = None
        if flags is not None:
            if CHECK_PERSISTENT_ERRORS:
                check_errors()
            db_kernel, word = _scratch_tail(lib, flags, meta, ndir, G)
            if lib.ptmi_lstm_split_enabled():
                amax_kernel = word
        flush_pending_wgrad(before_recurrence)
        amax_dg = None if gm is None else amax_kernel if (amax_kernel is not None or dg is None) else _gemm.absmax(dg)
        dx = _input_grad(ctx, lib, plan, dg, flags, amax_dg, amax_kernel, w_ih, ndir, H)
        gh0 = gc0 = None
        if plan.in_place:
            job.finish(dg, dg_t, todo, amax_dg, db_kernel)
            if plan.state_grad:
                gh0, gc0 = _state_grads(meta, dg, w_hh, carry, ndir, G, ctx.needs_input_grad)
            return (dx, None, None, None, None, gh0, gc0) + (None,) * 8
        db = dg.sum(0) if db_kernel is None else db_kernel
        if gm is not None:
            dw_ih = _gemm.mm(dg.t(), x, amax_x=amax_dg, amax_y=gm[0])
            dw_hh = torch.stack([_gemm.mm(a.t(), b, amax_x=amax_dg, amax_y=_gemm.UNIT_RANGE if h0 is None else None)
                                 for a, b in _recurrent_operands(meta, dg, hy, ctx.ext, h0, ndir, H)])
        else:
            dw_ih = dg.t() @ x
            dw_hh = torch.stack([a.t() @ b for a, b in _recurrent_operands(meta, dg, hy, ctx.ext, h0, ndir, H)])
        if plan.state_grad:
# ... 167 lines not shown
```

Measured before the change: 1.235 million frames/s.

## Fuse PIT partial reduction, fold LSTM pad zeroing into kernel, pair-store GEMM epilogues

Measured after the change: 1.238 million frames/s (median of 6 runs). No clear change (+0.3%).

```diff
diff --git a/include/ptmi.h b/include/ptmi.h
--- a/include/ptmi.h
+++ b/include/ptmi.h
@@ -61,6 +61,13 @@
 int ptmi_pit_assign(const double* sse, int64_t batch, int32_t nvar, int32_t K, int32_t F,
                     int64_t t_len, const int32_t* row_frames, float* loss, int32_t* perm,
                     float* ex_loss, ptmi_stream_t stream);
+
+int ptmi_pit_pairwise_partials(const float* est, const float* obs, const float* tgt, const float* tgt_scale,
+                               int64_t batch, int64_t t_len, const int64_t* strides, int32_t K, int32_t F,
+                               const int32_t* row_frames, double* workspace, ptmi_stream_t stream);
+int ptmi_pit_assign_chunks(const double* workspace, double* sse, int64_t batch, int32_t nvar, int32_t K,
+                           int32_t F, int64_t t_len, const int32_t* row_frames, float* loss, int32_t* perm,
+                           float* ex_loss, ptmi_stream_t stream);
 
 int ptmi_pit_backward(const float* est, const float* obs, const float* tgt, const float* tgt_scale,
                       const int32_t* perm, const float* gscale, int64_t batch, int64_t t_len,
@@ -100,6 +107,11 @@
                                  const uint64_t* step_masks, uint32_t* flags, int32_t T, int32_t max_batch, int64_t rows,
                                  int32_t H, int32_t KP, int32_t ndir, int32_t prefilled, uint32_t* backward_scratch,
                                  ptmi_stream_t stream);
+int ptmi_lstm_forward_persistent_padded(float* gates, float* ext, int64_t pad, float* c, const float* c0, const float* w_hh_pad,
+                                        const uint32_t* w_hh_amax, const int32_t* batch_sizes_dev, const int64_t* offsets_dev,
+                                        const uint64_t* step_masks, uint32_t* flags, int32_t T, int32_t max_batch, int64_t rows,
+                                        int32_t H, int32_t KP, int32_t ndir, int32_t prefilled, uint32_t* backward_scratch,
+                                        ptmi_stream_t stream);
 
 int ptmi_lstm_backward_persistent(const float* gates, const float* c, const float* c0, const float* dhy, const float* dc_n,
                                   const float* w_hh_t, float* dgates, uint16_t* dgates_t, const int32_t* batch_sizes_dev,
diff --git a/padertorch_amd/_lib.py b/padertorch_amd/_lib.py
--- a/padertorch_amd/_lib.py
+++ b/padertorch_amd/_lib.py
@@ -43,6 +43,8 @@
     'ptmi_pit_pairwise_sse': (c_int, [_P, _P, _P, _P, c_int64, c_int64, _I64P, c_int32, c_int32, _P,
                                       _P, _P, _P]),
     'ptmi_pit_assign': (c_int, [_P, c_int64, c_int32, c_int32, c_int32, c_int64, _P, _P, _P, _P, _P]),
+    'ptmi_pit_pairwise_partials': (c_int, [_P, _P, _P, _P, c_int64, c_int64, _I64P, c_int32, c_int32, _P, _P, _P]),
+    'ptmi_pit_assign_chunks': (c_int, [_P, _P, c_int64, c_int32, c_int32, c_int32, c_int64, _P, _P, _P, _P, _P]),
     'ptmi_pit_backward': (c_int, [_P, _P, _P, _P, _P, _P, c_int64, c_int64, _I64P, c_int32, c_int32,
                                   c_int32, _P, _P, _P]),
     'ptmi_dc_workspace_elems': (c_int64, [c_int64, c_int64, c_int32]),
@@ -134,6 +136,8 @@
     'ptmi_lstm_handoff_cols': (c_int32, [c_int32, c_int32]),
     'ptmi_lstm_forward_persistent': (c_int, [_P, _P, _P, _P, _P, _P, _P, _P, _P, _P, c_int32, c_int32, c_int64, c_int32, c_int32,
                                              c_int32, c_int32, _P, _P]),
+    'ptmi_lstm_forward_persistent_padded': (c_int, [_P, _P, c_int64, _P, _P, _P, _P, _P, _P, _P, _P, c_int32, c_int32, c_int64, c_int32,
+                                                    c_int32, c_int32, c_int32, _P, _P]),
     'ptmi_lstm_forward_fills': (c_int, [c_int32, c_int32, c_int32, c_int32]),
     'ptmi_lstm_backward_planes_ok': (c_int32, [c_int32, c_int32, c_int32, c_int64, c_int32]),
     'ptmi_lstm_backward_persistent': (c_int, [_P, _P, _P, _P, _P, _P, _P, _P, _P, _P, _P, _P, _P, c_int32, c_int32, c_int64, c_int32,
@@ -214,6 +218,14 @@
     return 0
 
 
+def select_gemm_pairs(on):
+    if on:
+        os.environ.pop('PTMI_GEMM_PAIRS', None)
+    else:
+        os.environ['PTMI_GEMM_PAIRS'] = '0'
+    return 0
+
+
 def check(rc, what=''):
     if rc != 0:
         msg = load().ptmi_error_string(int(rc)).decode()
diff --git a/padertorch_amd/csrc/gemm_planes.hip b/padertorch_amd/csrc/gemm_planes.hip
--- a/padertorch_amd/csrc/gemm_planes.hip
+++ b/padertorch_amd/csrc/gemm_planes.hip
@@ -7,6 +7,34 @@
 typedef _Float16 h8 __attribute__((ext_vector_type(8)));
 typedef __bf16 b8 __attribute__((ext_vector_type(8)));
 typedef float f4 __attribute__((ext_vector_type(4)));
+typedef float f2 __attribute__((ext_vector_type(2)));
+
+template <bool CHECK = true>
+__device__ __forceinline__ void store_pairs(float* o, const f4& v, int n, int N, bool add) {
+#pragma unroll
+    for (int p = 0; p < 2; ++p) {
+        const int c = n + 2 * p;
+        if (!CHECK || c + 1 < N) {
+            f2* o2 = reinterpret_cast<f2*>(o + 2 * p);
+            const f2 w = f2{v[2 * p], v[2 * p + 1]};
+            *o2 = add ? *o2 + w : w;
+        } else if (c < N) {
+            o[2 * p] = add ? o[2 * p] + v[2 * p] : v[2 * p];
+        }
+    }
+}
+
+__device__ __forceinline__ f4 bias_group(const float* bias, int n, int N, bool pairs) {
+    f4 b;
+    if (pairs && n + 3 < N) {
+        const f2 lo = *reinterpret_cast<const f2*>(bias + n), hi = *reinterpret_cast<const f2*>(bias + n + 2);
+        b = f4{lo[0], lo[1], hi[0], hi[1]};
+    } else {
+#pragma unroll
+        for (int e = 0; e < 4; ++e) b[e] = bias[min(n + e, N - 1)];
+    }
+    return b;
+}
 
 constexpr int PBM = 128, PBN = 128;
 constexpr int FR = 64;
@@ -35,6 +63,7 @@
     int m_split = 0;
     int relu = 0;
     unsigned* amax_out = nullptr;
+    int pairs = 0;
 };
 
 __device__ __forceinline__ void block_amax(unsigned* out, unsigned m, unsigned* red) {
@@ -125,12 +154,15 @@
     float* const Cz = slab ? G.workspace + (long long)blockIdx.z * G.M * G.N : G.C;
     const long long ldc = slab ? G.N : G.ldc;
     const bool vec = (ldc & 3) == 0 && ((reinterpret_cast<unsigned long long>(Cz) | reinterpret_cast<unsigned long long>(G.C2)) & 15) == 0;
+    const bool vec2 = G.pairs && !vec && (ldc & 1) == 0 &&
+                      ((reinterpret_cast<unsigned long long>(Cz) | reinterpret_cast<unsigned long long>(G.C2)) & 7) == 0;
     const bool add = G.accumulate && !slab;
     const int r = lane & 15, g = lane >> 4;
     f4 bv[4];
     {
         const bool bias_on = G.bias != nullptr && !slab;
         const bool bvec = (reinterpret_cast<unsigned long long>(G.bias) & 15) == 0;
+        const bool bvec2 = G.pairs && (reinterpret_cast<unsigned long long>(G.bias) & 7) == 0;
 #pragma unroll
         for (int j = 0; j < 4; ++j) {
             const int n = tn * PBN + wn * 64 + j * 16 + g * 4;
@@ -138,8 +170,7 @@
             if (bias_on && bvec && n + 3 < G.N) {
                 bv[j] = *reinterpret_cast<const f4*>(G.bias + n);
             } else if (bias_on) {
-#pragma unroll
-                for (int e = 0; e < 4; ++e) bv[j][e] = G.bias[min(n + e, G.N - 1)];
+                bv[j] = bias_group(G.bias, n, G.N, bvec2);
             }
         }
     }
@@ -166,6 +197,8 @@
             if (vec && n + 3 < G.N) {
                 f4* o4 = reinterpret_cast<f4*>(o);
                 *o4 = add ? *o4 + v : v;
+            } else if (vec2) {
+                store_pairs(o, v, n, G.N, add);
             } else {
 #pragma unroll
                 for (int e = 0; e < 4; ++e)
@@ -200,6 +233,7 @@
     int m_split = 0;
     int relu = 0;
     unsigned* amax_out = nullptr;
+    int pairs = 0;
 };
 
 constexpr int GROUP_SEGS = 3, GROUP_BLOCKS = 6;
@@ -390,14 +424,15 @@
             const int n0 = (tn * WN + wn) * NT * 16 + g * 4;
             const bool vec = (G.ldc & 3) == 0 && ((reinterpret_cast<unsigned long long>(G.C) | reinterpret_cast<unsigned long long>(G.C2)) & 15) == 0;
             const bool full = vec && (tn * WN + wn + 1) * NT * 16 <= G.N;
+            const bool vec2 = G.pairs && !vec && (G.ldc & 1) == 0 &&
+                              ((reinterpret_cast<unsigned long long>(G.C) | reinterpret_cast<unsigned long long>(G.C2)) & 7) == 0;
+            const bool full2 = vec2 && (tn * WN + wn + 1) * NT * 16 <= G.N;
+            const bool bvec2 = G.pairs && (reinterpret_cast<unsigned long long>(G.bias) & 7) == 0;
             f4 bv[NT];
 #pragma unroll
             for (int j = 0; j < NT; ++j) {
                 bv[j] = f4{0.f, 0.f, 0.f, 0.f};
-                if (G.bias) {
-#pragma unroll
-                    for (int e = 0; e < 4; ++e) bv[j][e] = G.bias[min(n0 + j * 16 + e, G.N - 1)];
-                }
+                if (G.bias) bv[j] = bias_group(G.bias, n0 + j * 16, G.N, bvec2);
             }
             const int mrow = (tm * WM + wm) * MT * 16 + r;
             if (GROUP || G.splits > 1) {
@@ -406,6 +441,7 @@
                                           : G.slabs + ((long long)tz * G.M + mrow) * G.N + n0;
                 const bool svec = (sN & 3) == 0 && (reinterpret_cast<unsigned long long>(G.slabs) & 15) == 0;
                 const bool sfull = svec && (tn * WN + wn + 1) * NT * 16 <= sN;
+                const bool svec2 = G.pairs && !svec && (sN & 1) == 0 && (reinterpret_cast<unsigned long long>(G.slabs) & 7) == 0;
 #pragma unroll
                 for (int i = 0; i < MT; ++i) {
                     const bool ok = mrow + i * 16 < sM;
@@ -416,6 +452,8 @@
                         float* o = srow + (long long)i * 16 * sN + j * 16;
                         if (sfull) {
                             if (ok) *reinterpret_cast<f4*>(o) = v;
+                        } else if (svec2) {
+                            if (ok) store_pairs(o, v, n0 + j * 16, sN, false);
                         } else {
 #pragma unroll
                             for (int e = 0; e < 4; ++e)
@@ -451,6 +489,10 @@
                         float* o = rowp(i) + j * 16;
                         if (full) {
                             if (ok) *reinterpret_cast<f4*>(o) = v;
+                        } else if (full2) {
+                            if (ok) store_pairs<false>(o, v, 0, 0, false);
+                        } else if (vec2) {
+                            if (ok) store_pairs(o, v, n0 + j * 16, G.N, false);
                         } else {
 #pragma unroll
                             for (int e = 0; e < 4; ++e)
@@ -483,6 +525,33 @@
                         if (ok) *reinterpret_cast<f4*>(rowp(i) + j * 16) = v;
                     }
                 }
+            } else if (full2 && !G.accumulate) {
+#pragma unroll
+                for (int i = 0; i < MT; ++i) {
+#pragma unroll
+                    for (int j = 0; j < NT; ++j) {
+                        const f4 v = acc[i][j] * inv + bv[j];
+                        acc[i][j] = f4{0.f, 0.f, 0.f, 0.f};
+                        if (mrow + i * 16 < G.M) store_pairs<false>(rowp(i) + j * 16, v, 0, 0, false);
+                    }
+                }
+            } else if (full2) {
+#pragma unroll
+                for (int i = 0; i < MT; ++i) {
+                    const bool ok = mrow + i * 16 < G.M;
+                    f2 old[NT][2];
+#pragma unroll
+                    for (int j = 0; j < NT; ++j)
+#pragma unroll
+                        for (int p = 0; p < 2; ++p)
+                            old[j][p] = ok ? *reinterpret_cast<const f2*>(rowp(i) + j * 16 + 2 * p) : f2{0.f, 0.f};
+#pragma unroll
+                    for (int j = 0; j < NT; ++j) {
+                        const f4 v = acc[i][j] * inv + bv[j] + f4{old[j][0][0], old[j][0][1], old[j][1][0], old[j][1][1]};
+                        acc[i][j] = f4{0.f, 0.f, 0.f, 0.f};
+                        if (ok) store_pairs<false>(rowp(i) + j * 16, v, 0, 0, false);
+                    }
+                }
             } else {
 #pragma unroll
                 for (int i = 0; i < MT; ++i) {
@@ -492,6 +561,10 @@
                         const f4 v = acc[i][j] * inv + bv[j];
                         acc[i][j] = f4{0.f, 0.f, 0.f, 0.f};
                         float* o = rowp(i) + j * 16;
+                        if (vec2) {
+                            if (ok) store_pairs(o, v, n0 + j * 16, G.N, G.accumulate != 0);
+                            continue;
+                        }
 #pragma unroll
                         for (int e = 0; e < 4; ++e)
                             if (ok && n0 + j * 16 + e < G.N) o[e] = G.accumulate ? o[e] + v[e] : v[e];
@@ -579,10 +652,26 @@
 __global__ __launch_bounds__(256) void planes_reduce_kernel(const float* __restrict__ ws, int splits, float* __restrict__ C, long long ldc,
                                                             const float* __restrict__ bias, int M, int N, int accumulate,
                                                             float* __restrict__ C2 = nullptr, int m_split = 0, int relu = 0,
-                                                            unsigned* __restrict__ amax_out = nullptr) {
+                                                            unsigned* __restrict__ amax_out = nullptr, int pairs = 0) {
     const long long total = (long long)M * N;
     unsigned mx = 0u;
-    for (long long i = blockIdx.x * 256ll + threadIdx.x; i < total; i += (long long)gridDim.x * 256) {
+    const bool bias2 = (reinterpret_cast<unsigned long long>(bias) & 7) == 0;
+    for (long long i = 2 * (blockIdx.x * 256ll + threadIdx.x); pairs && i < total; i += 2 * (long long)gridDim.x * 256) {
+        const int r = (int)(i / N), c = (int)(i - (long long)r * N);
+        f2 sum = f2{0.f, 0.f};
+        for (int z = 0; z < splits; ++z) sum += *reinterpret_cast<const f2*>(ws + (long long)z * total + i);
+        if (bias) sum += bias2 ? *reinterpret_cast<const f2*>(bias + c) : f2{bias[c], bias[c + 1]};
+        if (relu) {
+#pragma unroll
+            for (int e = 0; e < 2; ++e) {
+                sum[e] = sum[e] < 0.f ? 0.f : sum[e];
+                mx = max(mx, __float_as_uint(sum[e]));
+            }
+        }
+        f2* o = reinterpret_cast<f2*>((C2 != nullptr && r >= m_split) ? C2 + (long long)(r - m_split) * ldc + c : C + (long long)r * ldc + c);
+        *o = accumulate ? *o + sum : sum;
+    }
+    for (long long i = blockIdx.x * 256ll + threadIdx.x; !pairs && i < total; i += (long long)gridDim.x * 256) {
         const int r = (int)(i / N), c = (int)(i - (long long)r * N);
         float sum = 0.f;
         for (int z = 0; z < splits; ++z) sum += ws[(long long)z * total + i];
@@ -919,6 +1008,11 @@
     if (!v || !*v) return -1;
     const int t = atoi(v);
     return (t >= 0 && t <= 5) ? t : -1;
+}
+
+static int pair_epilogue() {
+    const char* v = getenv("PTMI_GEMM_PAIRS");
+    return (v && *v == '0') ? 0 : 1;
 }
 
 static int cu_count() {
@@ -1033,21 +1127,25 @@
             .bias = slabs ? nullptr : q.bias, .M = q.m, .N = q.n, .KB = p.KB, .ldc = q.ldc, .accumulate = (q.accumulate && !slabs) ? 1 : 0,
             .band = 4, .a_bytes = (unsigned)planes_bytes(q.m, p.KB), .b_bytes = (unsigned)planes_bytes(q.n, p.KB), .splits = p.splits,
             .kb_per_split = p.kb_per_split, .slabs = q.workspace, .C2 = q.c2, .m_split = q.m_split, .relu = slabs ? 0 : q.relu,
-            .amax_out = q.amax_out};
+            .amax_out = q.amax_out, .pairs = pair_epilogue()};
 }
 
 static PlanesArgs planes_args(const PlanesCall& q, const Plan& p) {
     return {.A = reinterpret_cast<const uint4*>(q.a), .B = reinterpret_cast<const uint4*>(q.b), .C = q.c, .workspace = q.workspace,
             .amax_a = q.amax_a, .amax_b = q.amax_b, .bias = q.bias, .M = q.m, .N = q.n, .KB = p.KB, .ldc = q.ldc,
             .accumulate = q.accumulate ? 1 : 0, .kb_per_split = p.kb_per_split, .tiles_m = (q.m + PBM - 1) / PBM, .tiles_n = (q.n + PBN - 1) / PBN,
-            .C2 = q.c2, .m_split = q.m_split, .relu = p.splits > 1 ? 0 : q.relu, .amax_out = q.amax_out};
+            .C2 = q.c2, .m_split = q.m_split, .relu = p.splits > 1 ? 0 : q.relu, .amax_out = q.amax_out,
+            .pairs = pair_epilogue()};
 }
 
 static int reduce_slabs(const PlanesCall& q, int splits, hipStream_t st) {
     const long long total = (long long)q.m * q.n;
-    const unsigned rgrid = (unsigned)std::min<long long>((total + 255) / 256, q.relu ? 1024 : 4096);
+    const uintptr_t ptrs = reinterpret_cast<uintptr_t>(q.workspace) | reinterpret_cast<uintptr_t>(q.c) | reinterpret_cast<uintptr_t>(q.c2);
+    const int pairs = (pair_epilogue() && q.n % 2 == 0 && q.ldc % 2 == 0 && (ptrs & 7) == 0) ? 1 : 0;
+    const long long units = pairs ? total / 2 : total;
+    const unsigned rgrid = (unsigned)std::min<long long>((units + 255) / 256, q.relu ? 1024 : 4096);
     hipLaunchKernelGGL(planes_reduce_kernel, dim3(rgrid), dim3(256), 0, st, q.workspace, splits, q.c, (long long)q.ldc, q.bias, q.m, q.n,
-                       q.accumulate ? 1 : 0, q.c2, q.m_split, q.relu, q.amax_out);
+                       q.accumulate ? 1 : 0, q.c2, q.m_split, q.relu, q.amax_out, pairs);
     return launch_status();
 }
 
diff --git a/padertorch_amd/csrc/lstm.hip b/padertorch_amd/csrc/lstm.hip
--- a/padertorch_amd/csrc/lstm.hip
+++ b/padertorch_amd/csrc/lstm.hip
@@ -467,11 +467,11 @@
     return v ? atoi(v) : fallback;
 }
 
-int ptmi_lstm_forward_persistent(float* gates, float* hy, float* c, const float* c0, const float* w_hh_pad,
-                                 const uint32_t* w_hh_amax, const int32_t* batch_sizes_dev, const int64_t* offsets_dev,
-                                 const uint64_t* step_masks, uint32_t* flags, int32_t T, int32_t max_batch, int64_t rows,
-                                 int32_t H, int32_t KP, int32_t ndir, int32_t prefilled, uint32_t* backward_scratch,
-                                 ptmi_stream_t stream) {
+static int forward_persistent(float* gates, float* hy, float* c, const float* c0, const float* w_hh_pad,
+                              const uint32_t* w_hh_amax, const int32_t* batch_sizes_dev, const int64_t* offsets_dev,
+                              const uint64_t* step_masks, uint32_t* flags, int32_t T, int32_t max_batch, int64_t rows,
+                              int32_t H, int32_t KP, int32_t ndir, int32_t prefilled, uint32_t* backward_scratch,
+                              float* ext, int64_t pad, ptmi_stream_t stream) {
     PTMI_RETURN_IF(!gates || !hy || !c || !w_hh_pad || !batch_sizes_dev || !offsets_dev || !flags, PTMI_E_INVALID);
     PTMI_RETURN_IF(T < 1 || max_batch < 1 || H < 1 || (ndir != 1 && ndir != 2) || rows < 1, PTMI_E_INVALID);
     const bool uniform = rows == (int64_t)T * max_batch;
@@ -481,13 +481,15 @@
     PTMI_RETURN_IF(!P.ok, PTMI_E_UNSUPPORTED);
     const long long hy_bytes = rows * ndir * H * 4;
     PTMI_RETURN_IF(hy_bytes > 0x7fffffffLL, PTMI_E_UNSUPPORTED);
+    const size_t pad_words = ext ? (size_t)pad * ndir * H : 0, pad_stride = ext ? (size_t)(pad + rows) * ndir * H : 0;
+    PTMI_RETURN_IF(ext && (pad < 1 || hy != ext + pad_words || (reinterpret_cast<uintptr_t>(ext) & 15) != 0), PTMI_E_INVALID);
 
     hipStream_t st = static_cast<hipStream_t>(stream);
     const int64_t plane_elems = lstm_tile_elems(T, ndir, max_batch, P.KP32), flag_elems = ptmi_lstm_flags_elems(T, ndir, max_batch);
     float* const hyt = reinterpret_cast<float*>(flags);
     flags += plane_elems;
-    if (!prefilled) {
-        int fe = daf_fill_and_zero(hyt, (size_t)plane_elems, flags, (size_t)flag_elems, st);
+    if (!prefilled || ext) {
+        int fe = daf_fill_and_zero(hyt, prefilled ? 0 : (size_t)plane_elems, flags, (size_t)flag_elems, st, ext, pad_words, pad_stride);
         if (fe) return fe;
     } else {
         hipError_t e = zero_words_async(flags, (size_t)flag_elems, st);
@@ -517,6 +519,25 @@
         if (rc) return rc;
     }
     return PTMI_OK;
+}
+
+int ptmi_lstm_forward_persistent(float* gates, float* hy, float* c, const float* c0, const float* w_hh_pad,
+                                 const uint32_t* w_hh_amax, const int32_t* batch_sizes_dev, const int64_t* offsets_dev,
+                                 const uint64_t* step_masks, uint32_t* flags, int32_t T, int32_t max_batch, int64_t rows,
+                                 int32_t H, int32_t KP, int32_t ndir, int32_t prefilled, uint32_t* backward_scratch,
+                                 ptmi_stream_t stream) {
+    return forward_persistent(gates, hy, c, c0, w_hh_pad, w_hh_amax, batch_sizes_dev, offsets_dev, step_masks, flags, T, max_batch, rows, H, KP,
+                              ndir, prefilled, backward_scratch, nullptr, 0, stream);
+}
+
+int ptmi_lstm_forward_persistent_padded(float* gates, float* ext, int64_t pad, float* c, const float* c0, const float* w_hh_pad,
+                                        const uint32_t* w_hh_amax, const int32_t* batch_sizes_dev, const int64_t* offsets_dev,
+                                        const uint64_t* step_masks, uint32_t* flags, int32_t T, int32_t max_batch, int64_t rows,
+                                        int32_t H, int32_t KP, int32_t ndir, int32_t prefilled, uint32_t* backward_scratch,
+                                        ptmi_stream_t stream) {
+    PTMI_RETURN_IF(!ext || pad < 1 || H < 1 || (ndir != 1 && ndir != 2), PTMI_E_INVALID);
+    return forward_persistent(gates, ext + pad * ndir * H, c, c0, w_hh_pad, w_hh_amax, batch_sizes_dev, offsets_dev, step_masks, flags, T,
+                              max_batch, rows, H, KP, ndir, prefilled, backward_scratch, ext, pad, stream);
 }
 
 __global__ void zero_tp_tail_kernel(uint4* planes, long long tiles, int kb_total) {
diff --git a/padertorch_amd/csrc/lstm_common.h b/padertorch_amd/csrc/lstm_common.h
--- a/padertorch_amd/csrc/lstm_common.h
+++ b/padertorch_amd/csrc/lstm_common.h
@@ -100,7 +100,8 @@
 
 
 bool fwd_split_instantiated(int jt, int mtl);
-int daf_fill_and_zero(void* p, size_t words, void* z, size_t zero_words, hipStream_t st);
+int daf_fill_and_zero(void* p, size_t words, void* z, size_t zero_words, hipStream_t st, void* z2 = nullptr, size_t z2_words = 0,
+                      size_t z2_stride = 0);
 int launch_fwd_split(const LstmPersistArgs& A, int jt, int mtl, dim3 grid, hipStream_t st);
 int launch_bwd_split(const LstmPersistBwdArgs& A, int mtl, unsigned nwg, hipStream_t st);
 
diff --git a/padertorch_amd/csrc/lstm_split.hip b/padertorch_amd/csrc/lstm_split.hip
--- a/padertorch_amd/csrc/lstm_split.hip
+++ b/padertorch_amd/csrc/lstm_split.hip
@@ -52,17 +52,19 @@
     }
 };
 
-__global__ void fill_and_zero_kernel(uint4* p, size_t n16, unsigned word, unsigned* z, size_t nz) {
+__global__ void fill_and_zero_kernel(uint4* p, size_t n16, unsigned word, unsigned* z, size_t nz, uint4* z2, size_t n2, size_t stride2) {
     const uint4 v = make_uint4(word, word, word, word);
     const size_t i0 = (size_t)blockIdx.x * blockDim.x + threadIdx.x, step = (size_t)gridDim.x * blockDim.x;
     for (size_t i = i0; i < n16; i += step) p[i] = v;
     for (size_t i = i0; i < nz; i += step) z[i] = 0u;
-}
-
-int daf_fill_and_zero(void* p, size_t words, void* z, size_t zero_words, hipStream_t st) {
-    const size_t n16 = words / 4;
-    const unsigned grid = (unsigned)std::min<size_t>((std::max(n16, zero_words) + 255) / 256, 8192);
-    hipLaunchKernelGGL(fill_and_zero_kernel, dim3(grid), dim3(256), 0, st, static_cast<uint4*>(p), n16, kFill, static_cast<unsigned*>(z), zero_words);
+    for (size_t i = i0; i < 2 * n2; i += step) z2[i < n2 ? i : i - n2 + stride2] = make_uint4(0u, 0u, 0u, 0u);
+}
+
+int daf_fill_and_zero(void* p, size_t words, void* z, size_t zero_words, hipStream_t st, void* z2, size_t z2_words, size_t z2_stride) {
+    const size_t n16 = words / 4, n2 = z2 ? z2_words / 4 : 0;
+    const unsigned grid = (unsigned)std::min<size_t>((std::max(std::max(n16, zero_words), 2 * n2) + 255) / 256, 8192);
+    hipLaunchKernelGGL(fill_and_zero_kernel, dim3(grid), dim3(256), 0, st, static_cast<uint4*>(p), n16, kFill, static_cast<unsigned*>(z), zero_words,
+                       static_cast<uint4*>(z2), n2, z2_stride / 4);
     return launch_status();
 }
 
diff --git a/padertorch_amd/csrc/pit_loss.hip b/padertorch_amd/csrc/pit_loss.hip
--- a/padertorch_amd/csrc/pit_loss.hip
+++ b/padertorch_amd/csrc/pit_loss.hip
@@ -131,9 +131,9 @@
     }
 }
 
-__global__ void pit_assign_kernel(const double* __restrict__ sse, int batch, int nvar, int K, int F,
-                                  long long t_len, const int32_t* row_frames, float* __restrict__ loss,
-                                  int32_t* __restrict__ perm_out, float* ex_loss, float* scratch) {
+__device__ __forceinline__ void assign_examples(const double* sse, int batch, int nvar, int K, int F, long long t_len,
+                                                const int32_t* row_frames, float* __restrict__ loss,
+                                                int32_t* __restrict__ perm_out, float* ex_loss, float* scratch) {
     const int total = batch * nvar;
     for (int id = threadIdx.x; id < total; id += blockDim.x) {
         const int b = id / nvar;
@@ -173,6 +173,39 @@
     }
 }
 
+__global__ void pit_assign_kernel(const double* __restrict__ sse, int batch, int nvar, int K, int F,
+                                  long long t_len, const int32_t* row_frames, float* __restrict__ loss,
+                                  int32_t* __restrict__ perm_out, float* ex_loss, float* scratch) {
+    assign_examples(sse, batch, nvar, K, F, t_len, row_frames, loss, perm_out, ex_loss, scratch);
+}
+
+constexpr int kAhead = 16;
+__global__ __launch_bounds__(256) void pit_reduce_assign_kernel(const double* __restrict__ partial, double* sse, int nchunks,
+                                                                int batch, int nvar, int K, int F, long long t_len,
+                                                                const int32_t* row_frames, float* __restrict__ loss,
+                                                                int32_t* __restrict__ perm_out, float* ex_loss, float* scratch) {
+    const int per = nvar * K * K;
+    const long long words = (long long)batch * per;
+    for (long long id = threadIdx.x; id < words; id += blockDim.x) {
+        const int b = (int)(id / per), e = (int)(id - (long long)b * per);
+        const long long T_b = row_frames ? (long long)row_frames[b] : t_len;
+        const int used = (int)min((T_b + kTChunk - 1) / kTChunk, (long long)nchunks);
+        const double* p = partial + (long long)b * nchunks * per + e;
+        double s = 0.0;
+        for (int c0 = 0; c0 < used; c0 += kAhead) {
+            double v[kAhead];
+#pragma unroll
+            for (int u = 0; u < kAhead; ++u) v[u] = c0 + u < used ? p[(long long)(c0 + u) * per] : 0.0;
+#pragma unroll
+            for (int u = 0; u < kAhead; ++u)
+                if (c0 + u < used) s += v[u];
+        }
+        sse[id] = s;
+    }
+    __syncthreads();
+    assign_examples(sse, batch, nvar, K, F, t_len, row_frames, loss, perm_out, ex_loss, scratch);
+}
+
 struct PitBwdArgs {
     const float* est;
     const float* obs;
@@ -240,14 +273,8 @@
     return batch * nchunks * 2 * K * K + batch * 2;
 }
 
-int ptmi_pit_pairwise_sse(const float* est, const float* obs, const float* tgt, const float* tgt_scale,
-                          int64_t batch, int64_t t_len, const int64_t* strides, int32_t K, int32_t F,
-                          const int32_t* row_frames, double* workspace, double* sse,
-                          ptmi_stream_t stream) {
-    PTMI_RETURN_IF(!est || !tgt || !workspace || !sse || !strides, PTMI_E_INVALID);
-    PTMI_RETURN_IF(batch < 0 || t_len < 0 || K < 1 || F < 1, PTMI_E_INVALID);
-    if (batch == 0) return PTMI_OK;
-    hipStream_t st = static_cast<hipStream_t>(stream);
+static int launch_pairwise(const float* est, const float* obs, const float* tgt, const float* tgt_scale, int64_t batch, int64_t t_len,
+                           const int64_t* strides, int32_t K, int32_t F, const int32_t* row_frames, double* workspace, hipStream_t st) {
     PitArgs A{};
     A.est = est;
     A.obs = obs;
@@ -262,7 +289,6 @@
     A.F = F;
     A.nvar = tgt_scale ? 2 : 1;
     A.nchunks = (int)((t_len + kTChunk - 1) / kTChunk);
-    const int per = A.nvar * K * K;
     if (A.nchunks > 0) {
         const long long blocks = (long long)batch * A.nchunks;
         PTMI_RETURN_IF(blocks > 0x7fffffffLL, PTMI_E_UNSUPPORTED);
@@ -275,11 +301,44 @@
                 PTMI_RETURN_IF(K * K > 65535, PTMI_E_UNSUPPORTED);
                 hipLaunchKernelGGL(pit_pairwise_generic_kernel, dim3((unsigned)blocks, (unsigned)(K * K)), dim3(256), 0, st, A, workspace);
         }
-        int rc = launch_status();
-        if (rc) return rc;
-    }
-    hipLaunchKernelGGL(pit_reduce_kernel, dim3((unsigned)batch), dim3(64), 0, st, workspace, sse, A.nchunks, per,
+        return launch_status();
+    }
+    return PTMI_OK;
+}
+
+int ptmi_pit_pairwise_sse(const float* est, const float* obs, const float* tgt, const float* tgt_scale,
+                          int64_t batch, int64_t t_len, const int64_t* strides, int32_t K, int32_t F,
+                          const int32_t* row_frames, double* workspace, double* sse,
+                          ptmi_stream_t stream) {
+    PTMI_RETURN_IF(!est || !tgt || !workspace || !sse || !strides, PTMI_E_INVALID);
+    PTMI_RETURN_IF(batch < 0 || t_len < 0 || K < 1 || F < 1, PTMI_E_INVALID);
+    if (batch == 0) return PTMI_OK;
+    hipStream_t st = static_cast<hipStream_t>(stream);
+    int rc = launch_pairwise(est, obs, tgt, tgt_scale, batch, t_len, strides, K, F, row_frames, workspace, st);
+    if (rc) return rc;
+    const int nchunks = (int)((t_len + kTChunk - 1) / kTChunk);
+    hipLaunchKernelGGL(pit_reduce_kernel, dim3((unsigned)batch), dim3(64), 0, st, workspace, sse, nchunks, (tgt_scale ? 2 : 1) * K * K,
                        row_frames, (long long)t_len);
+    return launch_status();
+}
+
+int ptmi_pit_pairwise_partials(const float* est, const float* obs, const float* tgt, const float* tgt_scale,
+                               int64_t batch, int64_t t_len, const int64_t* strides, int32_t K, int32_t F,
+                               const int32_t* row_frames, double* workspace, ptmi_stream_t stream) {
+    PTMI_RETURN_IF(!est || !tgt || !workspace || !strides, PTMI_E_INVALID);
+    PTMI_RETURN_IF(batch < 0 || t_len < 0 || K < 1 || F < 1, PTMI_E_INVALID);
+    if (batch == 0) return PTMI_OK;
+    return launch_pairwise(est, obs, tgt, tgt_scale, batch, t_len, strides, K, F, row_frames, workspace, static_cast<hipStream_t>(stream));
+}
+
+int ptmi_pit_assign_chunks(const double* workspace, double* sse, int64_t batch, int32_t nvar, int32_t K, int32_t F, int64_t t_len,
+                           const int32_t* row_frames, float* loss, int32_t* perm, float* ex_loss, ptmi_stream_t stream) {
+    PTMI_RETURN_IF(!workspace || !sse || !loss || !perm || !ex_loss, PTMI_E_INVALID);
+    PTMI_RETURN_IF(batch < 1 || batch > 0x7fffffffLL / (2 * kMaxK * kMaxK) || nvar < 1 || nvar > 2 || K < 1 || t_len < 0, PTMI_E_INVALID);
+    PTMI_RETURN_IF(K > kMaxK, PTMI_E_UNSUPPORTED);
+    const int nchunks = (int)((t_len + kTChunk - 1) / kTChunk);
+    hipLaunchKernelGGL(pit_reduce_assign_kernel, dim3(1), dim3(256), 0, static_cast<hipStream_t>(stream), workspace, sse, nchunks, (int)batch,
+                       (int)nvar, (int)K, (int)F, (long long)t_len, row_frames, loss, perm, ex_loss, ex_loss);
     return launch_status();
 }
 
diff --git a/padertorch_amd/ops/library.py b/padertorch_amd/ops/library.py
--- a/padertorch_amd/ops/library.py
+++ b/padertorch_amd/ops/library.py
@@ -85,6 +85,9 @@
     return Y_abs, X_abs, cos_pd
 
 
+PIT_GLUE = True
+
+
 @_register('pit_loss_forward(Tensor est, Tensor? obs, Tensor tgt, Tensor? scale, Tensor? row_frames, int B, int T, int K, int F, '
            'int[] strides) -> (Tensor, Tensor, Tensor, Tensor)')
 def pit_loss_forward(est, obs, tgt, scale, row_frames, B, T, K, F, strides):
@@ -94,12 +97,19 @@
     ws = torch.empty(int(lib.ptmi_pit_workspace_elems(B, T, K, F)), dtype=torch.float64, device=dev)
     sse = torch.empty((B, nvar, K, K), dtype=torch.float64, device=dev)
     st = _lib.stream(dev)
+    loss = torch.empty(nvar, dtype=torch.float32, device=dev)
+    perm = torch.empty((B, nvar, K), dtype=torch.int32, device=dev)
+    ex_loss = torch.empty((B, nvar), dtype=torch.float32, device=dev)
+    if PIT_GLUE and B > 0:
+        _lib.check(_lib.timed('pit_pairwise_sse', lib.ptmi_pit_pairwise_partials, est.data_ptr(), _lib.ptr(obs), tgt.data_ptr(),
+                              _lib.ptr(scale), B, T, _lib.strides6(*strides), K, F, _lib.ptr(row_frames), ws.data_ptr(), st),
+                   'ptmi_pit_pairwise_partials')
+        _lib.check(lib.ptmi_pit_assign_chunks(ws.data_ptr(), sse.data_ptr(), B, nvar, K, F, T, _lib.ptr(row_frames), loss.data_ptr(),
+                                              perm.data_ptr(), ex_loss.data_ptr(), st), 'ptmi_pit_assign_chunks')
+        return loss, perm, ex_loss, sse
     _lib.check(_lib.timed('pit_pairwise_sse', lib.ptmi_pit_pairwise_sse, est.data_ptr(), _lib.ptr(obs), tgt.data_ptr(),
                           _lib.ptr(scale), B, T, _lib.strides6(*strides), K, F, _lib.ptr(row_frames), ws.data_ptr(),
                           sse.data_ptr(), st), 'ptmi_pit_pairwise_sse')
-    loss = torch.empty(nvar, dtype=torch.float32, device=dev)
-    perm = torch.empty((B, nvar, K), dtype=torch.int32, device=dev)
-    ex_loss = torch.empty((B, nvar), dtype=torch.float32, device=dev)
     _lib.check(lib.ptmi_pit_assign(sse.data_ptr(), B, nvar, K, F, T, _lib.ptr(row_frames), loss.data_ptr(), perm.data_ptr(),
                                    ex_loss.data_ptr(), st), 'ptmi_pit_assign')
     return loss, perm, ex_loss, sse
@@ -919,9 +929,10 @@
 
 @_register('lstm_recurrence_forward(Tensor(a!) gates, Tensor(b!) hy, Tensor? c0, Tensor w_hh_pad, Tensor? w_amax, Tensor bs_dev, '
            'Tensor offs_dev, int bs_host, int offs_host, int T, int max_batch, int rows, int H, int KP, int ndir, bool persistent, '
-           'Tensor(c!)? scratch=None, bool prefilled=False, Tensor(d!)? backward_scratch=None, Tensor? step_masks=None) -> (Tensor, Tensor?)')
+           'Tensor(c!)? scratch=None, bool prefilled=False, Tensor(d!)? backward_scratch=None, Tensor? step_masks=None, '
+           'Tensor(e!)? ext=None, int pad=0) -> (Tensor, Tensor?)')
 def lstm_recurrence_forward(gates, hy, c0, w_hh_pad, w_amax, bs_dev, offs_dev, bs_host, offs_host, T, max_batch, rows, H, KP, ndir,
-                            persistent, scratch=None, prefilled=False, backward_scratch=None, step_masks=None):
+                            persistent, scratch=None, prefilled=False, backward_scratch=None, step_masks=None, ext=None, pad=0):
     lib = _lib.load()
     dev = gates.device
     st = _lib.stream(dev)
@@ -933,14 +944,23 @@
         flags = scratch if scratch is not None else torch.empty(n, dtype=torch.int32, device=dev)
         assert flags.numel() >= n and flags.dtype == torch.int32
         assert step_masks is None or (step_masks.dtype == torch.int64 and step_masks.numel() == 3 * T)
-        rc = _lib.timed('lstm_forward', lib.ptmi_lstm_forward_persistent, gates.data_ptr(), hy.data_ptr(), c.data_ptr(),
-                        _lib.ptr(c0), w_hh_pad.data_ptr(), _lib.ptr(w_amax), bs_dev.data_ptr(), offs_dev.data_ptr(),
-                        _lib.ptr(step_masks), flags.data_ptr(), T, max_batch, rows, H, KP, ndir,
-                        int(bool(prefilled and scratch is not None)), _lib.ptr(backward_scratch), st)
+        tail = (_lib.ptr(c0), w_hh_pad.data_ptr(), _lib.ptr(w_amax), bs_dev.data_ptr(), offs_dev.data_ptr(), _lib.ptr(step_masks),
+                flags.data_ptr(), T, max_batch, rows, H, KP, ndir, int(bool(prefilled and scratch is not None)),
+                _lib.ptr(backward_scratch), st)
+        if ext is not None:
+            assert pad > 0 and ext.shape == (rows + 2 * pad, ndir * H) and ext.is_contiguous() and ext.dtype == torch.float32 \
+                and hy.data_ptr() == ext.data_ptr() + 4 * pad * ndir * H, (ext.shape, pad, rows)
+            rc = _lib.timed('lstm_forward', lib.ptmi_lstm_forward_persistent_padded, gates.data_ptr(), ext.data_ptr(), pad, c.data_ptr(),
+                            *tail)
+        else:
+            rc = _lib.timed('lstm_forward', lib.ptmi_lstm_forward_persistent, gates.data_ptr(), hy.data_ptr(), c.data_ptr(), *tail)
         if rc != -2 or step_masks is not None:
             _lib.check(rc, 'ptmi_lstm_forward_persistent')
     if rc == -2:
         flags = None
+        if ext is not None:
+            ext[:pad].zero_()
+            ext[pad + rows:].zero_()
         _lib.check(_lib.timed('lstm_forward', lib.ptmi_lstm_forward, gates.data_ptr(), hy.data_ptr(), c.data_ptr(), _lib.ptr(c0),
                               w_hh_pad.data_ptr(), ctypes.c_void_p(bs_host), ctypes.c_void_p(offs_host), T, max_batch, H, KP, ndir,
                               st), 'ptmi_lstm_forward')
diff --git a/padertorch_amd/ops/lstm.py b/padertorch_amd/ops/lstm.py
--- a/padertorch_amd/ops/lstm.py
+++ b/padertorch_amd/ops/lstm.py
@@ -207,6 +207,8 @@
 
 
 GROUP_WGRAD = True
+
+SETUP_LAUNCH = True
 
 
 class _WgradJob:
@@ -398,7 +400,8 @@
         assert masks is None or not stateful, 'row-slot batches take no initial states'
         ext = (torch.zeros if masks is not None else torch.empty)((meta.rows + 2 * pad, ndir * H), dtype=torch.float32, device=x.device)
         hy = ext[pad:pad + meta.rows]
-        if pad:
+        in_setup = bool(pad) and SETUP_LAUNCH and not stateful and ext.data_ptr() % 16 == 0
+        if pad and not in_setup:
             C_ = ndir * H
             torch.as_strided(ext, (2, pad, C_), ((pad + meta.rows) * C_, C_, 1)).zero_()
             if stateful:
@@ -414,7 +417,8 @@
             _watchdog.arm(x.device)
         c, flags = torch.ops.ptmi.lstm_recurrence_forward(
             gates, hy, c0, w_pad, amax_whh, meta.bs_dev, meta.offs_dev, meta.bs_host.ctypes.data, meta.offs_host.ctypes.data,
-            meta.T, meta.max_batch, meta.rows, H, KP, ndir, PERSISTENT, None, False, scratch_b, masks)
+            meta.T, meta.max_batch, meta.rows, H, KP, ndir, PERSISTENT, None, False, scratch_b, masks,
+            *((ext, pad) if in_setup else ()))
         if flags is None:
             pre_b = 0
         if handoff is not None and flags is not None and not stateful and meta.uniform_rows:
```
